# hannes-holey/GaPFlow

Measured on AMD Instinct MI355X. Metric: Mcell-updates/s (fp64), 4096^2 grid, higher is better.
Workload: dtype f64; 1 GPU; 2D journal bearing 4096x4096, fixed DH EOS, all-periodic, adaptive CFL 0.5 (BASELINE.json configs[2]); slabs=1

## Files before the change

### gapflow_amd/_lib.py

```python
import ctypes as C
import os

import numpy as np

HERE = os.path.dirname(os.path.abspath(__file__))
LIB_PATH = os.environ.get('GPF_LIB_PATH', os.path.join(HERE, 'lib', 'libgapflow_hip.so'))

EOS_IDS = {'DH': 0, 'PL': 1, 'vdW': 2, 'MT': 3, 'cubic': 4, 'BWR': 5, 'Bayada': 6}
EOS_KEYS = {'DH': ['rho0', 'P0', 'C1', 'C2'], 'PL': ['rho0', 'P0', 'alpha'], 'vdW': ['M', 'T', 'a', 'b'],
            'MT': ['rho0', 'P0', 'K', 'n'], 'cubic': ['a', 'b', 'c', 'd'], 'BWR': ['T', 'gamma'],
            'Bayada': ['rho_l', 'rho_v', 'c_l', 'c_v']}
EOS_DEFAULTS = {'DH': {'rho0': 877.7007, 'P0': 101325., 'C1': 3.5e8, 'C2': 1.23}, 'PL': {'rho0': 1.1853, 'P0': 101325., 'alpha': 0.},
                'vdW': {'M': 39.948, 'T': 100., 'a': 1.355, 'b': 0.03201}, 'MT': {'rho0': 700., 'P0': 0.101e6, 'K': 0.557e9, 'n': 7.33},
                'cubic': {'a': 15.2, 'b': -9.6, 'c': 3.35, 'd': -0.07}, 'BWR': {'gamma': 3.}, 'Bayada': {}}
PIEZO_IDS = {'Barus': 1, 'Roelands': 2, 'Dukler': 3, 'McAdams': 4}
PIEZO_KEYS = {'Barus': ['aB'], 'Roelands': ['mu_inf', 'p_ref', 'z'], 'Dukler': ['eta_v', 'rho_l', 'rho_v'],
              'McAdams': ['eta_v', 'rho_l', 'rho_v']}
PIEZO_DEFAULTS = {'Barus': {'aB': 2.e-8}, 'Roelands': {'mu_inf': 1.e-3, 'p_ref': 1.96e8, 'z': 0.68},
                  'Dukler': {'eta_v': 3.9e-5, 'rho_l': 850., 'rho_v': 0.019}, 'McAdams': {'eta_v': 3.9e-5, 'rho_l': 850., 'rho_v': 0.019}}
THINNING_DEFAULTS = {'Eyring': {'tauE': 5.e5}, 'Carreau': {'mu_inf': 1.e-3, 'lam': 0.02, 'a': 2., 'N': 0.8}}
THINNING_IDS = {'Eyring': 1, 'Carreau': 2}
THINNING_KEYS = {'Eyring': ['tauE'], 'Carreau': ['mu_inf', 'lam', 'a', 'N']}
BC_P, BC_D, BC_N = 0, 1, 2
FIELD_Q, FIELD_TOPO, FIELD_EXTRA, FIELD_PRESSURE, FIELD_TAU_AVG, FIELD_WALL_LOWER, FIELD_WALL_UPPER = range(7)
FIELD_PRESSURE_VAR, FIELD_WALL_XZ_VAR, FIELD_WALL_YZ_VAR = 7, 8, 9
FIELD_DEFORMATION = 10
PROFILE_Z, PROFILE_U, PROFILE_V, PROFILE_TAU = 1, 2, 4, 8
PROFILE_GRADIENTS = 1
PROFILE_MODES = {'both': 0, 'top': 1, 'bottom': 2, 'none': 3}
FIELD_NCOMP = {FIELD_Q: 3, FIELD_TOPO: 3, FIELD_EXTRA: 1, FIELD_PRESSURE: 1, FIELD_TAU_AVG: 3,
               FIELD_WALL_LOWER: 6, FIELD_WALL_UPPER: 6, 7: 1, 8: 1, 9: 1, 10: 1}


class GpfConfig(C.Structure):
    _fields_ = [('Nx', C.c_int32), ('Ny', C.c_int32), ('dx', C.c_double), ('dy', C.c_double),
                ('U', C.c_double), ('V', C.c_double), ('eta', C.c_double), ('zeta', C.c_double),
                ('eos', C.c_int32), ('eos_par', C.c_double * 8),
                ('piezo', C.c_int32), ('piezo_par', C.c_double * 4),
                ('bc_rule', (C.c_int32 * 3) * 4), ('bc_value', C.c_double * 4),
                ('halo_lo', C.c_int32), ('halo_hi', C.c_int32),
                ('adaptive', C.c_int32), ('CFL', C.c_double), ('dt_fixed', C.c_double), ('tol', C.c_double),
                ('max_it', C.c_int64), ('mc_order', C.c_int32), ('device', C.c_int32),
                ('thinning', C.c_int32), ('thinning_par', C.c_double * 4)]


class GpfScalars(C.Structure):
    _fields_ = [('step', C.c_int64), ('simtime', C.c_double), ('dt', C.c_double), ('ekin', C.c_double),
                ('ekin_old', C.c_double), ('residual', C.c_double), ('v_max', C.c_double), ('v_sound', C.c_double),
                ('mass', C.c_double), ('invalid', C.c_int32), ('converged', C.c_int32)]


_DP = C.POINTER(C.c_double)
_VPP = C.POINTER(C.c_void_p)
SIGNATURES = {
    'gpf_create': (C.c_int, [C.POINTER(GpfConfig), _VPP]),
    'gpf_destroy': (C.c_int, [C.c_void_p]),
    'gpf_set_stream': (C.c_int, [C.c_void_p, C.c_void_p]),
    'gpf_last_error': (C.c_char_p, []),
    'gpf_device_count': (C.c_int, []),
    'gpf_upload': (C.c_int, [C.c_void_p, C.c_int, _DP, C.c_size_t]),
    'gpf_download': (C.c_int, [C.c_void_p, C.c_int, _DP, C.c_size_t]),
    'gpf_update_closures': (C.c_int, [C.c_void_p]),
    'gpf_pre_run': (C.c_int, [C.c_void_p]),
    'gpf_step': (C.c_int, [C.c_void_p, C.c_int64, C.c_int, C.POINTER(GpfScalars), C.c_int64, C.POINTER(C.c_int64)]),
    'gpf_step_unfused': (C.c_int, [C.c_void_p]),
    'gpf_step_timed': (C.c_int, [C.c_void_p, C.c_int64, _DP, _DP]),
    'gpf_scalars': (C.c_int, [C.c_void_p, C.POINTER(GpfScalars)]),
    'gpf_set_ekin_old': (C.c_int, [C.c_void_p, C.c_double]),
    'gpf_set_dt': (C.c_int, [C.c_void_p, C.c_double]),
    'gpf_slab_message': (C.c_int, [C.c_void_p, _VPP, C.POINTER(C.c_size_t)]),
    'gpf_step_local': (C.c_int, [C.c_void_p, C.c_int]),
    'gpf_step_commit': (C.c_int, [C.c_void_p, C.c_int, C.c_void_p, C.c_int, C.c_int, C.c_int]),
    'gpf_state': (C.c_int, [C.c_void_p, C.POINTER(GpfScalars)]),
    'gpf_viscous_stress': (C.c_int, [C.c_int64] + [C.c_void_p] * 6 + [C.c_double] * 3 + [C.c_int] + [C.c_void_p] * 3),
    'gpf_eos': (C.c_int, [C.c_int, C.c_void_p, C.c_int64, C.c_void_p, C.c_void_p, C.c_void_p]),
    'gpf_viscosity': (C.c_int, [C.c_int, C.c_int, C.c_void_p, C.c_double, C.c_int64, C.c_void_p, C.c_void_p, C.c_void_p,
                              C.c_double, C.c_double, C.c_void_p]),
    'gpf_elastic_setup': (C.c_int, [C.c_void_p, C.c_int, C.c_int, C.c_void_p, C.c_size_t, C.c_double, C.c_double, C.c_int]),
    'gpf_elastic_update': (C.c_int, [C.c_void_p]),
    'gpf_elastic_slab_setup': (C.c_int, [C.c_void_p, C.c_int, C.c_int, C.c_int, C.c_void_p, C.c_size_t, C.c_void_p, C.c_size_t,
                                         C.c_void_p, C.c_size_t, C.c_double, C.c_double, C.c_int]),
    'gpf_elastic_slab_buffer': (C.c_int, [C.c_void_p, C.c_int, C.POINTER(C.c_void_p), C.POINTER(C.c_size_t)]),
    'gpf_elastic_slab_forward': (C.c_int, [C.c_void_p, C.c_void_p, C.c_int]),
    'gpf_elastic_slab_convolve': (C.c_int, [C.c_void_p]),
    'gpf_elastic_slab_finish': (C.c_int, [C.c_void_p]),
    'gpf_elastic_slab_apply': (C.c_int, [C.c_void_p]),
    'gpf_p2p_export': (C.c_int, [C.c_void_p, C.c_void_p, C.c_size_t]),
    'gpf_p2p_connect': (C.c_int, [C.c_void_p, C.c_int, C.c_int, C.c_void_p, C.c_int, C.c_int]),
    'gpf_p2p_set_timeout': (C.c_int, [C.c_void_p, C.c_double]),
    'gpf_upload_beyond': (C.c_int, [C.c_void_p, C.c_int, _DP, C.c_size_t]),
    'gpf_stream_probe': (C.c_int, [C.c_int, C.c_int, C.c_int, C.c_int64, C.c_int, _DP]),
    'gpf_step_p2p': (C.c_int, [C.c_void_p, C.c_int64, C.c_int]),
    'gpf_stage_message': (C.c_int, [C.c_void_p]),
    'gpf_stage_absorb': (C.c_int, [C.c_void_p, C.c_void_p, C.c_int, C.c_int, C.c_int]),
    'gpf_close_step_local': (C.c_int, [C.c_void_p]),
    'gpf_close_step_commit': (C.c_int, [C.c_void_p, C.c_void_p, C.c_int, C.POINTER(GpfScalars)]),
    'gpf_set_seam_topo': (C.c_int, [C.c_void_p, C.c_int, _DP, C.c_size_t]),
    'gpf_predictor_corrector': (C.c_int, [C.c_int, C.c_int, _DP, _DP, _DP, C.c_int, _DP, _DP]),
    'gpf_source': (C.c_int, [C.c_int, C.c_int, _DP, _DP, _DP, _DP, _DP, _DP]),
    'gpf_open_step': (C.c_int, [C.c_void_p]),
    'gpf_stage_closures': (C.c_int, [C.c_void_p]),
    'gpf_stage_advance': (C.c_int, [C.c_void_p, C.c_int]),
    'gpf_close_step': (C.c_int, [C.c_void_p, C.POINTER(GpfScalars)]),
    'gpf_gp_fit': (C.c_int, [C.c_int, C.c_int, C.c_int, C.c_int, _DP, _DP, C.c_double, _DP, C.c_double, _DP, _DP, _DP]),
    'gpf_gp_set_model': (C.c_int, [C.c_void_p, C.c_int, C.c_int, C.c_int, C.c_int, C.POINTER(C.c_int32), _DP, _DP, _DP,
                                   C.c_double, _DP, C.c_double, C.c_double]),
    'gpf_gp_clear_model': (C.c_int, [C.c_void_p, C.c_int]),
    'gpf_gp_factorisation': (C.c_char_p, []),
    'gpf_plan_note': (C.c_char_p, [C.c_void_p]),
    'gpf_gp_set_scales': (C.c_int, [C.c_void_p, C.c_int, _DP, C.c_double]),
    'gpf_gp_variance': (C.c_int, [C.c_void_p, C.c_int, C.c_int, _DP]),
    'gpf_gp_pass_counts': (C.c_int, [C.c_void_p, C.POINTER(C.c_int64), C.POINTER(C.c_int64)]),
    'gpf_gp_nll_open': (C.c_int, [C.c_int, C.c_int, C.c_int, C.c_int, _DP, _DP, C.c_double, C.POINTER(C.c_void_p)]),
    'gpf_gp_nll_eval': (C.c_int, [C.c_void_p, _DP, _DP, _DP, C.POINTER(C.c_int)]),
    'gpf_gp_nll_close': (C.c_int, [C.c_void_p]),
    'gpf_gap_profiles_op': (C.c_int, [C.c_int64, C.c_int] + [C.c_void_p] * 8 + [C.c_int, C.c_double, C.c_double, C.c_int, C.c_int,
                                                                              C.c_void_p]),
    'gpf_gap_profiles': (C.c_int, [C.c_void_p, C.c_int, C.c_int, C.c_int, C.c_int, C.c_int, C.c_void_p]),
    'gpf_profile_store_probe': (C.c_int, [C.c_int, C.c_int64, C.c_int, C.c_int, C.c_int, _DP]),
}

_lib = None


class GapflowHipError(RuntimeError):
    pass


def _pin_hip_runtime():
    import sys
    if os.environ.get('GPF_SYSTEM_HIP') == '1':
        return
    if 'torch' in sys.modules:
        libdir = os.path.join(os.path.dirname(sys.modules['torch'].__file__), 'lib')
        for var, name in (('GPF_ROCBLAS_PATH', 'librocblas.so'), ('GPF_HIPFFT_PATH', 'libhipfft.so')):
            if os.path.exists(os.path.join(libdir, name)):
                os.environ.setdefault(var, os.path.join(libdir, name))
        return
    try:
        import importlib.util
        spec = importlib.util.find_spec('torch')
    except (ImportError, ValueError):
        spec = None
    if spec is None or not spec.submodule_search_locations:
        return
    libdir = os.path.join(list(spec.submodule_search_locations)[0], 'lib')
    cand = os.path.join(libdir, 'libamdhip64.so')
    if os.path.exists(cand):
        C.CDLL(cand, mode=C.RTLD_GLOBAL)
        for var, name in (('GPF_ROCBLAS_PATH', 'librocblas.so'), ('GPF_HIPFFT_PATH', 'libhipfft.so')):
            if os.path.exists(os.path.join(libdir, name)):
                os.environ.setdefault(var, os.path.join(libdir, name))


def _preload_rocsolver():
    if os.environ.get('GPF_USE_ROCSOLVER') == '0':
        return
    path = os.environ.get('GPF_ROCBLAS_PATH')
    try:
        blas = C.CDLL(path if path and os.path.exists(path) else 'librocblas.so.5', mode=C.RTLD_GLOBAL)
    except OSError:
        return
    info = _DlInfo()
    libdl = C.CDLL(None)
    libdl.dladdr.argtypes, libdl.dladdr.restype = [C.c_void_p, C.POINTER(_DlInfo)], C.c_int
    if not libdl.dladdr(C.cast(blas.rocblas_create_handle, C.c_void_p), C.byref(info)) or not info.dli_fname:
        return
    here = os.path.dirname(info.dli_fname.decode())
    for name in ('librocsolver.so.0', 'librocsolver.so'):
        if os.path.exists(os.path.join(here, name)):
            try:
                C.CDLL(os.path.join(here, name), mode=C.RTLD_GLOBAL)
            except OSError:
                pass
            return


class _DlInfo(C.Structure):
    _fields_ = [('dli_fname', C.c_char_p), ('dli_fbase', C.c_void_p), ('dli_sname', C.c_char_p), ('dli_saddr', C.c_void_p)]


def load():
    global _lib
    if _lib is None:
        _pin_hip_runtime()
        _preload_rocsolver()
        if not os.path.exists(LIB_PATH):
            raise GapflowHipError(
                f"{LIB_PATH} not found: build it with `python -m gapflow_amd.build` (needs hipcc). "
                "gapflow_amd has no CPU fallback.")
        lib = C.CDLL(LIB_PATH)
        for name, (res, args) in SIGNATURES.items():
            fn = getattr(lib, name)
            fn.restype, fn.argtypes = res, args
        _lib = lib
    return _lib


def check(code):
    if code != 0:
        raise GapflowHipError(f"libgapflow_hip error {code}: {load().gpf_last_error().decode()}")


def require_device():
    lib = load()
    if lib.gpf_device_count() < 1:
        raise GapflowHipError("no HIP device visible: gapflow_amd runs its hot path on an MI355X only "
                              "(there is no CPU fallback)")
    return lib


def as_dp(a):
    return a.ctypes.data_as(_DP)


def f64c(a):
    return np.ascontiguousarray(a, dtype=np.float64)
```

### gapflow_amd/csrc/api.hip

```cpp
#include <hip/hip_runtime.h>
#include <algorithm>
#include <cmath>
#include <cstdio>
#include <cstdlib>
#include <cstring>
#include <map>
#include <mutex>
#include <string>
#include <tuple>
#include <vector>

#include "../../include/gapflow_hip.h"
#include "phys_setup.hpp"
#include "step_kernel.hip"
#include "aux_kernels.hip"
#include "step2_kernel.hip"
#include "gp_kernels.hip"
#include "elastic_kernels.hip"
#include "small_kernel.hip"
#include "profile_kernels.hip"

using namespace gpf;

static thread_local std::string g_err;
static const bool g_debug = std::getenv("GPF_DEBUG") != nullptr;
#define DBG(...) do { if (g_debug) { std::fprintf(stderr, "[gpf] " __VA_ARGS__); std::fprintf(stderr, "\n"); std::fflush(stderr); } } while (0)

static int fail(int code, const std::string& msg) {
    g_err = msg;
    return code;
}

struct gpf_handle;
static int enter(gpf_handle* h, bool reads_only = false);

#define HIP_TRY(expr)                                                                                   \
    do {                                                                                                \
        hipError_t e_ = (expr);                                                                         \
        if (e_ != hipSuccess)                                                                           \
            return fail(GPF_ERR_HIP, std::string(#expr) + ": " + hipGetErrorString(e_));               \
    } while (0)

#define GPF_TRY(expr)                                                                                   \
    do {                                                                                                \
        int r_ = (expr);                                                                                \
        if (r_ != GPF_OK) return r_;                                                                    \
    } while (0)

static_assert(sizeof(LogEntry) == sizeof(gpf_scalars_t), "LogEntry must mirror gpf_scalars_t");
static constexpr size_t PLANE_PAD_BYTES = 256;

struct gpf_handle {
    gpf_config cfg;
    Layout L;
    Edges E;
    Phys P;
    hipStream_t stream = nullptr;
    size_t field_bytes = 0;
    double* q[2] = {nullptr, nullptr};
    double* topo = nullptr;
    double* topo_line = nullptr;
    int topo_mode = 0;
    bool topo_hy0 = false;
    double* Ls = nullptr;
    double* g1 = nullptr;
    double* seam = nullptr;
    bool has_seam[2] = {false, false};
    struct { bool on = false; int nranks = 0, rank = 0, rank_lo = -1, rank_hi = -1; char* mine = nullptr;
             char* box[P2P_MAX_RANKS] = {}; unsigned long long* seq = nullptr; } p2p;
    double* halo = nullptr;
    double* beyond = nullptr;
    StepState* st = nullptr;
    Partial* partials = nullptr;
    unsigned int* arrive = nullptr;
    long long p2p_timeout_ticks = P2P_TIMEOUT_TICKS;
    bool split_edges = false;
    bool g1_ready = false;
    Partial* block_partials = nullptr;
    int nghost_blocks = 0;
    ScalarPartial* spart = nullptr;
    int nspart = 0;
    LogEntry* log = nullptr;
    long long log_cap = 0;
    double* stage = nullptr;
    size_t stage_doubles = 0;
    double* fields = nullptr;
    double* work = nullptr;
    struct GpHost {
        bool set = false;
        GpModelDev dev;
        double *Z = nullptr, *alpha = nullptr, *L = nullptr, *Linv = nullptr, *W = nullptr;
        int cap = 0;
        bool has_linv = false;
        double xscale0 = 1.0;
        double inv_scale[GP_MAX_D] = {};
        double yscale_fit = 1.0;
    } gp[3];
    double* gp_state_mean = nullptr;
    bool gp_state_mean_valid = false;
    long long gp_state_mean_step = -1;
    bool gp_state_mean_fresh = false;
    bool open_first_closures = false;
    bool gp_reuse_state_mean = true;
    long long gp_passes[3] = {0, 0, 0}, gp_reused = 0;
    double* gpvar = nullptr;
    double* gpscratch = nullptr;
    int gpscratch_n = 0;
    struct { bool on = false; int px = 0, py = 0, relative = 0; double alpha = 1.0, scale = 1.0; void* plan_f = nullptr; void* plan_b = nullptr;
             double2* greens = nullptr; double2* spec = nullptr; double* dense = nullptr;
             double* u_prev = nullptr; double* h0 = nullptr; double* deformation = nullptr; } el;
    struct { bool on = false; int px = 0, py = 0, nky = 0, nranks = 1, relative = 0;
             int row0 = 0, nrows = 0, k0 = 0, nk = 0, nret = 0, nrows_all = 0, nmain = 0, main_g0 = 0, seam_side = -1, seam_g0 = 0, ref_row = -1;
             double alpha = 1.0, scale = 1.0;
             void* plan_y = nullptr; void* plan_x = nullptr; void* plan_yb = nullptr; int nxg = 0, g_lo = 0;
             double* dense = nullptr; double2* spec = nullptr; double2* send1 = nullptr; double2* recv1 = nullptr; double2* xspec = nullptr;
             double2* greens = nullptr; double2* send2 = nullptr; double2* recv2 = nullptr; double2* line = nullptr; double* ureal = nullptr;
             double* u_prev = nullptr; double* h0 = nullptr; double* deformation = nullptr; double* ref = nullptr; int* rows_all = nullptr; } els;
    double* gptile = nullptr;
    size_t gptile_doubles = 0;
    void* blas = nullptr;
    bool step_open = false;
    int open_parity = 0;
    bool has_q = false, has_topo = false, pre_run_done = false;
    bool prev_state_valid = false;
    long long host_step = 0;
    long long next_step = 0;
    Strip2Geom geom2[2];
    int nchunks2 = 0, nblocks2 = 0, npartials2_cap = 0, nblock_partials_cap = 0;
    bool plan2_valid = false;
    int nt_policy2 = 0;
    int keep_rows2 = 0;
    StepState* st_trial = nullptr;
    double* plan_master = nullptr;
    char plan2_note[400] = "";
};

static int enter(gpf_handle* h, bool reads_only) {
    HIP_TRY(hipSetDevice(h->cfg.device));
    if (!reads_only) h->gp_state_mean_valid = false;
    return GPF_OK;
}

static void make_phys(const gpf_config& c, Phys& P) {
    setup_phys(P, c.U, c.V, c.eta, c.zeta, c.dx, c.dy, c.eos, c.eos_par, c.piezo, c.piezo_par, c.thinning, c.thinning_par);
}

static int blocks_for(long long n, int bs = 256, int cap = 4096) {
    long long b = (n + bs - 1) / bs;
    return (int)std::max<long long>(1, std::min<long long>(b, cap));
}

#ifdef GPF_ONLY_EOS_DH
#define EOS_DISPATCH(eos, ...)                                                                          \
    do {                                                                                                \
        if ((eos) == GPF_EOS_DH) { constexpr int EOS_ = EOS_DH; __VA_ARGS__; }       \
    } while (0)
#else
#define EOS_DISPATCH(eos, ...)                                                                          \
    switch (eos) {                                                                                      \
    case GPF_EOS_DH: { constexpr int EOS_ = EOS_DH; __VA_ARGS__; } break;                              \
    case GPF_EOS_PL: { constexpr int EOS_ = EOS_PL; __VA_ARGS__; } break;                              \
    case GPF_EOS_VDW: { constexpr int EOS_ = EOS_VDW; __VA_ARGS__; } break;                            \
    case GPF_EOS_MT: { constexpr int EOS_ = EOS_MT; __VA_ARGS__; } break;                              \
    case GPF_EOS_CUBIC: { constexpr int EOS_ = EOS_CUBIC; __VA_ARGS__; } break;                        \
    case GPF_EOS_BWR: { constexpr int EOS_ = EOS_BWR; __VA_ARGS__; } break;                            \
    default: { constexpr int EOS_ = EOS_BAYADA; __VA_ARGS__; } break;                                  \
    }
#endif

#define LS_PIEZO_DISPATCH(ls, pz, ...)                                                                  \
    do {                                                                                                \
        if (ls) {                                                                                       \
            constexpr bool LS_ = true;                                                                  \
            if (pz) { constexpr bool PZ_ = true; __VA_ARGS__; } else { constexpr bool PZ_ = false; __VA_ARGS__; }     \
        } else {                                                                                        \
            constexpr bool LS_ = false;                                                                 \
            if (pz) { constexpr bool PZ_ = true; __VA_ARGS__; } else { constexpr bool PZ_ = false; __VA_ARGS__; }     \
        }                                                                                               \
    } while (0)

extern "C" const char* gpf_last_error(void) { return g_err.c_str(); }

extern "C" int gpf_device_count(void) {
    int n = 0;
    if (hipGetDeviceCount(&n) != hipSuccess) return 0;
    return n;
}

static int ensure_stage(gpf_handle* h, size_t doubles) {
    if (h->stage_doubles >= doubles) return GPF_OK;
    if (h->stage) HIP_TRY(hipFree(h->stage));
    h->stage = nullptr; h->stage_doubles = 0;
    HIP_TRY(hipMalloc(&h->stage, doubles * sizeof(double)));
    h->stage_doubles = doubles;
    return GPF_OK;
}

#include "api_fields.inc"

extern "C" int gpf_create(const gpf_config* cfg, gpf_handle** out) {
    if (!cfg || !out) return fail(GPF_ERR_INVALID, "gpf_create: null argument");
    if (cfg->Nx < 1 || cfg->Ny < 1) return fail(GPF_ERR_INVALID, "gpf_create: Nx, Ny must be >= 1");
    if (!(cfg->dx > 0) || !(cfg->dy > 0)) return fail(GPF_ERR_INVALID, "gpf_create: dx, dy must be > 0");
    if (((long long)cfg->Nx + 2) * ((long long)cfg->Ny + 2 + 64) > 2000000000ll)
        return fail(GPF_ERR_INVALID, "gpf_create: more than 2e9 cells per plane; cut the domain into x-slabs (gapflow_amd/slab.py)");
    if (cfg->eos < GPF_EOS_DH || cfg->eos > GPF_EOS_BAYADA) return fail(GPF_ERR_INVALID, "gpf_create: unknown EOS id");
    if (cfg->thinning < 0 || cfg->thinning > GPF_THINNING_CARREAU) return fail(GPF_ERR_INVALID, "gpf_create: unknown shear-thinning id");
    for (int e = 0; e < 4; ++e) {
        int np = 0;
        for (int c = 0; c < 3; ++c) {
            int r = cfg->bc_rule[e][c];
            if (r < 0 || r > 2) return fail(GPF_ERR_INVALID, "gpf_create: bad ghost rule");
            np += (r == GPF_BC_PERIODIC);
        }
        if (np != 0 && np != 3)
            return fail(GPF_ERR_INVALID, "gpf_create: an edge must be periodic for all components or for none "
                                         "(problem.py:682-707 applies the periodic copy only when all three are 'P')");
    }
#ifdef GPF_ONLY_EOS_DH
    if (cfg->eos != GPF_EOS_DH) return fail(GPF_ERR_INVALID, "gpf_create: this build (-DGPF_ONLY_EOS_DH) holds the Dowson-Higginson kernels only");
#endif
    int ndev = 0;
    if (hipGetDeviceCount(&ndev) != hipSuccess || ndev == 0)
        return fail(GPF_ERR_NO_DEVICE, "gpf_create: no HIP device visible (this library has no CPU path)");
    if (cfg->device < 0 || cfg->device >= ndev) return fail(GPF_ERR_INVALID, "gpf_create: device ordinal out of range");
    HIP_TRY(hipSetDevice(cfg->device));

    gpf_handle* h = new gpf_handle();
    h->cfg = *cfg;
    Layout& L = h->L;
    L.Nx = cfg->Nx; L.Ny = cfg->Ny; L.off = 15;
    L.pitch = ((cfg->Ny + 2 + L.off + 15) / 16) * 16;
    if (const char* s = std::getenv("GPF_PITCH_PAD")) L.pitch += (std::atoi(s) / 16) * 16;
    L.plane = (long long)(cfg->Nx + 2) * L.pitch;
    if (const char* s = std::getenv("GPF_PLANE_PAD")) L.plane += (std::atoll(s) & ~1ll);
    for (int e = 0; e < 4; ++e) {
        for (int c = 0; c < 3; ++c) h->E.rule[e][c] = cfg->bc_rule[e][c];
        h->E.value[e] = cfg->bc_value[e];
    }
    h->E.halo[0] = cfg->halo_lo; h->E.halo[1] = cfg->halo_hi;
    h->split_edges = std::getenv("GPF_STEP_UNFUSED_EDGES") != nullptr;
    h->gp_reuse_state_mean = std::getenv("GPF_GP_NO_STATE_MEAN") == nullptr;
    make_phys(*cfg, h->P);

    const size_t plane_b = (size_t)L.plane * sizeof(double);
    auto cleanup = [&](int code) { gpf_destroy(h); return code; };
#define HIP_TRY_C(expr)                                                                                 \
    do {                                                                                                \
        hipError_t e_ = (expr);                                                                         \
        if (e_ != hipSuccess)                                                                           \
            return cleanup(fail(GPF_ERR_HIP, std::string(#expr) + ": " + hipGetErrorString(e_)));      \
    } while (0)
    h->field_bytes = (3 * plane_b + PLANE_PAD_BYTES + 255) & ~(size_t)255;
    for (int b = 0; b < 2; ++b) {
        HIP_TRY_C(field_malloc((void**)&h->q[b], h->field_bytes));
        if (field_zero(0, h->q[b], h->field_bytes) != GPF_OK) { gpf_destroy(h); return GPF_ERR_HIP; }
    }
    HIP_TRY_C(field_malloc((void**)&h->topo, h->field_bytes));
    if (field_zero(0, h->topo, h->field_bytes) != GPF_OK) { gpf_destroy(h); return GPF_ERR_HIP; }
    HIP_TRY_C(hipDeviceSynchronize());
    const size_t g1n = (size_t)3 * L.pitch + (size_t)3 * (L.Nx + 2);
    HIP_TRY_C(hipMalloc(&h->g1, g1n * sizeof(double)));
    HIP_TRY_C(hipMemset(h->g1, 0, g1n * sizeof(double)));
    HIP_TRY_C(hipMalloc(&h->st, sizeof(StepState)));
    HIP_TRY_C(hipMemset(h->st, 0, sizeof(StepState)));
    h->nghost_blocks = std::max(1, std::min(64, (2 * (L.Ny + 2) + 2 * L.Nx + 255) / 256));
    HIP_TRY_C(hipMalloc(&h->arrive, 4 * sizeof(unsigned int)));
    HIP_TRY_C(hipMemset(h->arrive, 0, 4 * sizeof(unsigned int)));
    HIP_TRY_C(hipMalloc(&h->block_partials, 1024 * sizeof(Partial)));
    h->nspart = 1024;
    HIP_TRY_C(hipMalloc(&h->spart, (size_t)(h->nspart + 8) * sizeof(ScalarPartial)));
    HIP_TRY_C(hipMemset(h->spart, 0, (size_t)(h->nspart + 8) * sizeof(ScalarPartial)));
    h->log_cap = 4096;
    HIP_TRY_C(hipMalloc(&h->log, (size_t)h->log_cap * sizeof(LogEntry)));
#undef HIP_TRY_C
    *out = h;
    return GPF_OK;
}

extern "C" int gpf_destroy(gpf_handle* h) {
    if (!h) return GPF_OK;
    hipSetDevice(h->cfg.device);
    hipStreamSynchronize(h->stream);
    for (void* p : {(void*)h->q[0], (void*)h->q[1], (void*)h->topo, (void*)h->plan_master}) field_free(p);
    void* ptrs[] = {h->topo_line, h->Ls, h->g1, h->seam, h->halo, h->beyond, h->st, h->partials, h->arrive, h->block_partials, h->spart,
                    h->log, h->stage, h->fields, h->work, h->st_trial, h->gpvar, h->gp_state_mean, h->gpscratch, h->gptile,
                    h->gp[0].Z, h->gp[0].alpha, h->gp[0].L, h->gp[1].Z, h->gp[1].alpha, h->gp[1].L,
                    h->gp[2].Z, h->gp[2].alpha, h->gp[2].L, h->gp[0].Linv, h->gp[1].Linv, h->gp[2].Linv, h->gp[0].W, h->gp[1].W, h->gp[2].W};
    if (h->blas && roclibs().ok) roclibs().destroy(h->blas);
    if (h->el.plan_f) fftlib().destroy(h->el.plan_f);
    if (h->el.plan_b) fftlib().destroy(h->el.plan_b);
    for (void* p : {(void*)h->el.greens, (void*)h->el.spec, (void*)h->el.dense, (void*)h->el.u_prev})
        if (p) hipFree(p);
    for (void* pl : {h->els.plan_y, h->els.plan_x, h->els.plan_yb})
        if (pl) fftlib().destroy(pl);
    for (void* p : {(void*)h->els.dense, (void*)h->els.spec, (void*)h->els.send1, (void*)h->els.recv1, (void*)h->els.xspec, (void*)h->els.greens,
                    (void*)h->els.send2, (void*)h->els.recv2, (void*)h->els.line, (void*)h->els.ureal, (void*)h->els.u_prev, (void*)h->els.ref,
                    (void*)h->els.rows_all})
        if (p) hipFree(p);
    for (int r = 0; r < h->p2p.nranks; ++r)
        if (h->p2p.box[r] && r != h->p2p.rank) hipIpcCloseMemHandle(h->p2p.box[r]);
    if (h->p2p.mine) hipFree(h->p2p.mine);
    if (h->p2p.seq) hipFree(h->p2p.seq);
    for (void* p : ptrs)
        if (p) hipFree(p);
    delete h;
    return GPF_OK;
}

extern "C" int gpf_set_stream(gpf_handle* h, void* s) {
    if (!h) return fail(GPF_ERR_INVALID, "null handle");
    h->stream = (hipStream_t)s;
    return GPF_OK;
}

static int field_ncomp(int field) {
    switch (field) {
    case GPF_FIELD_Q: return 3;
    case GPF_FIELD_TOPO: return 3;
    case GPF_FIELD_EXTRA: return 1;
    case GPF_FIELD_PRESSURE: return 1;
    case GPF_FIELD_TAU_AVG: return 3;
    case GPF_FIELD_WALL_LOWER: return 6;
    case GPF_FIELD_WALL_UPPER: return 6;
    case GPF_FIELD_PRESSURE_VAR: case GPF_FIELD_WALL_XZ_VAR: case GPF_FIELD_WALL_YZ_VAR: return 1;
    case GPF_FIELD_DEFORMATION: return 1;
    }
    return 0;
}

static int current_parity(gpf_handle* h, int* par) {
    StepState s;
    HIP_TRY(hipMemcpyAsync(&s, h->st, sizeof(s), hipMemcpyDeviceToHost, h->stream));
    HIP_TRY(hipStreamSynchronize(h->stream));
    *par = s.parity;
    return GPF_OK;
}

static int ensure_fields(gpf_handle* h) {
    if (h->fields) return GPF_OK;
    HIP_TRY(hipMalloc(&h->fields, (size_t)16 * h->L.plane * sizeof(double)));
    HIP_TRY(hipMemsetAsync(h->fields, 0, (size_t)16 * h->L.plane * sizeof(double), h->stream));
    return GPF_OK;
}

extern "C" int gpf_upload(gpf_handle* h, int field, const double* host, size_t count) {
    if (!h || !host) return fail(GPF_ERR_INVALID, "gpf_upload: null argument");
    GPF_TRY(enter(h));
    const Layout& L = h->L;
    const int nc = field_ncomp(field);
    if (field != GPF_FIELD_Q && field != GPF_FIELD_TOPO && field != GPF_FIELD_EXTRA)
        return fail(GPF_ERR_INVALID, "gpf_upload: only q, topography and the extra field are inputs");
    const size_t ncell = (size_t)(L.Nx + 2) * (L.Ny + 2);
    if (count != ncell * nc) return fail(GPF_ERR_INVALID, "gpf_upload: count does not match ncomp*(Nx+2)*(Ny+2)");
    double* dst = nullptr;
    if (field == GPF_FIELD_Q) {
        int par = 0;
        GPF_TRY(current_parity(h, &par));
        dst = h->q[par];
    } else if (field == GPF_FIELD_TOPO) {
        dst = h->topo;
    } else {
        bool nz = false;
        for (size_t i = 0; i < count && !nz; ++i) nz = host[i] != 0.0;
        if (!nz && !h->Ls) return GPF_OK;
        if (!h->Ls) { HIP_TRY(hipMalloc(&h->Ls, (size_t)L.plane * sizeof(double) + PLANE_PAD_BYTES)); h->plan2_valid = false; }
        HIP_TRY(hipMemsetAsync(h->Ls, 0, (size_t)L.plane * sizeof(double), h->stream));
        dst = h->Ls;
    }
    if (field == GPF_FIELD_TOPO) {
        const int nx = L.Nx + 2, ny = L.Ny + 2;
        bool xonly = true, yonly = true;
        for (int c = 0; c < 3 && (xonly || yonly); ++c)
            for (int ix = 0; ix < nx && (xonly || yonly); ++ix) {
                const double* row = host + ((size_t)c * nx + ix) * ny;
                const double* row0 = host + (size_t)c * nx * ny;
                for (int iy = 0; iy < ny; ++iy) {
                    if (std::memcmp(&row[iy], &row[0], 8) != 0) xonly = false;
                    if (std::memcmp(&row[iy], &row0[iy], 8) != 0) yonly = false;
                }
            }
        const int mode = xonly ? 1 : (yonly ? 2 : 0);
        if (mode != h->topo_mode) { h->plan2_valid = false; }
        h->topo_mode = (h->el.on || h->els.on) ? 0 : mode;
        if (mode) {
            const int n = mode == 1 ? nx : ny;
            std::vector<double> line((size_t)3 * n);
            for (int c = 0; c < 3; ++c)
                for (int i = 0; i < n; ++i)
                    line[(size_t)c * n + i] = mode == 1 ? host[((size_t)c * nx + i) * ny] : host[(size_t)c * nx * ny + i];
            bool hy0 = mode == 1;
            for (int i = 0; i < n && hy0; ++i) hy0 = line[(size_t)2 * n + i] == 0.0;
            if (hy0 != h->topo_hy0) h->plan2_valid = false;
            h->topo_hy0 = hy0;
            if (!h->topo_line) HIP_TRY(hipMalloc(&h->topo_line, (size_t)3 * (std::max(nx, ny)) * sizeof(double)));
            HIP_TRY(hipMemcpy(h->topo_line, line.data(), line.size() * sizeof(double), hipMemcpyHostToDevice));
        }
    }
    GPF_TRY(ensure_stage(h, count));
    HIP_TRY(hipMemcpyAsync(h->stage, host, count * sizeof(double), hipMemcpyHostToDevice, h->stream));
    hipLaunchKernelGGL(k_pack, dim3(blocks_for((long long)count)), dim3(256), 0, h->stream, h->stage, dst, L, nc);
    HIP_TRY(hipGetLastError());
    HIP_TRY(hipStreamSynchronize(h->stream));
    if (field == GPF_FIELD_Q) h->has_q = true;
    h->g1_ready = false;
    h->prev_state_valid = false;
    if (field == GPF_FIELD_TOPO) h->has_topo = true;
    return GPF_OK;
}

extern "C" int gpf_download(gpf_handle* h, int field, double* host, size_t count) {
    if (!h || !host) return fail(GPF_ERR_INVALID, "gpf_download: null argument");
    GPF_TRY(enter(h, true));
    const Layout& L = h->L;
    const int nc = field_ncomp(field);
    if (nc == 0) return fail(GPF_ERR_INVALID, "gpf_download: unknown field id");
    const size_t ncell = (size_t)(L.Nx + 2) * (L.Ny + 2);
    if (count != ncell * nc) return fail(GPF_ERR_INVALID, "gpf_download: count does not match ncomp*(Nx+2)*(Ny+2)");
    const double* src = nullptr;
    switch (field) {
    case GPF_FIELD_Q: {
        int par = 0;
        GPF_TRY(current_parity(h, &par));
        src = h->q[par];
        break;
    }
    case GPF_FIELD_TOPO: src = h->topo; break;
    case GPF_FIELD_EXTRA:
        if (!h->Ls) { std::memset(host, 0, count * sizeof(double)); return GPF_OK; }
        src = h->Ls; break;
    case GPF_FIELD_DEFORMATION:
        if (!h->el.on && !h->els.on) { std::memset(host, 0, count * sizeof(double)); return GPF_OK; }
        src = h->el.on ? h->el.deformation : h->els.deformation; break;
    case GPF_FIELD_PRESSURE_VAR: case GPF_FIELD_WALL_XZ_VAR: case GPF_FIELD_WALL_YZ_VAR:
        if (!h->gpvar) return fail(GPF_ERR_STATE, "gpf_download: no GP variance has been computed");
        src = h->gpvar + (size_t)(field - GPF_FIELD_PRESSURE_VAR) * L.plane;
        break;
    default:
        if (!h->fields) return fail(GPF_ERR_STATE, "gpf_download: derived fields requested before gpf_update_closures");
        src = h->fields + (field == GPF_FIELD_PRESSURE ? 0 : field == GPF_FIELD_TAU_AVG ? 1 : field == GPF_FIELD_WALL_LOWER ? 4 : 10) * L.plane;
    }
    GPF_TRY(ensure_stage(h, count));
    hipLaunchKernelGGL(k_unpack, dim3(blocks_for((long long)count)), dim3(256), 0, h->stream, src, h->stage, L, nc);
    HIP_TRY(hipGetLastError());
    HIP_TRY(hipMemcpyAsync(host, h->stage, count * sizeof(double), hipMemcpyDeviceToHost, h->stream));
    HIP_TRY(hipStreamSynchronize(h->stream));
    return GPF_OK;
}

static FieldPtrs field_ptrs(gpf_handle* h) {
    FieldPtrs F;
    F.p = h->fields; F.tau = h->fields + h->L.plane; F.lower = h->fields + 4 * h->L.plane; F.upper = h->fields + 10 * h->L.plane;
    return F;
}

static int gp_launch_mean(gpf_handle* h, int which, const double* q, bool with_grad, double* c2_out);
static int read_state(gpf_handle* h, StepState& s);

static const double* beyond_rows(gpf_handle* h, const double* q) {
    if (!h->beyond || (h->E.halo[0] != 1 && h->E.halo[1] != 1)) return nullptr;
    const bool working = h->step_open && q == h->q[h->open_parity ^ 1];
    return h->beyond + (working ? 2 * h->L.pitch : 0);
}

static int launch_fields(gpf_handle* h, const double* q, bool pressure_mean_cached = false) {
    GPF_TRY(ensure_fields(h));
    const Layout& L = h->L;
    const long long n = (long long)(L.Nx + 2) * (L.Ny + 2);
    FieldPtrs F = field_ptrs(h);
    EOS_DISPATCH(h->cfg.eos, {
        if (h->cfg.thinning != GPF_THINNING_NONE) {
            hipLaunchKernelGGL((k_pressure<EOS_>), dim3(blocks_for(n)), dim3(256), 0, h->stream, q, F.p, L, h->P);
            if ((h->E.halo[0] == 1 || h->E.halo[1] == 1) && !h->beyond)
                return fail(GPF_ERR_STATE, "shear thinning on a slab: upload the rows beyond the halo first (gpf_upload_beyond)");
            const double* by = beyond_rows(h, q);
            if (h->Ls) hipLaunchKernelGGL((k_fields_thinning<EOS_, true>), dim3(blocks_for(n)), dim3(256), 0, h->stream, q, h->topo, h->Ls, F, L, h->P, h->cfg.dx, h->cfg.dy, h->E.halo[0], h->E.halo[1], by);
            else hipLaunchKernelGGL((k_fields_thinning<EOS_, false>), dim3(blocks_for(n)), dim3(256), 0, h->stream, q, h->topo, (const double*)nullptr, F, L, h->P, h->cfg.dx, h->cfg.dy, h->E.halo[0], h->E.halo[1], by);
        } else if (h->Ls) hipLaunchKernelGGL((k_fields<EOS_, true>), dim3(blocks_for(n)), dim3(256), 0, h->stream, q, h->topo, h->Ls, F, L, h->P);
        else hipLaunchKernelGGL((k_fields<EOS_, false>), dim3(blocks_for(n)), dim3(256), 0, h->stream, q, h->topo, (const double*)nullptr, F, L, h->P);
    });
    HIP_TRY(hipGetLastError());
    for (int w = 0; w < 3; ++w) {
        if (!h->gp[w].set) continue;
        if (w == 0 && pressure_mean_cached) {
            HIP_TRY(hipMemcpyAsync(F.p, h->gp_state_mean, (size_t)L.plane * sizeof(double), hipMemcpyDeviceToDevice, h->stream));
            h->gp_reused += 1;
        } else GPF_TRY(gp_launch_mean(h, w, q, false, nullptr));
    }
    return GPF_OK;
}

extern "C" int gpf_update_closures(gpf_handle* h) {
    if (!h) return fail(GPF_ERR_INVALID, "null handle");
    if (!h->has_q || !h->has_topo) return fail(GPF_ERR_STATE, "gpf_update_closures: upload q and topography first");
    GPF_TRY(enter(h));
    int par = 0;
    GPF_TRY(current_parity(h, &par));
    if (h->prev_state_valid && !h->E.halo[0] && !h->E.halo[1]) {
        const Layout& L = h->L;
        StepState s;
        GPF_TRY(read_state(h, s));
        double* w = h->q[par ^ 1];
        const long long n = (long long)(L.Nx + 2) * (L.Ny + 2);
        const int nb = blocks_for(n);
        if (!h->work) HIP_TRY(hipMalloc(&h->work, (size_t)9 * L.plane * sizeof(double)));
        GPF_TRY(launch_fields(h, w));
        double *fx = h->work, *fy = h->work + 3 * L.plane, *src = h->work + 6 * L.plane;
        FieldPtrs F = field_ptrs(h);
        const int mc = h->cfg.mc_order;
        const int sw = mc == 0 ? (((s.step - 1) % 2 == 0) ? 1 : -1) : mc;
        const int dir = ((sw + 1) / 2) ? 1 : -1;
        hipLaunchKernelGGL(k_fluxdiff, dim3(nb), dim3(256), 0, h->stream, w, F.p, F.tau, dir, fx, fy, L);
        hipLaunchKernelGGL(k_source, dim3(nb), dim3(256), 0, h->stream, w, h->topo, F.tau, F.lower, F.upper, src, L);
        hipLaunchKernelGGL(k_axpy, dim3(nb), dim3(256), 0, h->stream, w, fx, fy, src, (const double*)&h->st->dt_last, h->cfg.dx, h->cfg.dy, L);
        hipLaunchKernelGGL(k_bc_x, dim3((L.Ny + 2 + 255) / 256), dim3(256), 0, h->stream, w, L, h->E);
        hipLaunchKernelGGL(k_bc_y, dim3((L.Nx + 2 + 255) / 256), dim3(256), 0, h->stream, w, L, h->E);
        HIP_TRY(hipGetLastError());
        GPF_TRY(launch_fields(h, w));
        h->prev_state_valid = false;
    } else {
        GPF_TRY(launch_fields(h, h->q[par]));
    }
    HIP_TRY(hipStreamSynchronize(h->stream));
    return GPF_OK;
}

static int launch_scalars(gpf_handle* h, const double* q, ScalarPartial* total, bool need_sound_speed = true) {
    const Layout& L = h->L;
    const int row0 = h->E.halo[0] == 1 ? 1 : 0, row1 = h->E.halo[1] == 1 ? L.Nx : L.Nx + 1;
    const long long n = (long long)(row1 - row0 + 1) * (L.Ny + 2);
    const int nb = blocks_for(n, 256, h->nspart);
    EOS_DISPATCH(h->cfg.eos, {
        hipLaunchKernelGGL((k_scalars<EOS_>), dim3(nb), dim3(256), 0, h->stream, q, h->topo, L, h->P, row0, row1, h->spart);
    });
    HIP_TRY(hipGetLastError());
    hipLaunchKernelGGL(k_scalars_final, dim3(1), dim3(256), 0, h->stream, h->spart, nb, total);
    HIP_TRY(hipGetLastError());
    if (h->gp[0].set && need_sound_speed) GPF_TRY(gp_launch_mean(h, 0, q, true, &total->c2));
    return GPF_OK;
}

static void fill_scalars(const StepState& s, const ScalarPartial* sp, double dxdy, gpf_scalars_t* out) {
    out->step = s.step; out->simtime = s.simtime; out->dt = s.dt;
    out->ekin = sp ? sp->ekin : s.ekin; out->ekin_old = s.ekin_old; out->residual = s.residual;
    out->v_max = std::sqrt(sp ? sp->v2 : s.vmax2);
    out->v_sound = (sp && ((int)sp->flags & 4)) ? std::nan("") : std::sqrt(sp ? sp->c2 : s.c2max);
    out->mass = sp ? sp->mass * dxdy : 0.0;
    out->invalid = s.invalid; out->converged = s.converged;
}

extern "C" int gpf_scalars(gpf_handle* h, gpf_scalars_t* out) {
    if (!h || !out) return fail(GPF_ERR_INVALID, "gpf_scalars: null argument");
    if (!h->has_q || !h->has_topo) return fail(GPF_ERR_STATE, "gpf_scalars: upload q and topography first");
    GPF_TRY(enter(h, true));
    int par = 0;
    GPF_TRY(current_parity(h, &par));
    ScalarPartial* tot = h->spart + h->nspart;
    h->gp_state_mean_fresh = false;
    GPF_TRY(launch_scalars(h, h->q[par], tot));
    ScalarPartial sp; StepState s;
    HIP_TRY(hipMemcpyAsync(&sp, tot, sizeof(sp), hipMemcpyDeviceToHost, h->stream));
    HIP_TRY(hipMemcpyAsync(&s, h->st, sizeof(s), hipMemcpyDeviceToHost, h->stream));
    HIP_TRY(hipStreamSynchronize(h->stream));
    if (h->gp_state_mean_fresh && s.parity == par) {
        h->gp_state_mean_valid = true;
        h->gp_state_mean_step = s.step;
    }
    h->gp_state_mean_fresh = false;
    fill_scalars(s, &sp, h->cfg.dx * h->cfg.dy, out);
    return GPF_OK;
}

static int write_state(gpf_handle* h, const StepState& s) {
    HIP_TRY(hipMemcpyAsync(h->st, &s, sizeof(s), hipMemcpyHostToDevice, h->stream));
    HIP_TRY(hipStreamSynchronize(h->stream));
    return GPF_OK;
}
static int read_state(gpf_handle* h, StepState& s) {
    HIP_TRY(hipMemcpyAsync(&s, h->st, sizeof(s), hipMemcpyDeviceToHost, h->stream));
    HIP_TRY(hipStreamSynchronize(h->stream));
    return GPF_OK;
}

extern "C" int gpf_set_ekin_old(gpf_handle* h, double v) {
    if (!h) return fail(GPF_ERR_INVALID, "null handle");
    StepState s;
    GPF_TRY(read_state(h, s));
    s.ekin_old = v;
    return write_state(h, s);
}

extern "C" int gpf_set_dt(gpf_handle* h, double dt) {
    if (!h) return fail(GPF_ERR_INVALID, "null handle");
    StepState s;
    GPF_TRY(read_state(h, s));
    s.dt = dt;
    h->g1_ready = false;
    return write_state(h, s);
}

extern "C" int gpf_pre_run(gpf_handle* h) {
    if (!h) return fail(GPF_ERR_INVALID, "null handle");
    if (!h->has_q || !h->has_topo) return fail(GPF_ERR_STATE, "gpf_pre_run: upload q and topography first");
    GPF_TRY(enter(h));
    gpf_scalars_t sc;
    GPF_TRY(gpf_scalars(h, &sc));
    StepState s;
    GPF_TRY(read_state(h, s));
    const gpf_config& c = h->cfg;
    s.hmin = std::min(c.dx, c.dy);
    s.tol = c.tol; s.CFL = c.CFL; s.adaptive = c.adaptive; s.mc_order = c.mc_order; s.max_it = c.max_it;
    s.step = 0; s.simtime = 0.0; s.residual = 1.0;
    s.rbuf[0] = 1.0; s.rcount = 1; s.rhead = 0;
    s.converged = (1.0 < c.tol) ? 1 : 0;
    s.invalid = 0;
    s.dt_last = 0.0;
    if (!h->pre_run_done) s.ekin_old = sc.ekin;
    s.ekin = sc.ekin;
    s.vmax2 = sc.v_max * sc.v_max; s.c2max = sc.v_sound * sc.v_sound;
    const double dt_crit = s.hmin / (sc.v_max + sc.v_sound);
    s.dt = c.adaptive ? c.CFL * dt_crit : c.dt_fixed;
    GPF_TRY(write_state(h, s));
    h->pre_run_done = true;
    h->g1_ready = false;
    h->prev_state_valid = false;
    h->host_step = 0; h->next_step = 0;
    return GPF_OK;
}

static int topo_mode_of(const gpf_handle* h) {
    if (h->Ls != nullptr || h->cfg.piezo != 0 || std::getenv("GPF_TOPO_PLANES")) return 0;
    if (h->topo_mode == 1 && h->topo_hy0 && !std::getenv("GPF_TOPO_GENERIC")) return 3;
    return h->topo_mode;
}

typedef void (*step2_kernel_t)(const Step2Args, const Phys);

static step2_kernel_t step2_kernel(int eos, bool has_ls, bool piezo, int D, int topo_mode) {
    step2_kernel_t k = nullptr;
    EOS_DISPATCH(eos, {
        if (piezo) {
            if (has_ls) k = D > 0 ? k_step2<EOS_, true, true, 1, 0> : k_step2<EOS_, true, true, -1, 0>;
            else k = D > 0 ? k_step2<EOS_, false, true, 1, 0> : k_step2<EOS_, false, true, -1, 0>;
        } else if (has_ls) {
            k = D > 0 ? k_step2<EOS_, true, false, 1, 0> : k_step2<EOS_, true, false, -1, 0>;
        } else if (topo_mode == 1) {
            k = D > 0 ? k_step2<EOS_, false, false, 1, 1> : k_step2<EOS_, false, false, -1, 1>;
        } else if (topo_mode == 2) {
            k = D > 0 ? k_step2<EOS_, false, false, 1, 2> : k_step2<EOS_, false, false, -1, 2>;
        } else if (topo_mode == 3) {
            k = D > 0 ? k_step2<EOS_, false, false, 1, 3> : k_step2<EOS_, false, false, -1, 3>;
        } else {
            k = D > 0 ? k_step2<EOS_, false, false, 1, 0> : k_step2<EOS_, false, false, -1, 0>;
        }
    });
    return k;
}

static Strip2Geom strip2_geom(const Layout& L, int D) {
    Strip2Geom G;
    const int e = (D < 0 && (L.Ny & 1)) ? 1 : 0;
    for (int k = 0; k < 2; ++k) {
        G.w0 = -1 - e - 4 * k;
        G.s_ghost = (L.Ny - G.w0 - 1) / STRIP2;
        const int p_ny = L.Ny - G.w0 - STRIP2 * G.s_ghost;
        G.lane_ghost = (p_ny + 1) >> 1; G.slot_ghost = (p_ny + 1) & 1;
        if (G.lane_ghost + 2 <= 63) break;
    }
    G.nstrips = G.s_ghost + 1;
    G.lane_wrap = G.lane_ghost + 1;
    const int p0 = -G.w0;
    G.wrap_ma = (p0 % 2 == 0) ? 0 : -1;
    const int d = 1 - G.wrap_ma;
    G.wrap_src_lane = G.lane_wrap + d / 2; G.wrap_src_slot = d & 1;
    return G;
}

static bool step2_fused(const gpf_handle* h) { return !h->split_edges; }

#include "api_plan.inc"

#ifndef GPF_SLAB_COMMIT_BLOCKS
#define GPF_SLAB_COMMIT_BLOCKS 24
#endif
constexpr int SLAB_COMMIT_BLOCKS = GPF_SLAB_COMMIT_BLOCKS;

static P2PArgs p2p_args(gpf_handle* h, bool on) {
    P2PArgs c;
    c.on = on ? 1 : 0; c.nranks = h->p2p.nranks; c.rank = h->p2p.rank; c.rank_lo = h->p2p.rank_lo; c.rank_hi = h->p2p.rank_hi;
    for (int r = 0; r < P2P_MAX_RANKS; ++r) c.box[r] = h->p2p.box[r];
    c.seq = h->p2p.seq; c.qa = h->q[0]; c.qb = h->q[1];
    return c;
}

static int ghost_args(gpf_handle* h, int honor_stop, GhostArgs& g) {
    const Layout& L = h->L;
    g.qa = h->q[0]; g.qb = h->q[1]; g.topo = h->topo; g.Ls = h->Ls;
    for (int e = 0; e < 2; ++e) {
        g.seam[e] = nullptr;
        if (h->E.halo[e] == 2) {
            if (!h->has_seam[e]) return fail(GPF_ERR_STATE, "periodic slab seam: call gpf_set_seam_topo for this edge first");
            g.seam[e] = h->seam + (size_t)e * 8 * L.pitch;
        }
    }
    g.g1x = h->g1; g.g1y = h->g1 + 3 * L.pitch;
    g.st = h->st; g.L = L; g.E = h->E; g.honor_stop = honor_stop;
    return GPF_OK;
}

static void fill_step2_args(gpf_handle* h, Step2Args& a2, int D, int honor_stop, long long log_base, double* slab_out, bool p2p) {
    const Layout& L = h->L;
    const bool fused = step2_fused(h);
    const Strip2Geom& G2 = h->geom2[D > 0 ? 0 : 1];
    a2.qa = h->q[0]; a2.qb = h->q[1]; a2.topo = h->topo; a2.topo_line = h->topo_line; a2.Ls = h->Ls;
    a2.g1x = h->g1; a2.g1y = h->g1 + 3 * L.pitch;
    a2.st = h->st; a2.partials = h->partials; a2.block_partials = h->block_partials; a2.arrive = h->arrive;
    a2.log = h->log; a2.log_base = log_base; a2.log_cap = h->log_cap;
    a2.L = L; a2.E = h->E; a2.G = G2; a2.nchunks = h->nchunks2; a2.fused = (fused ? 1 : 0) | (h->nt_policy2 >= 1 ? 2 : 0) | (h->nt_policy2 >= 2 ? 4 : 0) |
               (h->nt_policy2 >= 1 ? h->keep_rows2 << 3 : 0); a2.honor_stop = honor_stop;
    const bool slab = slab_out != nullptr;
    for (int e = 0; e < 2; ++e) a2.seam[e] = (h->E.halo[e] == 2 && h->has_seam[e]) ? h->seam + (size_t)e * 8 * L.pitch : nullptr;
    a2.out = slab_out; a2.msg = (slab && !p2p) ? h->halo : nullptr; a2.p2p = p2p_args(h, p2p);
}

static int enqueue_step(gpf_handle* h, int honor_stop, long long log_base, double* slab_out,
                        hipEvent_t ev0 = nullptr, hipEvent_t ev1 = nullptr, bool p2p = false) {
    const Layout& L = h->L;
    const int mc = h->cfg.mc_order;
    const int D = mc == 0 ? ((h->next_step % 2 == 0) ? 1 : -1) : (((mc + 1) / 2) ? 1 : -1);
    GPF_TRY(plan_step2(h, D));
    h->next_step += 1;
    const bool fused = step2_fused(h);
    const Strip2Geom& G2 = h->geom2[D > 0 ? 0 : 1];
    const int np_step = G2.nstrips * h->nchunks2;
    GhostArgs g;
    GPF_TRY(ghost_args(h, honor_stop, g));
    Step2Args a2;
    fill_step2_args(h, a2, D, honor_stop, log_base, slab_out, p2p);
    const bool slab = slab_out != nullptr;
    FinishArgs f;
    f.partials = h->partials; f.st = h->st;
    f.log = h->log; f.log_base = log_base; f.log_cap = h->log_cap; f.out = slab_out; f.honor_stop = honor_stop;
    f.L = L; f.E = h->E;
    f.p2p = p2p_args(h, p2p);
    f.arrive = h->arrive; f.msg = slab ? h->halo : nullptr;
    f.nstep_partials = np_step; f.block_partials = h->block_partials;
    GhostFillArgs gf;
    gf.qa = h->q[0]; gf.qb = h->q[1]; gf.st = h->st;
    gf.L = L; gf.E = h->E; gf.honor_stop = honor_stop;

    const int ntiles = (L.Nx + L.Ny + 63) / 64;
    const dim3 ggrid(std::min(ntiles, 512));
    const int nsend = slab ? std::min((6 * L.pitch + 1023) / 1024, 256) : 0;
    WaitArgs w;
    w.qa = h->q[0]; w.qb = h->q[1]; w.st = h->st; w.log = h->log; w.log_base = log_base; w.log_cap = h->log_cap;
    w.L = L; w.E = h->E; w.honor_stop = honor_stop; w.arrive = h->arrive + 1; w.timeout_ticks = h->p2p_timeout_ticks; w.p2p = f.p2p;
    w.gathered = nullptr; w.msg_len = 0; w.nranks = 0; w.rank_lo = w.rank_hi = -1; w.stage1 = fused ? 0 : 1;
    const bool has_ls = h->Ls != nullptr;
    if (fused) {
        const step2_kernel_t k2 = step2_kernel(h->cfg.eos, h->Ls != nullptr, h->cfg.piezo != 0, D, topo_mode_of(h));
        if (ev0) hipEventRecord(ev0, h->stream);
        hipLaunchKernelGGL(k2, dim3(h->nblocks2), dim3(256), 0, h->stream, a2, h->P);
        if (ev1) hipEventRecord(ev1, h->stream);
        if (p2p) {
            const dim3 cgrid(SLAB_COMMIT_BLOCKS);
            EOS_DISPATCH(h->cfg.eos, {
                hipLaunchKernelGGL((k_begin_slab<EOS_, false, false, false, true>), cgrid, dim3(256), 0, h->stream, g, w, h->P);
            });
        }
        h->g1_ready = false;
        HIP_TRY(hipGetLastError());
        return GPF_OK;
    }
    EOS_DISPATCH(h->cfg.eos, {
        if (!h->g1_ready) {
            if (topo_mode_of(h) == 3) hipLaunchKernelGGL((k_ghost_stage1<EOS_, false, false, true>), ggrid, dim3(256), 0, h->stream, g, h->P);
            else LS_PIEZO_DISPATCH(has_ls, h->cfg.piezo != 0, hipLaunchKernelGGL((k_ghost_stage1<EOS_, LS_, PZ_, false>), ggrid, dim3(256), 0, h->stream, g, h->P));
        }
        if (ev0) hipEventRecord(ev0, h->stream);
        hipLaunchKernelGGL(step2_kernel(h->cfg.eos, h->Ls != nullptr, h->cfg.piezo != 0, D, topo_mode_of(h)), dim3(h->nblocks2), dim3(256), 0, h->stream, a2, h->P);
        if (ev1) hipEventRecord(ev1, h->stream);
        hipLaunchKernelGGL((k_ghost_fill<EOS_>), dim3(h->nghost_blocks + nsend), dim3(256), 0, h->stream, gf, f, h->nghost_blocks, h->P);
        if (p2p) {
            if (topo_mode_of(h) == 3) hipLaunchKernelGGL((k_begin_slab<EOS_, false, false, true, true>), ggrid, dim3(256), 0, h->stream, g, w, h->P);
            else LS_PIEZO_DISPATCH(has_ls, h->cfg.piezo != 0, hipLaunchKernelGGL((k_begin_slab<EOS_, LS_, PZ_, false, true>), ggrid, dim3(256), 0, h->stream, g, w, h->P));
        }
    });
    h->g1_ready = p2p;
    HIP_TRY(hipGetLastError());
    return GPF_OK;
}

static bool small_grid_eligible(gpf_handle* h) {
    static const bool off = getenv("GPF_SMALL_GRID") && atoi(getenv("GPF_SMALL_GRID")) == 0;
    const long long nc = (long long)(h->L.Nx + 2) * (h->L.Ny + 2);
    return !off && nc * SMALL_DOUBLES_PER_CELL * 8 <= 150 * 1024 && h->cfg.thinning == GPF_THINNING_NONE && !h->E.halo[0] && !h->E.halo[1] &&
           !h->gp[0].set && !h->gp[1].set && !h->gp[2].set && !h->el.on;
}

static int enqueue_small_steps(gpf_handle* h, int nsteps, int honor_stop, long long log_base) {
    const Layout& L = h->L;
    SmallArgs a;
    a.qa = h->q[0]; a.qb = h->q[1]; a.topo = h->topo; a.Ls = h->Ls; a.st = h->st;
    a.log = h->log; a.log_base = log_base; a.log_cap = h->log_cap; a.L = L; a.E = h->E; a.nsteps = nsteps; a.honor_stop = honor_stop;
    const size_t lds = (size_t)(L.Nx + 2) * (L.Ny + 2) * SMALL_DOUBLES_PER_CELL * 8;
    EOS_DISPATCH(h->cfg.eos, {
        if (h->Ls) {
            HIP_TRY(hipFuncSetAttribute((const void*)k_small_steps<EOS_, true>, hipFuncAttributeMaxDynamicSharedMemorySize, (int)lds));
            hipLaunchKernelGGL((k_small_steps<EOS_, true>), dim3(1), dim3(512), lds, h->stream, a, h->P);
        } else {
            HIP_TRY(hipFuncSetAttribute((const void*)k_small_steps<EOS_, false>, hipFuncAttributeMaxDynamicSharedMemorySize, (int)lds));
            hipLaunchKernelGGL((k_small_steps<EOS_, false>), dim3(1), dim3(512), lds, h->stream, a, h->P);
        }
    });
    HIP_TRY(hipGetLastError());
    h->next_step += nsteps;
    h->g1_ready = false;
    return GPF_OK;
}

extern "C" int gpf_step(gpf_handle* h, int64_t n, int honor_stop, gpf_scalars_t* log, int64_t log_capacity,
                        int64_t* n_executed) {
    if (!h) return fail(GPF_ERR_INVALID, "null handle");
    if (!h->pre_run_done) return fail(GPF_ERR_STATE, "gpf_step: call gpf_pre_run first (Problem._pre_run, problem.py:412)");
    if (h->E.halo[0] || h->E.halo[1]) return fail(GPF_ERR_STATE, "gpf_step: this handle is a slab; use gpf_step_local / gpf_step_commit");
    if (h->cfg.thinning != GPF_THINNING_NONE)
        return fail(GPF_ERR_STATE, "gpf_step: shear thinning needs grad p (a wider stencil than the fused step has); use the stage-wise calls");
    if (n < 0) return fail(GPF_ERR_INVALID, "gpf_step: n < 0");
    GPF_TRY(enter(h));
    int64_t done = 0, logged = 0;
    const bool small = small_grid_eligible(h);
    while (done < n) {
        const int64_t batch = std::min<int64_t>(n - done, h->log_cap);
        const long long base = h->host_step;
        if (small) GPF_TRY(enqueue_small_steps(h, (int)batch, honor_stop, base));
        else for (int64_t i = 0; i < batch; ++i) GPF_TRY(enqueue_step(h, honor_stop, base, nullptr));
        StepState s;
        GPF_TRY(read_state(h, s));
        const long long ran = s.step - base;
        const long long entries = ran + ((s.invalid && ran < batch) ? 1 : 0);
        if (log && entries > 0) {
            const long long take = std::min<long long>(entries, log_capacity - logged);
            if (take > 0) {
                HIP_TRY(hipMemcpy(log + logged, h->log, (size_t)take * sizeof(LogEntry), hipMemcpyDeviceToHost));
                logged += take;
            }
        }
        h->host_step = s.step; h->next_step = s.step;
        h->prev_state_valid = ran >= 1 && !s.invalid;
        done += batch;
        if (ran < batch) break;
    }
    if (n_executed) *n_executed = h->host_step;
    return GPF_OK;
}

extern "C" int gpf_step_timed(gpf_handle* h, int64_t n, double* kernel_ms, double* total_ms) {
    if (!h || !kernel_ms || !total_ms) return fail(GPF_ERR_INVALID, "gpf_step_timed: null argument");
    if (!h->pre_run_done) return fail(GPF_ERR_STATE, "gpf_step_timed: call gpf_pre_run first");
    if (n < 1 || n > h->log_cap) return fail(GPF_ERR_INVALID, "gpf_step_timed: 1 <= n <= 4096");
    GPF_TRY(enter(h));
    std::vector<hipEvent_t> ev(2 * n + 2);
    for (auto& e : ev) HIP_TRY(hipEventCreate(&e));
    HIP_TRY(hipEventRecord(ev[2 * n], h->stream));
    int rc = GPF_OK;
    for (int64_t i = 0; i < n && rc == GPF_OK; ++i) rc = enqueue_step(h, 0, h->host_step, nullptr, ev[2 * i], ev[2 * i + 1]);
    HIP_TRY(hipEventRecord(ev[2 * n + 1], h->stream));
    HIP_TRY(hipStreamSynchronize(h->stream));
    double sum = 0.0;
    float ms = 0.f;
    for (int64_t i = 0; i < n; ++i) {
        HIP_TRY(hipEventElapsedTime(&ms, ev[2 * i], ev[2 * i + 1]));
        sum += ms;
    }
    HIP_TRY(hipEventElapsedTime(&ms, ev[2 * n], ev[2 * n + 1]));
    *kernel_ms = sum; *total_ms = ms;
    for (auto& e : ev) hipEventDestroy(e);
    StepState s;
    GPF_TRY(read_state(h, s));
    h->prev_state_valid = s.step > h->host_step && !s.invalid;
    h->host_step = s.step; h->next_step = s.step;
    return rc;
}

#include "api_unfused_step.inc"
#include "api_operators.inc"
#include "api_slab_allgather.inc"
#include "api_elastic.inc"
#include "api_slab_p2p.inc"
#include "api_gp.inc"
#include "api_stagewise.inc"
#include "api_slab_stagewise.inc"
#include "api_slab_elastic.inc"
#include "api_profiles.inc"
```

### gapflow_amd/csrc/api_plan.inc

```

constexpr int K2_LONG_MARCH_ROWS = 100;

static int plan_apply(gpf_handle* h, int nchunks, int nt, int keep = 0) {
    const Layout& L = h->L;
    const int nstrips = std::max(h->geom2[0].nstrips, h->geom2[1].nstrips);
    nchunks = std::max(1, std::min(nchunks, std::max(1, L.Nx / 4)));
    h->nchunks2 = nchunks;
    h->nt_policy2 = nt;
    h->keep_rows2 = nt >= 1 ? std::max(0, std::min(7, keep)) : 0;
    const int nwaves = nstrips * nchunks;
    h->nblocks2 = (((nwaves + 3) / 4) + 7) / 8 * 8;
    if (nwaves > h->npartials2_cap) {
        if (h->partials) HIP_TRY(hipFree(h->partials));
        h->partials = nullptr;
        HIP_TRY(hipMalloc(&h->partials, (size_t)nwaves * sizeof(Partial)));
        HIP_TRY(hipMemset(h->partials, 0, (size_t)nwaves * sizeof(Partial)));
        h->npartials2_cap = nwaves;
    }
    if (h->nblocks2 > h->nblock_partials_cap) {
        const int cap = std::max(1024, h->nblocks2);
        if (h->block_partials) HIP_TRY(hipFree(h->block_partials));
        h->block_partials = nullptr;
        HIP_TRY(hipMalloc(&h->block_partials, (size_t)cap * sizeof(Partial)));
        h->nblock_partials_cap = cap;
    }
    return GPF_OK;
}

static void fill_step2_args(gpf_handle* h, Step2Args& a2, int D, int honor_stop, long long log_base, double* slab_out, bool p2p);

static int plan_trial(gpf_handle* h, int D, float* us, int reps = 6, bool both = false) {
    static const int parity_value[2] = {0, 1};
    if (!h->st_trial) HIP_TRY(hipMalloc(&h->st_trial, sizeof(StepState)));
    h->prev_state_valid = false;
    both = both && h->plan_master != nullptr;
    int par = 0;
    if (both) GPF_TRY(current_parity(h, &par));
    Step2Args a2;
    fill_step2_args(h, a2, D, 0, 0, nullptr, false);
    a2.st = h->st_trial; a2.log = nullptr;
    const step2_kernel_t k2 = step2_kernel(h->cfg.eos, h->Ls != nullptr, h->cfg.piezo != 0, D, topo_mode_of(h));
    hipEvent_t e0, e1;
    HIP_TRY(hipEventCreate(&e0)); HIP_TRY(hipEventCreate(&e1));
    float total = 0.f;
    for (int r = -1; r < reps; ++r) {
        HIP_TRY(hipMemcpyAsync(h->st_trial, h->st, sizeof(StepState), hipMemcpyDeviceToDevice, h->stream));
        if (both && ((r + 1) & 1))
            HIP_TRY(hipMemcpyAsync(&h->st_trial->parity, &parity_value[par ^ 1], sizeof(int), hipMemcpyHostToDevice, h->stream));
        HIP_TRY(hipEventRecord(e0, h->stream));
        hipLaunchKernelGGL(k2, dim3(h->nblocks2), dim3(256), 0, h->stream, a2, h->P);
        HIP_TRY(hipEventRecord(e1, h->stream));
        HIP_TRY(hipEventSynchronize(e1));
        float ms = 0.f;
        HIP_TRY(hipEventElapsedTime(&ms, e0, e1));
        if (r >= 0) total += ms;
    }
    hipEventDestroy(e0); hipEventDestroy(e1);
    if (both) GPF_TRY(field_copy(h->stream, h->q[par], h->plan_master, h->field_bytes));
    HIP_TRY(hipGetLastError());
    *us = total / reps * 1e3f;
    return GPF_OK;
}

static float placement_best_seen(const gpf_handle* h, int D, float mine) {
    static std::mutex lock;
    static std::map<std::tuple<int, int, int, int, int, int, int>, float> seen;
    const auto key = std::make_tuple(h->L.Nx, h->L.Ny, h->cfg.eos, topo_mode_of(h), D, h->Ls ? 1 : 0, h->cfg.piezo != 0 ? 1 : 0);
    std::lock_guard<std::mutex> g(lock);
    float& v = seen[key];
    if (mine > 0.f && (v == 0.f || mine < v)) v = mine;
    return v;
}

static int plan_placement(gpf_handle* h, int D, std::string& note) {
    const char* env_tries = std::getenv("GPF_PLACEMENT_TRIES");
    const int fixed = env_tries ? std::atoi(env_tries) : -1;
    if (fixed == 0 || !h->plan_master) return GPF_OK;
    const bool print = std::getenv("GPF_PLACEMENT_PRINT") && std::atoi(std::getenv("GPF_PLACEMENT_PRINT")) != 0;
    int par = 0;
    GPF_TRY(current_parity(h, &par));
    const bool planes = topo_mode_of(h) == 0;
    double* const master = h->plan_master;
    std::vector<double*> pool = {h->q[par], h->q[par ^ 1]};
    std::vector<char> holds_state = {1, 0};
    std::vector<float> w = {0.f, 0.f};
    auto trial = [&](int i, int j, float* us, bool both) -> int {
        if (!holds_state[i]) {
            GPF_TRY(field_copy(h->stream, pool[i], master, h->field_bytes));
            holds_state[i] = 1;
        }
        holds_state[j] = 0;
        h->q[par] = pool[i]; h->q[par ^ 1] = pool[j];
        return plan_trial(h, D, us, 6, both);
    };
    float best_w = 0.f;
    for (int round = 0; round < (fixed > 0 ? 1 : 5); ++round) {
        int want = fixed > 0 ? fixed : 12;
        size_t free_b = 0, total_b = 0;
        HIP_TRY(hipMemGetInfo(&free_b, &total_b));
        while (want > 0 && (size_t)want * h->field_bytes + (2ull << 30) > free_b) --want;
        const size_t first = pool.size();
        for (int k = 0; k < want; ++k) {
            double* b = nullptr;
            if (field_malloc((void**)&b, h->field_bytes) != hipSuccess) { (void)hipGetLastError(); break; }
            GPF_TRY(field_zero(h->stream, b, h->field_bytes));
            pool.push_back(b); holds_state.push_back(0); w.push_back(0.f);
        }
        if (pool.size() == first) break;
        float batch_best = 0.f;
        for (size_t k = first; k < pool.size(); ++k) {
            GPF_TRY(trial(0, (int)k, &w[k], false));
            if (batch_best == 0.f || w[k] < batch_best) batch_best = w[k];
        }
        const bool paid = best_w == 0.f || batch_best < 0.99f * best_w;
        if (best_w == 0.f || batch_best < best_w) best_w = batch_best;
        const float known = placement_best_seen(h, D, 0.f);
        if (round >= 1 && !paid && !(known > 0.f && best_w > 1.03f * known)) break;
    }
    (void)placement_best_seen(h, D, best_w);
    const int n = (int)pool.size();
    if (n == 2) return GPF_OK;
    GPF_TRY(trial(0, 1, &w[1], false));
    GPF_TRY(trial(1, 0, &w[0], false));
    std::vector<int> order(n);
    for (int k = 0; k < n; ++k) order[k] = k;
    std::stable_sort(order.begin(), order.end(), [&](int x, int y) { return w[x] < w[y]; });
    const int m = std::min(n, 4);
    float own_pair = 0.f;
    GPF_TRY(trial(0, 1, &own_pair, true));
    int bi = 0, bj = 1;
    float best = own_pair, worst = own_pair;
    std::string pairs;
    for (int i = 0; i < m; ++i)
        for (int j = i + 1; j < m; ++j) {
            const int x = std::min(order[i], order[j]), y = std::max(order[i], order[j]);
            if (x == 0 && y == 1) continue;
            float t = 0.f;
            GPF_TRY(trial(x, y, &t, true));
            if (print) { char b2[40]; std::snprintf(b2, sizeof b2, " (%d,%d) %.1f", x, y, t); pairs += b2; }
            if (t < best) { best = t; bi = x; bj = y; }
            worst = std::max(worst, t);
        }
    if (print) {
        std::fprintf(stderr, "[gpf] placement: us per step writing each buffer (0, 1: the handle's own):");
        for (int k = 0; k < n; ++k) std::fprintf(stderr, " %.1f", w[k]);
        std::fprintf(stderr, "\n[gpf] placement: pairs, both directions: (0,1) %.1f%s\n", own_pair, pairs.c_str());
    }
    char buf[200];
    std::snprintf(buf, sizeof buf, " placement: %d buffers, written %.0f .. %.0f us, pair kept %.0f, the handle's own %.0f", n,
                  *std::min_element(w.begin(), w.end()), *std::max_element(w.begin(), w.end()), best, own_pair);
    note = buf;
    std::vector<double*> rest;
    for (int k = 0; k < n; ++k) if (k != bi && k != bj) rest.push_back(pool[k]);
    float us = 0.f;
    if (planes) {
        double* const own = h->topo;
        double* best_home = own;
        float best_t = 0.f;
        std::string seen;
        for (size_t k = 0; k <= std::min<size_t>(rest.size(), 3); ++k) {
            double* cand = k == 0 ? own : rest[k - 1];
            if (cand != own) GPF_TRY(field_copy(h->stream, cand, own, h->field_bytes));
            h->topo = cand;
            float t = 0.f;
            GPF_TRY(trial(bi, bj, &t, true));
            std::snprintf(buf, sizeof buf, " %.0f", t);
            seen += buf;
            if (k == 0 || t < best_t) { best_t = t; best_home = cand; }
        }
        note += "; gap planes:" + seen;
        if (best_home != own) {
            rest.erase(std::find(rest.begin(), rest.end(), best_home));
            rest.push_back(own);
        }
        h->topo = best_home;
    }
    GPF_TRY(trial(bi, bj, &us, true));
    HIP_TRY(hipStreamSynchronize(h->stream));
    for (double* b : rest) field_free(b);
    h->q[par] = pool[bi]; h->q[par ^ 1] = pool[bj];
    return GPF_OK;
}

static const char* const NT_NAME[3] = {"plain loads and stores", "non-temporal stores", "non-temporal loads and stores"};
constexpr int K2_KEEP_ROWS_DEFAULT = 4;
static const int K2_KEEP_CANDIDATES[2] = {3, 4};
static std::string keep_note(const gpf_handle* h) {
    if (h->nt_policy2 < 1) return "";
    char buf[64];
    std::snprintf(buf, sizeof buf, ", keep %d/8 rows on-die", h->keep_rows2);
    return buf;
}
static int plan_step2(gpf_handle* h, int D) {
    if (h->plan2_valid) return GPF_OK;
    const Layout& L = h->L;
    h->geom2[0] = strip2_geom(L, 1);
    h->geom2[1] = strip2_geom(L, -1);
    const int nstrips = std::max(h->geom2[0].nstrips, h->geom2[1].nstrips);
    int per_cu = 0, ncu = 0;
    HIP_TRY(hipOccupancyMaxActiveBlocksPerMultiprocessor(&per_cu, (const void*)step2_kernel(h->cfg.eos, h->Ls != nullptr, h->cfg.piezo != 0, 1, topo_mode_of(h)), 256, 0));
    HIP_TRY(hipDeviceGetAttribute(&ncu, hipDeviceAttributeMultiprocessorCount, h->cfg.device));
    const int all_resident = std::max(1, std::max(1, per_cu * ncu) * 4 / nstrips);
    const int one_per_simd = (ncu * 4) / nstrips;
    const double streamed = (double)L.plane * 8.0 * (6 + (topo_mode_of(h) == 0 ? 3 : 0) + (h->Ls ? 1 : 0));
    const bool nt_possible = streamed > 192.0 * 1024 * 1024;
    const char* env_chunks = std::getenv("GPF_CHUNKS");
    const char* env_nt = std::getenv("GPF_NT") ? std::getenv("GPF_NT") : std::getenv("GPF_NT_STORES");
    const char* env_tune = std::getenv("GPF_PLAN_TUNE");
    int nchunks = all_resident;
    if (one_per_simd >= 1 && L.Nx / one_per_simd >= K2_LONG_MARCH_ROWS) nchunks = one_per_simd;
    int nt = nt_possible ? 2 : 0;
    if (env_chunks && std::atoi(env_chunks) > 0) nchunks = std::atoi(env_chunks);
    if (env_nt) nt = std::max(0, std::min(2, std::atoi(env_nt)));
    const char* env_keep = std::getenv("GPF_KEEP_ROWS");
    int keep = nt_possible ? K2_KEEP_ROWS_DEFAULT : 0;
    if (env_keep) keep = std::max(0, std::min(7, std::atoi(env_keep)));
    const bool tune = !(env_tune && std::atoi(env_tune) == 0) && !h->split_edges && h->pre_run_done && (long long)L.Nx * L.Ny >= (1ll << 20) &&
                      one_per_simd >= 1 && L.Nx / one_per_simd >= 16 && !(env_chunks && env_nt);
    if (!tune) {
        GPF_TRY(plan_apply(h, nchunks, nt, keep));
        std::snprintf(h->plan2_note, sizeof h->plan2_note, "%d chunks per strip, %s%s (rule of thumb%s)", h->nchunks2,
                      NT_NAME[h->nt_policy2], keep_note(h).c_str(), (env_chunks || env_nt || env_keep) ? ", pinned by the environment" : "");
        h->plan2_valid = true;
        return GPF_OK;
    }
    std::string placement_note;
    GPF_TRY(plan_apply(h, nchunks, nt));
    {
        int par = 0;
        GPF_TRY(current_parity(h, &par));
        if (field_malloc((void**)&h->plan_master, h->field_bytes) == hipSuccess)
            GPF_TRY(field_copy(h->stream, h->plan_master, h->q[par], h->field_bytes));
        else { (void)hipGetLastError(); h->plan_master = nullptr; }
    }
    {
        float unused = 0.f;
        const double step_s = 1.1e-11 * (double)L.Nx * L.Ny + 1e-5;
        GPF_TRY(plan_trial(h, D, &unused, (int)std::min(200.0, std::max(8.0, 0.012 / step_s))));
    }
    float best = 0.f;
    int best_chunks = nchunks;
    int best_nt = nt;
    int best_keep = 0;
    std::string seen, keep_seen;
    auto pick_plan = [&]() -> int {
        best = 0.f;
        seen.clear();
        for (int c : {one_per_simd, all_resident}) {
            if (env_chunks && std::atoi(env_chunks) > 0) c = std::atoi(env_chunks);
            for (int pol = 0; pol < (nt_possible && !env_nt ? 3 : 1); ++pol) {
                const int cand_nt = env_nt ? nt : pol;
                GPF_TRY(plan_apply(h, c, cand_nt));
                float us = 0.f;
                GPF_TRY(plan_trial(h, D, &us, 6, true));
                char buf[48];
                std::snprintf(buf, sizeof buf, " %d/%s %.0f", h->nchunks2, cand_nt == 2 ? "nt" : cand_nt == 1 ? "nts" : "plain", us);
                seen += buf;
                if (best == 0.f || us < best) { best = us; best_chunks = c; best_nt = cand_nt; }
            }
            if ((env_chunks && std::atoi(env_chunks) > 0) || one_per_simd == all_resident) break;
        }
        best_keep = 0;
        keep_seen.clear();
        if (best_nt >= 1) {
            if (env_keep) best_keep = keep;
            else if (nt_possible) {
                char buf[48];
                std::snprintf(buf, sizeof buf, " 0 %.0f", best);
                keep_seen = buf;
                float best_k = best;
                for (int k : K2_KEEP_CANDIDATES) {
                    GPF_TRY(plan_apply(h, best_chunks, best_nt, k));
                    float us = 0.f;
                    GPF_TRY(plan_trial(h, D, &us, 6, true));
                    std::snprintf(buf, sizeof buf, ", %d %.0f", k, us);
                    keep_seen += buf;
                    if (us < best_k) { best_k = us; best_keep = k; }
                }
            }
        }
        return plan_apply(h, best_chunks, best_nt, best_keep);
    };
    const bool verify = std::getenv("GPF_PLACEMENT_PRINT") && std::atoi(std::getenv("GPF_PLACEMENT_PRINT")) >= 2;
    auto stamp = [&](const char* when) {
        if (!verify) return;
        int par = 0;
        if (current_parity(h, &par) != GPF_OK) return;
        std::fprintf(stderr, "[gpf] %-28s q[par] %p %016llx   master %p %016llx\n", when, (void*)h->q[par], field_checksum(h->stream, h->q[par], h->field_bytes),
                     (void*)h->plan_master, h->plan_master ? field_checksum(h->stream, h->plan_master, h->field_bytes) : 0ull);
    };
    stamp("before the first plan");
    GPF_TRY(pick_plan());
    stamp("after the first plan");
    const std::string first_seen = seen;
    GPF_TRY(plan_placement(h, D, placement_note));
    stamp("after the placement");
    if (!placement_note.empty()) GPF_TRY(pick_plan());
    stamp("after the second plan");
    HIP_TRY(hipStreamSynchronize(h->stream));
    field_free(h->plan_master);
    h->plan_master = nullptr;
    GPF_TRY(plan_apply(h, best_chunks, best_nt, best_keep));
    const std::string kept = keep_note(h) + (keep_seen.empty() ? (env_keep && h->nt_policy2 >= 1 ? " (pinned by the environment)" : "")
                                                               : " (timed, us: k" + keep_seen + ")");
    std::snprintf(h->plan2_note, sizeof h->plan2_note, "%d chunks per strip, %s%s (timed, us:%s;%s%s%s)", h->nchunks2,
                  NT_NAME[h->nt_policy2], kept.c_str(), seen.c_str(), placement_note.c_str(),
                  placement_note.empty() ? "" : "; before the placement:", placement_note.empty() ? "" : first_seen.c_str());
    DBG("plan_step2: %s", h->plan2_note);
    h->plan2_valid = true;
    return GPF_OK;
}

extern "C" const char* gpf_plan_note(gpf_handle* h) { return h ? h->plan2_note : ""; }
```

### gapflow_amd/csrc/api_slab_allgather.inc

```
static size_t halo_rows(const gpf_handle* h) { return h->cfg.thinning != GPF_THINNING_NONE ? 8 : 6; }
static size_t halo_len(gpf_handle* h) { return halo_rows(h) * h->L.pitch + 8; }

static int ensure_halo(gpf_handle* h) {
    if (h->halo) return GPF_OK;
    HIP_TRY(hipMalloc(&h->halo, halo_len(h) * sizeof(double)));
    HIP_TRY(hipMemsetAsync(h->halo, 0, halo_len(h) * sizeof(double), h->stream));
    return GPF_OK;
}

extern "C" int gpf_slab_message(gpf_handle* h, void** message, size_t* count) {
    if (!h || !message || !count) return fail(GPF_ERR_INVALID, "gpf_slab_message: null argument");
    GPF_TRY(enter(h, true));
    GPF_TRY(ensure_halo(h));
    *message = h->halo;
    *count = halo_len(h);
    return GPF_OK;
}

static HaloArgs halo_args(gpf_handle* h, int honor_stop, const double* gathered, int rank_lo, int rank_hi) {
    HaloArgs a;
    a.qa = h->q[0]; a.qb = h->q[1];
    a.msg = h->halo; a.gathered = gathered; a.rank_lo = rank_lo; a.rank_hi = rank_hi;
    a.st = h->st; a.L = h->L; a.E = h->E; a.honor_stop = honor_stop;
    a.work_parity = -1;
    a.beyond = nullptr;
    a.msg_rows = (int)halo_rows(h);
    return a;
}

extern "C" int gpf_step_local(gpf_handle* h, int honor_stop) {
    if (!h) return fail(GPF_ERR_INVALID, "gpf_step_local: null handle");
    if (!h->pre_run_done) return fail(GPF_ERR_STATE, "gpf_step_local: call gpf_pre_run first");
    GPF_TRY(enter(h));
    if (h->cfg.thinning != GPF_THINNING_NONE)
        return fail(GPF_ERR_STATE, "gpf_step_local: shear thinning needs grad p; use the stage-wise slab calls (gpf_stage_message / gpf_stage_absorb)");
    GPF_TRY(ensure_halo(h));
    double* rec = h->halo + (size_t)6 * h->L.pitch;
    GPF_TRY(enqueue_step(h, honor_stop, h->host_step, rec));
    return GPF_OK;
}

extern "C" int gpf_step_commit(gpf_handle* h, int honor_stop, const void* gathered, int nranks, int rank_lo, int rank_hi) {
    if (!h || !gathered || nranks < 1) return fail(GPF_ERR_INVALID, "gpf_step_commit: bad argument");
    if (rank_lo >= nranks || rank_hi >= nranks) return fail(GPF_ERR_INVALID, "gpf_step_commit: neighbour rank out of range");
    if (!h->halo) return fail(GPF_ERR_STATE, "gpf_step_commit without gpf_step_local");
    GPF_TRY(enter(h));
    const Layout& L = h->L;
    GhostArgs g;
    GPF_TRY(ghost_args(h, honor_stop, g));
    const bool fused = step2_fused(h);
    WaitArgs w;
    w.qa = h->q[0]; w.qb = h->q[1]; w.st = h->st; w.log = h->log; w.log_base = h->host_step; w.log_cap = h->log_cap;
    w.L = L; w.E = h->E; w.honor_stop = honor_stop; w.arrive = h->arrive + 1; w.timeout_ticks = h->p2p_timeout_ticks; w.p2p = p2p_args(h, false);
    w.gathered = (const double*)gathered; w.msg_len = (long long)halo_len(h); w.nranks = nranks; w.rank_lo = rank_lo; w.rank_hi = rank_hi;
    w.stage1 = fused ? 0 : 1;
    const dim3 ggrid(fused ? SLAB_COMMIT_BLOCKS : std::min((L.Nx + L.Ny + 63) / 64, 512));
    EOS_DISPATCH(h->cfg.eos, {
        if (fused) hipLaunchKernelGGL((k_begin_slab<EOS_, false, false, false, false>), ggrid, dim3(256), 0, h->stream, g, w, h->P);
        else if (topo_mode_of(h) == 3) hipLaunchKernelGGL((k_begin_slab<EOS_, false, false, true, false>), ggrid, dim3(256), 0, h->stream, g, w, h->P);
        else LS_PIEZO_DISPATCH(h->Ls != nullptr, h->cfg.piezo != 0, hipLaunchKernelGGL((k_begin_slab<EOS_, LS_, PZ_, false, false>), ggrid, dim3(256), 0, h->stream, g, w, h->P));
    });
    HIP_TRY(hipGetLastError());
    h->g1_ready = !fused;
    return GPF_OK;
}
```

### gapflow_amd/csrc/api_slab_p2p.inc

```
extern "C" int gpf_p2p_export(gpf_handle* h, void* ipc_handle, size_t handle_bytes) {
    if (!h || !ipc_handle) return fail(GPF_ERR_INVALID, "gpf_p2p_export: null argument");
    if (handle_bytes != sizeof(hipIpcMemHandle_t)) return fail(GPF_ERR_INVALID, "gpf_p2p_export: the handle buffer must hold 64 bytes");
    if (h->p2p.on) return fail(GPF_ERR_STATE, "gpf_p2p_export: already connected");
    GPF_TRY(enter(h));
    const size_t bytes = p2p_mailbox_bytes(h->L.pitch);
    if (!h->p2p.mine) {
        HIP_TRY(hipExtMallocWithFlags((void**)&h->p2p.mine, bytes, hipDeviceMallocFinegrained));
    }
    HIP_TRY(hipMemset(h->p2p.mine, 0, bytes));
    HIP_TRY(hipDeviceSynchronize());
    hipIpcMemHandle_t hm;
    HIP_TRY(hipIpcGetMemHandle(&hm, h->p2p.mine));
    std::memcpy(ipc_handle, &hm, sizeof(hm));
    return GPF_OK;
}

extern "C" int gpf_p2p_connect(gpf_handle* h, int rank, int nranks, const void* ipc_handles, int rank_lo, int rank_hi) {
    if (!h || !ipc_handles) return fail(GPF_ERR_INVALID, "gpf_p2p_connect: null argument");
    if (nranks < 1 || nranks > P2P_MAX_RANKS) return fail(GPF_ERR_INVALID, "gpf_p2p_connect: 1 <= nranks <= 16");
    if (rank < 0 || rank >= nranks || rank_lo >= nranks || rank_hi >= nranks) return fail(GPF_ERR_INVALID, "gpf_p2p_connect: rank out of range");
    if (!h->p2p.mine) return fail(GPF_ERR_STATE, "gpf_p2p_connect: call gpf_p2p_export first");
    if (h->p2p.on) return fail(GPF_ERR_STATE, "gpf_p2p_connect: already connected");
    GPF_TRY(enter(h));
    const hipIpcMemHandle_t* hs = (const hipIpcMemHandle_t*)ipc_handles;
    for (int r = 0; r < nranks; ++r) {
        if (r == rank) { h->p2p.box[r] = h->p2p.mine; continue; }
        void* p = nullptr;
        hipError_t e = hipIpcOpenMemHandle(&p, hs[r], hipIpcMemLazyEnablePeerAccess);
        if (e != hipSuccess) {
            for (int k = 0; k < r; ++k)
                if (k != rank && h->p2p.box[k]) { hipIpcCloseMemHandle(h->p2p.box[k]); h->p2p.box[k] = nullptr; }
            return fail(GPF_ERR_HIP, std::string("gpf_p2p_connect: hipIpcOpenMemHandle(rank ") + std::to_string(r) + "): " + hipGetErrorString(e));
        }
        h->p2p.box[r] = (char*)p;
    }
    if (!h->p2p.seq) HIP_TRY(hipMalloc((void**)&h->p2p.seq, sizeof(unsigned long long)));
    HIP_TRY(hipMemset(h->p2p.seq, 0, sizeof(unsigned long long)));
    HIP_TRY(hipDeviceSynchronize());
    h->p2p.nranks = nranks; h->p2p.rank = rank; h->p2p.rank_lo = rank_lo; h->p2p.rank_hi = rank_hi;
    h->p2p.on = true;
    return GPF_OK;
}

extern "C" int gpf_p2p_set_timeout(gpf_handle* h, double seconds) {
    if (!h || !(seconds > 0.0)) return fail(GPF_ERR_INVALID, "gpf_p2p_set_timeout: need a handle and a positive time");
    h->p2p_timeout_ticks = (long long)(seconds * 1e8);
    return GPF_OK;
}

extern "C" int gpf_step_p2p(gpf_handle* h, int64_t n, int honor_stop) {
    if (!h) return fail(GPF_ERR_INVALID, "gpf_step_p2p: null handle");
    if (!h->pre_run_done) return fail(GPF_ERR_STATE, "gpf_step_p2p: call gpf_pre_run first");
    if (!h->p2p.on) return fail(GPF_ERR_STATE, "gpf_step_p2p: call gpf_p2p_export / gpf_p2p_connect first");
    if (n < 0) return fail(GPF_ERR_INVALID, "gpf_step_p2p: n < 0");
    if (h->cfg.thinning != GPF_THINNING_NONE) return fail(GPF_ERR_STATE, "gpf_step_p2p: shear thinning needs grad p; use the stage-wise slab calls");
    GPF_TRY(enter(h));
    GPF_TRY(ensure_halo(h));
    double* rec = h->halo + (size_t)6 * h->L.pitch;
    for (int64_t i = 0; i < n; ++i) GPF_TRY(enqueue_step(h, honor_stop, h->host_step, rec, nullptr, nullptr, true));
    return GPF_OK;
}

extern "C" int gpf_state(gpf_handle* h, gpf_scalars_t* out) {
    if (!h || !out) return fail(GPF_ERR_INVALID, "gpf_state: null argument");
    GPF_TRY(enter(h, true));
    StepState s;
    GPF_TRY(read_state(h, s));
    fill_scalars(s, nullptr, 0.0, out);
    h->host_step = s.step; h->next_step = s.step;
    return GPF_OK;
}

extern "C" int gpf_set_seam_topo(gpf_handle* h, int side, const double* host, size_t count) {
    if (!h || !host || side < 0 || side > 1) return fail(GPF_ERR_INVALID, "gpf_set_seam_topo: bad argument");
    const Layout& L = h->L;
    if (count != (size_t)8 * (L.Ny + 2)) return fail(GPF_ERR_INVALID, "gpf_set_seam_topo: count must be 2*4*(Ny+2)");
    GPF_TRY(enter(h));
    if (!h->seam) {
        HIP_TRY(hipMalloc(&h->seam, (size_t)16 * L.pitch * sizeof(double)));
        HIP_TRY(hipMemset(h->seam, 0, (size_t)16 * L.pitch * sizeof(double)));
    }
    std::vector<double> tmp((size_t)8 * L.pitch, 0.0);
    for (int r = 0; r < 8; ++r)
        for (int iy = 0; iy < L.Ny + 2; ++iy) tmp[(size_t)r * L.pitch + L.off + iy] = host[(size_t)r * (L.Ny + 2) + iy];
    HIP_TRY(hipMemcpy(h->seam + (size_t)side * 8 * L.pitch, tmp.data(), tmp.size() * sizeof(double), hipMemcpyHostToDevice));
    h->has_seam[side] = true;
    return GPF_OK;
}
```

### gapflow_amd/csrc/aux_kernels.hip

```cpp
#include <hip/hip_runtime.h>
#include "device_types.hpp"

namespace gpf {

__global__ void k_pack(const double* __restrict__ src, double* __restrict__ dst, Layout L, int ncomp) {
    const long long ncell = (long long)(L.Nx + 2) * (L.Ny + 2);
    for (long long i = blockIdx.x * (long long)blockDim.x + threadIdx.x; i < ncell * ncomp;
         i += (long long)gridDim.x * blockDim.x) {
        const int c = (int)(i / ncell);
        const long long r = i - c * ncell;
        const int ix = (int)(r / (L.Ny + 2)), iy = (int)(r - (long long)ix * (L.Ny + 2));
        dst[c * L.plane + L.at(ix, iy)] = src[i];
    }
}

__global__ void k_unpack(const double* __restrict__ src, double* __restrict__ dst, Layout L, int ncomp) {
    const long long ncell = (long long)(L.Nx + 2) * (L.Ny + 2);
    for (long long i = blockIdx.x * (long long)blockDim.x + threadIdx.x; i < ncell * ncomp;
         i += (long long)gridDim.x * blockDim.x) {
        const int c = (int)(i / ncell);
        const long long r = i - c * ncell;
        const int ix = (int)(r / (L.Ny + 2)), iy = (int)(r - (long long)ix * (L.Ny + 2));
        dst[i] = src[c * L.plane + L.at(ix, iy)];
    }
}

__device__ __forceinline__ double ghost_x(const double* q, const Layout& L, const Edges& E, int e, int c, int iy) {
    const int r = E.rule[e][c];
    const int adj = e == 0 ? 1 : L.Nx;
    const int src = (r == BC_P) ? (e == 0 ? L.Nx : 1) : adj;
    const double v = q[c * L.plane + L.at(src, iy)];
    return r == BC_D ? 2.0 * E.value[e] - v : v;
}
__device__ __forceinline__ double ghost_y(const double* q, const Layout& L, const Edges& E, int e, int c, int ix) {
    const int r = E.rule[e][c];
    const int adj = e == 2 ? 1 : L.Ny;
    const int src = (r == BC_P) ? (e == 2 ? L.Ny : 1) : adj;
    const double v = q[c * L.plane + L.at(ix, src)];
    return r == BC_D ? 2.0 * E.value[e] - v : v;
}

__global__ void k_bc_x(double* q, Layout L, Edges E) {
    const int iy = blockIdx.x * blockDim.x + threadIdx.x;
    if (iy > L.Ny + 1) return;
    for (int e = 0; e < 2; ++e) {
        if (E.halo[e]) continue;
        const int ix = e == 0 ? 0 : L.Nx + 1;
        double v[3];
        for (int c = 0; c < 3; ++c) v[c] = ghost_x(q, L, E, e, c, iy);
        for (int c = 0; c < 3; ++c) q[c * L.plane + L.at(ix, iy)] = v[c];
    }
}
__global__ void k_bc_y(double* q, Layout L, Edges E) {
    const int ix = blockIdx.x * blockDim.x + threadIdx.x;
    if (ix > L.Nx + 1) return;
    for (int e = 2; e < 4; ++e) {
        const int iy = e == 2 ? 0 : L.Ny + 1;
        double v[3];
        for (int c = 0; c < 3; ++c) v[c] = ghost_y(q, L, E, e, c, ix);
        for (int c = 0; c < 3; ++c) q[c * L.plane + L.at(ix, iy)] = v[c];
    }
}

struct Acc {
    double ekin, v2, c2, mass;
    int flags;
    __device__ __forceinline__ void zero() { ekin = 0; v2 = 0; c2 = 0; mass = 0; flags = 0; }
    template <int EOS>
    __device__ __forceinline__ void cell(double r, double jx, double jy, double h, const Phys& P, double w = 1.0) {
        const double v = (jx * jx + jy * jy) / r;
        ekin += w * (v * 0.5);
        v2 = nanmax(v2, v);
        const double c = eos_c2<EOS>(r, P);
        if (!(c >= 0.0)) flags |= 4;
        c2 = fmax(c2, c);
        mass += w * (r * h);
        if (r != r || jx != jx || jy != jy) flags |= 1;
        if (r < 0.0) flags |= 2;
    }
    __device__ __forceinline__ void merge(const Acc& o) {
        ekin += o.ekin; v2 = nanmax(v2, o.v2); c2 = nanmax(c2, o.c2); mass += o.mass; flags |= o.flags;
    }
};

__device__ __forceinline__ Acc wave_reduce(Acc a) {
    for (int s = 32; s >= 1; s >>= 1) {
        Acc o;
        o.ekin = __shfl_down(a.ekin, s); o.v2 = __shfl_down(a.v2, s); o.c2 = __shfl_down(a.c2, s);
        o.mass = __shfl_down(a.mass, s); o.flags = __shfl_down(a.flags, s);
        a.merge(o);
    }
    return a;
}

__device__ __forceinline__ Acc block_reduce(Acc a, Acc* smem) {
    a = wave_reduce(a);
    const int lane = threadIdx.x & 63, w = threadIdx.x >> 6;
    if (lane == 0) smem[w] = a;
    __syncthreads();
    Acc r; r.zero();
    if (threadIdx.x == 0) {
        for (int i = 0; i < (int)(blockDim.x >> 6); ++i) r.merge(smem[i]);
    }
    __syncthreads();
    return r;
}

struct ScalarPartial { double ekin, v2, c2, mass, flags; };

template <int EOS>
__global__ __launch_bounds__(256) void k_scalars(const double* q, const double* topo, Layout L, Phys P, int row0,
                                                 int row1, ScalarPartial* out) {
    __shared__ Acc sm[4];
    Acc a; a.zero();
    const long long w = L.Ny + 2;
    const long long n = (long long)(row1 - row0 + 1) * w;
    for (long long i = blockIdx.x * (long long)blockDim.x + threadIdx.x; i < n; i += (long long)gridDim.x * blockDim.x) {
        const int ix = row0 + (int)(i / w), iy = (int)(i % w);
        const long long o = L.at(ix, iy);
        a.cell<EOS>(q[o], q[o + L.plane], q[o + 2 * L.plane], topo[o], P);
    }
    a = block_reduce(a, sm);
    if (threadIdx.x == 0) {
        ScalarPartial p = {a.ekin, a.v2, a.c2, a.mass, (double)a.flags};
        out[blockIdx.x] = p;
    }
}

__device__ __forceinline__ double critical_dt(const StepState* st, double v2, double c2) {
    return st->hmin / (sqrt(v2) + sqrt(c2));
}

__device__ inline void commit_step(StepState* st, double ekin, double v2, double c2, int flags, LogEntry* log,
                                   long long log_base, long long log_cap) {
    if (flags & 4) c2 = __builtin_nan("");
    flags &= 3;
    if (flags) {
        st->invalid = (flags & 1) ? 1 : 2;
    } else {
        const double dt_crit = critical_dt(st, v2, c2);
        const double cfl = st->dt / dt_crit;
        const double res = fabs(ekin - st->ekin_old) / st->ekin_old / cfl;
        st->residual = res;
        if (st->rcount < 5) { st->rbuf[st->rcount++] = res; }
        else { st->rbuf[st->rhead] = res; st->rhead = (st->rhead + 1) % 5; }
        bool conv = true;
        for (int i = 0; i < st->rcount; ++i) conv = conv && (st->rbuf[i] < st->tol);
        st->converged = conv ? 1 : 0;
        st->ekin_old = ekin;
        st->ekin = ekin; st->vmax2 = v2; st->c2max = c2;
        st->step += 1;
        st->simtime += st->dt;
        st->dt_last = st->dt;
        if (st->adaptive) st->dt = st->CFL * dt_crit;
        st->parity ^= 1;
    }
    if (log) {
        const long long k = (flags ? st->step : st->step - 1) - log_base;
        if (k >= 0 && k < log_cap) {
            LogEntry e;
            e.step = st->step; e.simtime = st->simtime; e.dt = st->dt; e.ekin = st->ekin; e.ekin_old = st->ekin_old;
            e.residual = st->residual; e.v_max = sqrt(st->vmax2); e.v_sound = sqrt(st->c2max); e.mass = 0.0;
            e.invalid = st->invalid; e.converged = st->converged;
            log[k] = e;
        }
    }
}

constexpr long long P2P_TIMEOUT_TICKS = 3000000000ll;
constexpr int P2P_MAX_RANKS = 16;
constexpr size_t P2P_ROWS_OFFSET = 4096;
struct MailHeader {
    unsigned long long flag[2][P2P_MAX_RANKS];
    double rec[2][P2P_MAX_RANKS][8];
};
__host__ __device__ inline size_t p2p_mailbox_bytes(int pitch) { return P2P_ROWS_OFFSET + (size_t)2 * 2 * 3 * pitch * sizeof(double); }
__device__ inline double* p2p_rows(char* box, int slot, int side, int pitch) {
    return (double*)(box + P2P_ROWS_OFFSET) + (size_t)(slot * 2 + side) * 3 * pitch;
}
struct P2PArgs {
    int on, nranks, rank, rank_lo, rank_hi;
    char* box[P2P_MAX_RANKS];
    unsigned long long* seq;
    const double* qa; const double* qb;
};

struct FinishArgs {
    const Partial* partials;
    StepState* st;
    LogEntry* log; long long log_base, log_cap;
    double* out;
    int honor_stop;
    Layout L; Edges E;
    int nstep_partials;
    Partial* block_partials;
    unsigned int* arrive;
    double* msg;
    P2PArgs p2p;
};

#ifdef GPF_STRICT_ATOMICS
#define GPF_ORDER_ARRIVE __ATOMIC_ACQ_REL
#define GPF_ORDER_LOAD __ATOMIC_ACQUIRE
#else
#define GPF_ORDER_ARRIVE __ATOMIC_RELAXED
#define GPF_ORDER_LOAD __ATOMIC_RELAXED
#endif

__device__ __forceinline__ void publish_partial(Partial* slot, const Acc& acc) {
    unsigned long long* w = reinterpret_cast<unsigned long long*>(slot);
    __hip_atomic_store(w + 0, (unsigned long long)__double_as_longlong(acc.ekin), __ATOMIC_RELAXED, __HIP_MEMORY_SCOPE_AGENT);
    __hip_atomic_store(w + 1, (unsigned long long)__double_as_longlong(acc.v2), __ATOMIC_RELAXED, __HIP_MEMORY_SCOPE_AGENT);
    __hip_atomic_store(w + 2, (unsigned long long)__double_as_longlong(acc.c2), __ATOMIC_RELAXED, __HIP_MEMORY_SCOPE_AGENT);
    __hip_atomic_store(w + 3, (unsigned long long)__double_as_longlong((double)acc.flags), __ATOMIC_RELAXED, __HIP_MEMORY_SCOPE_AGENT);
    asm volatile("s_waitcnt vmcnt(0)" ::: "memory");
}
__device__ __forceinline__ void merge_published(Acc& acc, const Partial* slot) {
    const unsigned long long* w = reinterpret_cast<const unsigned long long*>(slot);
    const double ekin = __longlong_as_double((long long)__hip_atomic_load(w + 0, GPF_ORDER_LOAD, __HIP_MEMORY_SCOPE_AGENT));
    const double v2 = __longlong_as_double((long long)__hip_atomic_load(w + 1, GPF_ORDER_LOAD, __HIP_MEMORY_SCOPE_AGENT));
    const double c2 = __longlong_as_double((long long)__hip_atomic_load(w + 2, GPF_ORDER_LOAD, __HIP_MEMORY_SCOPE_AGENT));
    const double fl = __longlong_as_double((long long)__hip_atomic_load(w + 3, GPF_ORDER_LOAD, __HIP_MEMORY_SCOPE_AGENT));
    acc.ekin += ekin; acc.v2 = nanmax(acc.v2, v2); acc.c2 = nanmax(acc.c2, c2); acc.flags |= (int)fl;
}

__device__ inline void finish_tail(StepState* st, LogEntry* log, long long log_base, long long log_cap, double* out,
                                   const Partial* block_partials, const P2PArgs& p2p, Acc* sm) {
    __shared__ double rec_sm[8];
    Acc acc; acc.zero();
    for (int i = threadIdx.x; i < (int)gridDim.x; i += blockDim.x) merge_published(acc, block_partials + i);
    acc = block_reduce(acc, sm);
    if (threadIdx.x == 0) {
        if (out) {
            const double inf = __builtin_inf();
            out[0] = acc.ekin;
            out[1] = acc.v2 != acc.v2 ? inf : acc.v2;
            out[2] = acc.c2 != acc.c2 ? inf : acc.c2;
            out[3] = (double)acc.flags;
            out[4] = out[5] = out[6] = out[7] = 0.0;
            for (int k = 0; k < 8; ++k) rec_sm[k] = out[k];
        } else {
            commit_step(st, acc.ekin, acc.v2, acc.c2, acc.flags, log, log_base, log_cap);
        }
    }
    if (p2p.on) {
        __syncthreads();
        const P2PArgs& c = p2p;
        const unsigned long long n = *c.seq + 1;
        const int slot = (int)(n & 1);
        if (threadIdx.x < c.nranks) {
            MailHeader* hd = (MailHeader*)c.box[threadIdx.x];
            for (int k = 0; k < 8; ++k) hd->rec[slot][c.rank][k] = rec_sm[k];
            __hip_atomic_store(&hd->flag[slot][c.rank], n, __ATOMIC_RELEASE, __HIP_MEMORY_SCOPE_SYSTEM);
        }
    }
}

__device__ inline void finish_tail(const FinishArgs& a, Acc* sm) {
    finish_tail(a.st, a.log, a.log_base, a.log_cap, a.out, a.block_partials, a.p2p, sm);
}

__device__ inline void finish_step(const FinishArgs& f, Acc own, Acc* sm) {
    __shared__ int last;
    const int per = (f.nstep_partials + (int)gridDim.x - 1) / (int)gridDim.x;
    const int i0 = blockIdx.x * per, i1 = min(i0 + per, f.nstep_partials);
    for (int i = i0 + threadIdx.x; i < i1; i += blockDim.x) {
        const Partial p = f.partials[i];
        own.ekin += p.ekin; own.v2 = nanmax(own.v2, p.vmax2); own.c2 = nanmax(own.c2, p.c2max); own.flags |= (int)p.flags;
    }
    own = block_reduce(own, sm);
    if (threadIdx.x == 0) {
        publish_partial(f.block_partials + blockIdx.x, own);
        last = __hip_atomic_fetch_add(f.arrive, 1u, GPF_ORDER_ARRIVE, __HIP_MEMORY_SCOPE_AGENT) == gridDim.x - 1 ? 1 : 0;
        if (last) __hip_atomic_store(f.arrive, 0u, __ATOMIC_RELAXED, __HIP_MEMORY_SCOPE_AGENT);
    }
    __syncthreads();
    if (!last) return;
    finish_tail(f, sm);
}

__device__ inline void send_rows_block(const double* q, const FinishArgs& f, int sblock, int nsblocks) {
    const Layout& L = f.L;
    double *dst_first, *dst_last;
    if (f.p2p.on) {
        const P2PArgs& c = f.p2p;
        const int slot = (int)((*c.seq + 1) & 1);
        dst_first = (c.rank_lo >= 0 && f.E.halo[0]) ? p2p_rows(c.box[c.rank_lo], slot, 1, L.pitch) : nullptr;
        dst_last = (c.rank_hi >= 0 && f.E.halo[1]) ? p2p_rows(c.box[c.rank_hi], slot, 0, L.pitch) : nullptr;
    } else {
        dst_first = f.msg; dst_last = f.msg + 3 * L.pitch;
    }
    const int total = 6 * L.pitch;
    for (int t = sblock * blockDim.x + threadIdx.x; t < total; t += nsblocks * blockDim.x) {
        const int side = t / (3 * L.pitch), k = (t / L.pitch) % 3, i = t % L.pitch;
        double* dst = side ? dst_last : dst_first;
        if (!dst) continue;
        const int ix = side ? L.Nx : 1, iy = i - L.off;
        double v = 0.0;
        if (iy >= 1 && iy <= L.Ny) v = q[k * L.plane + (long long)ix * L.pitch + i];
        else if (iy == 0 || iy == L.Ny + 1) v = ghost_y(q, L, f.E, iy == 0 ? 2 : 3, k, ix);
        if (f.p2p.on)
            __hip_atomic_store(reinterpret_cast<unsigned long long*>(dst + k * L.pitch + i), (unsigned long long)__double_as_longlong(v),
                               __ATOMIC_RELAXED, __HIP_MEMORY_SCOPE_SYSTEM);
        else dst[k * L.pitch + i] = v;
    }
    if (f.p2p.on) asm volatile("s_waitcnt vmcnt(0)" ::: "memory");
}

struct GhostFillArgs {
    double* qa; double* qb;
    const StepState* st;
    Layout L; Edges E;
    int honor_stop;
};

template <int EOS>
__device__ __forceinline__ Acc ghost_fill_block(const GhostFillArgs& a, const Phys& P, int block, int nblocks) {
    const Layout& L = a.L;
    double* q = a.st->parity ? a.qa : a.qb;
    Acc acc; acc.zero();
    auto put = [&](int ix, int iy, const double v[3], double w) {
        const long long o = L.at(ix, iy);
        q[o] = v[0]; q[o + L.plane] = v[1]; q[o + 2 * L.plane] = v[2];
        acc.cell<EOS>(v[0], v[1], v[2], 0.0, P, w);
    };
    const int nrow = 2 * (L.Ny + 2), ncol = 2 * L.Nx;
    for (int t = block * blockDim.x + threadIdx.x; t < nrow + ncol; t += nblocks * blockDim.x) {
        double v[3];
        if (t < nrow) {
            const int e = t / (L.Ny + 2), iy = t % (L.Ny + 2);
            if (a.E.halo[e]) continue;
            const int ix = e == 0 ? 0 : L.Nx + 1;
            if (iy >= 1 && iy <= L.Ny) {
                for (int c = 0; c < 3; ++c) v[c] = ghost_x(q, L, a.E, e, c, iy);
            } else {
                const int ey = iy == 0 ? 2 : 3;
                const int r0 = a.E.rule[ey][0];
                const int src = (r0 == BC_P) ? (ey == 2 ? L.Ny : 1) : (ey == 2 ? 1 : L.Ny);
                for (int c = 0; c < 3; ++c) {
                    const double gx = ghost_x(q, L, a.E, e, c, src);
                    v[c] = a.E.rule[ey][c] == BC_D ? 2.0 * a.E.value[ey] - gx : gx;
                }
            }
            put(ix, iy, v, 1.0);
        } else {
            const int u = t - nrow;
            const int e = 2 + u / L.Nx, ix = 1 + u % L.Nx;
            for (int c = 0; c < 3; ++c) v[c] = ghost_y(q, L, a.E, e, c, ix);
            const double w = 1.0 + ((ix == 1 && a.E.halo[0] == 2) ? 1.0 : 0.0) + ((ix == L.Nx && a.E.halo[1] == 2) ? 1.0 : 0.0);
            put(ix, e == 2 ? 0 : L.Ny + 1, v, w);
        }
    }
    return acc;
}

template <int EOS>
__global__ __launch_bounds__(256) void k_ghost_fill(const GhostFillArgs a, const FinishArgs f, int nfill, const Phys P) {
    __shared__ Acc sm[4];
    const StepState* st = a.st;
    if (st->invalid != 0 || (a.honor_stop && (st->converged || st->step >= st->max_it))) return;
    Acc own; own.zero();
    if ((int)blockIdx.x < nfill) own = ghost_fill_block<EOS>(a, P, blockIdx.x, nfill);
    else send_rows_block(st->parity ? a.qa : a.qb, f, blockIdx.x - nfill, gridDim.x - nfill);
    finish_step(f, own, sm);
}


struct HaloArgs {
    double* qa; double* qb;
    double* msg;
    const double* gathered;
    int rank_lo, rank_hi;
    const StepState* st;
    Layout L; Edges E;
    int honor_stop;
    int work_parity;
    double* beyond;
    int msg_rows;
};
__global__ void k_halo_pack(const HaloArgs a) {
    if (a.st->invalid != 0 || (a.honor_stop && (a.st->converged || a.st->step >= a.st->max_it))) return;
    const double* q = a.work_parity >= 0 ? (a.work_parity ? a.qb : a.qa) : (a.st->parity ? a.qa : a.qb);
    const int i = blockIdx.x * blockDim.x + threadIdx.x;
    if (i >= a.L.pitch) return;
    for (int c = 0; c < 3; ++c) {
        a.msg[c * a.L.pitch + i] = q[c * a.L.plane + (long long)1 * a.L.pitch + i];
        a.msg[(3 + c) * a.L.pitch + i] = q[c * a.L.plane + (long long)a.L.Nx * a.L.pitch + i];
    }
    if (a.msg_rows == 8) {
        a.msg[6 * a.L.pitch + i] = q[(long long)min(2, a.L.Nx) * a.L.pitch + i];
        a.msg[7 * a.L.pitch + i] = q[(long long)max(a.L.Nx - 1, 1) * a.L.pitch + i];
    }
}
__global__ void k_halo_unpack(const HaloArgs a) {
    if (a.st->invalid != 0 || (a.honor_stop && (a.st->converged || a.st->step >= a.st->max_it))) return;
    double* q = a.work_parity >= 0 ? (a.work_parity ? a.qb : a.qa) : (a.st->parity ? a.qa : a.qb);
    const int i = blockIdx.x * blockDim.x + threadIdx.x;
    if (i >= a.L.pitch) return;
    const long long len = (long long)a.msg_rows * a.L.pitch + 8;
    for (int c = 0; c < 3; ++c) {
        if (a.E.halo[0] && a.rank_lo >= 0) q[c * a.L.plane + i] = a.gathered[a.rank_lo * len + (3 + c) * a.L.pitch + i];
        if (a.E.halo[1] && a.rank_hi >= 0)
            q[c * a.L.plane + (long long)(a.L.Nx + 1) * a.L.pitch + i] = a.gathered[a.rank_hi * len + c * a.L.pitch + i];
    }
    if (a.beyond) {
        if (a.E.halo[0] && a.rank_lo >= 0) a.beyond[i] = a.gathered[a.rank_lo * len + 7 * a.L.pitch + i];
        if (a.E.halo[1] && a.rank_hi >= 0) a.beyond[a.L.pitch + i] = a.gathered[a.rank_hi * len + 6 * a.L.pitch + i];
    }
}

__global__ void k_beyond_average(double* state, const double* work, int n) {
    const int i = blockIdx.x * blockDim.x + threadIdx.x;
    if (i < n) state[i] = (work[i] + state[i]) / 2.0;
}

constexpr int INVALID_PEER_TIMEOUT = 3;
struct WaitArgs {
    double* qa; double* qb;
    StepState* st;
    LogEntry* log; long long log_base, log_cap;
    Layout L; Edges E;
    int honor_stop;
    unsigned int* arrive;
    long long timeout_ticks;
    P2PArgs p2p;
    const double* gathered;
    long long msg_len;
    int nranks, rank_lo, rank_hi;
    int stage1;
};
template <int EOS, bool HAS_LS, bool PIEZO, bool XONLY, bool MAILBOX>
__global__ __launch_bounds__(256) void k_begin_slab(const GhostArgs g, const WaitArgs a, const Phys P) {
    __shared__ int missing, last;
    __shared__ double tiles[2][3][64];
    StepState* st = a.st;
    if (st->invalid != 0 || (a.honor_stop && (st->converged || st->step >= st->max_it))) return;
    const P2PArgs& c = a.p2p;
    const unsigned long long n = MAILBOX ? *c.seq + 1 : 0ull;
    const int slot = (int)(n & 1);
    MailHeader* hd = MAILBOX ? (MailHeader*)c.box[c.rank] : nullptr;
    const int nranks = MAILBOX ? c.nranks : a.nranks, rank_lo = MAILBOX ? c.rank_lo : a.rank_lo, rank_hi = MAILBOX ? c.rank_hi : a.rank_hi;
    if (threadIdx.x == 0) missing = 0;
    __syncthreads();
    if (MAILBOX && threadIdx.x < c.nranks) {
        const long long t0 = wall_clock64();
        bool ok = false;
        int probes = 0;
        for (;;) {
            ok = __hip_atomic_load(&hd->flag[slot][threadIdx.x], __ATOMIC_RELAXED, __HIP_MEMORY_SCOPE_SYSTEM) >= n;
            if (ok) break;
            __builtin_amdgcn_s_sleep(2);
            if ((++probes & 255) == 0 && wall_clock64() - t0 > a.timeout_ticks) break;
        }
        if (!ok) atomicAdd(&missing, 1);
        __builtin_amdgcn_fence(__ATOMIC_ACQUIRE, "");
    }
    __syncthreads();
    const bool timed_out = missing != 0;
    double ekin = 0.0, v2 = 0.0, c2 = 0.0;
    int flags = 0;
    const Layout& L = a.L;
    for (int r = 0; r < nranks; ++r) {
        const double* p = MAILBOX ? hd->rec[slot][r] : a.gathered + r * a.msg_len + 6ll * L.pitch;
        ekin += p[0];
        v2 = fmax(v2, p[1]); c2 = fmax(c2, p[2]);
        flags |= (int)p[3];
    }
    const double inf = __builtin_inf();
    if (v2 == inf) v2 = __builtin_nan("");
    if (c2 == inf) c2 = __builtin_nan("");
    const int nblocks = gridDim.x * gridDim.y, block = blockIdx.y * gridDim.x + blockIdx.x;
    if (!timed_out && (flags & 3) == 0) {
        double* q = st->parity ? a.qa : a.qb;
        const double* row_lo = !(rank_lo >= 0 && a.E.halo[0]) ? nullptr
                             : MAILBOX ? p2p_rows(c.box[c.rank], slot, 0, L.pitch) : a.gathered + rank_lo * a.msg_len + 3ll * L.pitch;
        const double* row_hi = !(rank_hi >= 0 && a.E.halo[1]) ? nullptr
                             : MAILBOX ? p2p_rows(c.box[c.rank], slot, 1, L.pitch) : a.gathered + rank_hi * a.msg_len;
        for (int t = block * blockDim.x + threadIdx.x; t < 6 * L.pitch; t += nblocks * blockDim.x) {
            const int side = t / (3 * L.pitch), k = (t / L.pitch) % 3, i = t % L.pitch;
            const double* src = side ? row_hi : row_lo;
            if (src) q[k * L.plane + (long long)(side ? L.Nx + 1 : 0) * L.pitch + i] = src[k * L.pitch + i];
        }
        if (a.stage1) {
        const double c2_eff = (flags & 4) ? __builtin_nan("") : c2;
        const double dt = st->adaptive ? st->CFL * critical_dt(st, v2, c2_eff) : st->dt;
        const int D = direction_of_step(st, st->step + 1);
        MailField fld;
        fld.q = q; fld.L = L; fld.row_lo = row_lo; fld.row_hi = row_hi;
        const int ntiles = (L.Ny + L.Nx + 63) / 64;
        for (int tile = block; tile < ntiles; tile += nblocks) ghost_stage1_tile<EOS, HAS_LS, PIEZO, XONLY>(fld, g, P, D, tile * 64, dt, tiles);
        }
    }
    __syncthreads();
    if (threadIdx.x == 0) {
        if (timed_out) {
            __hip_atomic_fetch_add(a.arrive + 1, 1u, __ATOMIC_RELAXED, __HIP_MEMORY_SCOPE_AGENT);
            asm volatile("s_waitcnt vmcnt(0)" ::: "memory");
        }
        last = __hip_atomic_fetch_add(a.arrive, 1u, GPF_ORDER_ARRIVE, __HIP_MEMORY_SCOPE_AGENT) == (unsigned)nblocks - 1 ? 1 : 0;
    }
    __syncthreads();
    if (last && threadIdx.x == 0) {
        const unsigned int misses = __hip_atomic_load(a.arrive + 1, __ATOMIC_RELAXED, __HIP_MEMORY_SCOPE_AGENT);
        __hip_atomic_store(a.arrive, 0u, __ATOMIC_RELAXED, __HIP_MEMORY_SCOPE_AGENT);
        __hip_atomic_store(a.arrive + 1, 0u, __ATOMIC_RELAXED, __HIP_MEMORY_SCOPE_AGENT);
        if (misses) {
            st->invalid = INVALID_PEER_TIMEOUT;
        } else {
            if (MAILBOX) *c.seq = n;
            commit_step(st, ekin, v2, c2, flags, a.log, a.log_base, a.log_cap);
        }
    }
}

__global__ void k_record_unfused(const ScalarPartial* pre, const ScalarPartial* post, double* rec) {
    const double inf = __builtin_inf();
    rec[0] = post->ekin;
    rec[1] = post->v2 != post->v2 ? inf : post->v2;
    rec[2] = post->c2 != post->c2 ? inf : post->c2;
    rec[3] = (double)(((int)pre->flags & 3) | ((int)post->flags & 4));
    rec[4] = rec[5] = rec[6] = rec[7] = 0.0;
}

__global__ void k_commit_gathered(StepState* st, const double* gathered, long long len, long long rec_off, int nranks,
                                  LogEntry* log, long long log_base, long long log_cap, int honor_stop) {
    if (st->invalid != 0 || (honor_stop && (st->converged || st->step >= st->max_it))) return;
    double ekin = 0.0, v2 = 0.0, c2 = 0.0;
    int flags = 0;
    for (int r = 0; r < nranks; ++r) {
        const double* p = gathered + r * len + rec_off;
        ekin += p[0];
        v2 = fmax(v2, p[1]); c2 = fmax(c2, p[2]);
        flags |= (int)p[3];
    }
    const double inf = __builtin_inf();
    if (v2 == inf) v2 = __builtin_nan("");
    if (c2 == inf) c2 = __builtin_nan("");
    commit_step(st, ekin, v2, c2, flags, log, log_base, log_cap);
}

__global__ __launch_bounds__(256) void k_scalars_final(const ScalarPartial* in, int n, ScalarPartial* out) {
    __shared__ Acc sm[4];
    Acc a; a.zero();
    for (int i = threadIdx.x; i < n; i += blockDim.x) {
        Acc o; o.ekin = in[i].ekin; o.v2 = in[i].v2; o.c2 = in[i].c2; o.mass = in[i].mass; o.flags = (int)in[i].flags;
        a.merge(o);
    }
    a = block_reduce(a, sm);
    if (threadIdx.x == 0) {
        ScalarPartial p = {a.ekin, a.v2, a.c2, a.mass, (double)a.flags};
        out[0] = p;
    }
}

struct FieldPtrs {
    double* p;
    double* tau;
    double* lower;
    double* upper;
};

template <int EOS, bool HAS_LS>
__global__ __launch_bounds__(256) void k_fields(const double* q, const double* topo, const double* Ls, FieldPtrs F,
                                                Layout L, Phys P) {
    const long long w = L.Ny + 2, n = (long long)(L.Nx + 2) * w;
    for (long long i = blockIdx.x * (long long)blockDim.x + threadIdx.x; i < n; i += (long long)gridDim.x * blockDim.x) {
        const long long o = L.at((int)(i / w), (int)(i % w));
        CellIn c;
        c.rho = q[o]; c.jx = q[o + L.plane]; c.jy = q[o + 2 * L.plane];
        c.h = topo[o]; c.hx = topo[o + L.plane]; c.hy = topo[o + 2 * L.plane];
        c.Ls = HAS_LS ? Ls[o] : 0.0;
        CellFields f;
        cell_fields<EOS>(c, P, f);
        F.p[o] = f.p;
        for (int k = 0; k < 3; ++k) F.tau[o + k * L.plane] = f.tau[k];
        for (int k = 0; k < 6; ++k) { F.lower[o + k * L.plane] = f.lower[k]; F.upper[o + k * L.plane] = f.upper[k]; }
    }
}

template <int EOS>
__global__ __launch_bounds__(256) void k_pressure(const double* q, double* p, Layout L, Phys P) {
    const long long w = L.Ny + 2, n = (long long)(L.Nx + 2) * w;
    for (long long i = blockIdx.x * (long long)blockDim.x + threadIdx.x; i < n; i += (long long)gridDim.x * blockDim.x) {
        const long long o = L.at((int)(i / w), (int)(i % w));
        p[o] = eos_pressure<EOS>(q[o], P);
    }
}

template <int EOS, bool HAS_LS>
__global__ __launch_bounds__(256) void k_fields_thinning(const double* q, const double* topo, const double* Ls, FieldPtrs F,
                                                         Layout L, Phys P, double dx, double dy, int halo_lo, int halo_hi,
                                                         const double* beyond) {
    const long long w = L.Ny + 2, n = (long long)(L.Nx + 2) * w;
    for (long long i = blockIdx.x * (long long)blockDim.x + threadIdx.x; i < n; i += (long long)gridDim.x * blockDim.x) {
        const int ix = (int)(i / w), iy = (int)(i % w);
        const long long o = L.at(ix, iy);
        CellIn c;
        c.rho = q[o]; c.jx = q[o + L.plane]; c.jy = q[o + 2 * L.plane];
        c.h = topo[o]; c.hx = topo[o + L.plane]; c.hy = topo[o + 2 * L.plane];
        c.Ls = HAS_LS ? Ls[o] : 0.0;
        const double pc = F.p[o];
        const int ixm = ix > 0 ? ix - 1 : ix, ixp = ix < L.Nx + 1 ? ix + 1 : ix;
        const int iym = iy > 0 ? iy - 1 : iy, iyp = iy < L.Ny + 1 ? iy + 1 : iy;
        double dpx = (F.p[L.at(ixp, iy)] - F.p[L.at(ixm, iy)]) / ((ixp - ixm) * dx);
        if (beyond && ix == 0 && halo_lo == 1)
            dpx = (F.p[L.at(1, iy)] - eos_pressure<EOS>(beyond[L.off + iy], P)) / (2 * dx);
        if (beyond && ix == L.Nx + 1 && halo_hi == 1)
            dpx = (eos_pressure<EOS>(beyond[L.pitch + L.off + iy], P) - F.p[L.at(L.Nx, iy)]) / (2 * dx);
        const double dpy = (F.p[L.at(ix, iyp)] - F.p[L.at(ix, iym)]) / ((iyp - iym) * dy);
        const double mu0 = (P.piezo == PIEZO_NONE) ? P.eta : piezo_eta(P.eta, (EOS == EOS_BAYADA) ? c.rho : pc, P);
        const double eta = thinning_eta(mu0, dpx, dpy, c.h, P);
        CellFields f;
        cell_fields<EOS>(c, P, f, eta);
        for (int k = 0; k < 3; ++k) F.tau[o + k * L.plane] = f.tau[k];
        for (int k = 0; k < 6; ++k) { F.lower[o + k * L.plane] = f.lower[k]; F.upper[o + k * L.plane] = f.upper[k]; }
    }
}

__global__ __launch_bounds__(256) void k_fluxdiff(const double* q, const double* p, const double* tau, int d, double* fx,
                                                  double* fy, Layout L) {
    const long long w = L.Ny + 2, n = (long long)(L.Nx + 2) * w;
    for (long long i = blockIdx.x * (long long)blockDim.x + threadIdx.x; i < n; i += (long long)gridDim.x * blockDim.x) {
        const int ix = (int)(i / w), iy = (int)(i % w);
        const int ixn = (ix - d + (L.Nx + 2)) % (L.Nx + 2);
        const int iyn = (iy - d + (L.Ny + 2)) % (L.Ny + 2);
        const long long o = L.at(ix, iy), ox = L.at(ixn, iy), oy = L.at(ix, iyn);
        const double Fx0 = q[o + L.plane], Fx1 = p[o] + tau[o], Fx2 = tau[o + 2 * L.plane];
        const double Fy0 = q[o + 2 * L.plane], Fy1 = Fx2, Fy2 = p[o] + tau[o + L.plane];
        const double Gx0 = q[ox + L.plane], Gx1 = p[ox] + tau[ox], Gx2 = tau[ox + 2 * L.plane];
        const double Gy0 = q[oy + 2 * L.plane], Gy1 = tau[oy + 2 * L.plane], Gy2 = p[oy] + tau[oy + L.plane];
        const double s = -(double)d;
        fx[o] = s * (Gx0 - Fx0); fx[o + L.plane] = s * (Gx1 - Fx1); fx[o + 2 * L.plane] = s * (Gx2 - Fx2);
        fy[o] = s * (Gy0 - Fy0); fy[o + L.plane] = s * (Gy1 - Fy1); fy[o + 2 * L.plane] = s * (Gy2 - Fy2);
    }
}

__global__ __launch_bounds__(256) void k_source(const double* q, const double* h, const double* tau, const double* lower,
                                                const double* upper, double* out, Layout L) {
    const long long w = L.Ny + 2, n = (long long)(L.Nx + 2) * w, S = L.plane;
    for (long long i = blockIdx.x * (long long)blockDim.x + threadIdx.x; i < n; i += (long long)gridDim.x * blockDim.x) {
        const long long o = L.at((int)(i / w), (int)(i % w));
        const double h0 = h[o], hx = h[o + S], hy = h[o + 2 * S];
        out[o] = (-q[o + S] * hx - q[o + 2 * S] * hy) / h0;
        out[o + S] = ((tau[o] - upper[o]) * hx + (tau[o + 2 * S] - upper[o + 5 * S]) * hy + upper[o + 4 * S] - lower[o + 4 * S]) / h0;
        out[o + 2 * S] = ((tau[o + 2 * S] - upper[o + 5 * S]) * hx + (tau[o + S] - upper[o + S]) * hy + upper[o + 3 * S] - lower[o + 3 * S]) / h0;
    }
}

__global__ __launch_bounds__(256) void k_axpy(double* q, const double* fx, const double* fy, const double* src,
                                              const double* dtp, double dx, double dy, Layout L) {
    const double dt = *dtp;
    const long long w = L.Ny + 2, n = (long long)(L.Nx + 2) * w;
    for (long long i = blockIdx.x * (long long)blockDim.x + threadIdx.x; i < n; i += (long long)gridDim.x * blockDim.x) {
        const long long o = L.at((int)(i / w), (int)(i % w));
        for (int c = 0; c < 3; ++c) {
            const long long oc = o + c * L.plane;
            q[oc] = q[oc] - dt * (fx[oc] / dx + fy[oc] / dy - src[oc]);
        }
    }
}

__global__ __launch_bounds__(256) void k_average(double* q, const double* q0, Layout L) {
    const long long w = L.Ny + 2, n = (long long)(L.Nx + 2) * w;
    for (long long i = blockIdx.x * (long long)blockDim.x + threadIdx.x; i < n; i += (long long)gridDim.x * blockDim.x) {
        const long long o = L.at((int)(i / w), (int)(i % w));
        for (int c = 0; c < 3; ++c) q[o + c * L.plane] = (q[o + c * L.plane] + q0[o + c * L.plane]) / 2.0;
    }
}

__global__ void k_copy3(const double* src, double* dst, long long n) {
    for (long long i = blockIdx.x * (long long)blockDim.x + threadIdx.x; i < n; i += (long long)gridDim.x * blockDim.x)
        dst[i] = src[i];
}

__global__ void k_commit_unfused(StepState* st, const ScalarPartial* pre_bc, const ScalarPartial* post_bc) {
    const int flags = ((int)pre_bc->flags & 3) | ((int)post_bc->flags & 4);
    commit_step(st, post_bc->ekin, post_bc->v2, post_bc->c2, flags, nullptr, 0, 0);
}

struct ViscousArgs {
    const double* q; const double* h; const double* dqx; const double* dqy;
    const double* eta; const double* Ls;
    double U, V, zeta;
    int slip_both;
    double* out[3];
    long long n;
};
__global__ __launch_bounds__(256) void k_viscous(const ViscousArgs a) {
    for (long long i = blockIdx.x * (long long)blockDim.x + threadIdx.x; i < a.n; i += (long long)gridDim.x * blockDim.x) {
        double q[3], h[3], dx[3] = {0.0, 0.0, 0.0}, dy[3] = {0.0, 0.0, 0.0};
        for (int c = 0; c < 3; ++c) {
            q[c] = a.q[c * a.n + i]; h[c] = a.h[c * a.n + i];
            if (a.dqx) dx[c] = a.dqx[c * a.n + i];
            if (a.dqy) dy[c] = a.dqy[c * a.n + i];
        }
        const double Ls = a.Ls[i], lo = a.slip_both ? Ls : 0.0;
        for (int w = 0; w < 3; ++w) {
            if (!a.out[w]) continue;
            double t[6];
            viscous_general(w, q, h, dx, dy, a.U, a.V, a.eta[i], a.zeta, lo, Ls, t);
            if (w < 2) {
                for (int c = 0; c < 6; ++c) a.out[w][c * a.n + i] = t[c];
            } else {
                a.out[2][i] = t[0]; a.out[2][a.n + i] = t[1]; a.out[2][2 * a.n + i] = t[5];
            }
        }
    }
}

template <int EOS>
__global__ __launch_bounds__(256) void k_eos(const double* rho, long long n, Phys P, double* p, double* c) {
    for (long long i = blockIdx.x * (long long)blockDim.x + threadIdx.x; i < n; i += (long long)gridDim.x * blockDim.x) {
        if (p) p[i] = eos_pressure<EOS>(rho[i], P);
        if (c) c[i] = sqrt(eos_c2<EOS>(rho[i], P));
    }
}

__global__ __launch_bounds__(256) void k_viscosity(int kind, const double* a0, const double* a1, const double* a2, long long n,
                                                   double mu0, double u1, double u2, Phys P, double* out) {
    for (long long i = blockIdx.x * (long long)blockDim.x + threadIdx.x; i < n; i += (long long)gridDim.x * blockDim.x) {
        if (kind == 0) out[i] = piezo_eta(mu0, a0[i], P);
        else if (kind == 1) out[i] = thinning_factor(a0[i], mu0, P);
        else out[i] = shear_rate_avg(a0[i], a1[i], a2[i], u1, u2, mu0);
    }
}

}
```

### gapflow_amd/csrc/step2_kernel.hip

```cpp
#include <hip/hip_runtime.h>
#include "device_types.hpp"

namespace gpf {

constexpr int STRIP2 = 126;
#ifndef GPF_K2_AHEAD
#define GPF_K2_AHEAD 2
#endif
#ifndef GPF_K2_AHEAD_LINE
#define GPF_K2_AHEAD_LINE 4
#endif
#ifndef GPF_K2_MINWAVES
#define GPF_K2_MINWAVES 2
#endif
#ifndef GPF_K2_MINWAVES_LINE
#define GPF_K2_MINWAVES_LINE GPF_K2_MINWAVES
#endif
template <int EOS, bool HAS_LS, bool PIEZO>
struct Step2Weight {
    static constexpr bool heavy = EOS == EOS_PL || EOS == EOS_MT || EOS == EOS_BWR || EOS == EOS_BAYADA || (HAS_LS && PIEZO);
};

struct Strip2Geom {
    int w0;
    int nstrips;
    int s_ghost, lane_ghost, slot_ghost;
    int lane_wrap;
    int wrap_ma;
    int wrap_src_lane, wrap_src_slot;
};

struct Step2Args {
    const double* qa; const double* qb;
    const double* topo; const double* topo_line; const double* Ls;
    const double* g1x; const double* g1y;
    const double* seam[2];
    double* out;
    double* msg;
    P2PArgs p2p;
    StepState* st;
    Partial* partials;
    Partial* block_partials;
    unsigned int* arrive;
    LogEntry* log; long long log_base, log_cap;
    Layout L; Edges E; Strip2Geom G;
    int nchunks;
    int fused;
    int honor_stop;
};

__device__ __forceinline__ double lane_from_below(double v) {
#ifdef GPF_SHUFFLE_BPERMUTE
    return __shfl_up(v, 1);
#else
    const long long b = __double_as_longlong(v);
    int lo = (int)b, hi = (int)(b >> 32);
    lo = __builtin_amdgcn_update_dpp(lo, lo, 0x138, 0xf, 0xf, false);
    hi = __builtin_amdgcn_update_dpp(hi, hi, 0x138, 0xf, 0xf, false);
    return __longlong_as_double(((long long)hi << 32) | (unsigned int)lo);
#endif
}
__device__ __forceinline__ double lane_from_above(double v) {
#ifdef GPF_SHUFFLE_BPERMUTE
    return __shfl_down(v, 1);
#else
    const long long b = __double_as_longlong(v);
    int lo = (int)b, hi = (int)(b >> 32);
    lo = __builtin_amdgcn_update_dpp(lo, lo, 0x130, 0xf, 0xf, false);
    hi = __builtin_amdgcn_update_dpp(hi, hi, 0x130, 0xf, 0xf, false);
    return __longlong_as_double(((long long)hi << 32) | (unsigned int)lo);
#endif
}

typedef double dpair __attribute__((ext_vector_type(2)));
#ifndef GPF_K2_NT
#define GPF_K2_NT 2
#endif
__device__ __forceinline__ void asm_load16(dpair& dst, const double* lane_ptr) {
#if GPF_K2_NT & 1
    asm volatile("global_load_dwordx4 %0, %1, off nt" : "=v"(dst) : "v"(lane_ptr) : "memory");
#else
    asm volatile("global_load_dwordx4 %0, %1, off" : "=v"(dst) : "v"(lane_ptr) : "memory");
#endif
}
template <int N>
__device__ __forceinline__ void asm_wait3(dpair& a, dpair& b, dpair& c) {
    asm volatile("s_waitcnt vmcnt(%3)" : "+v"(a), "+v"(b), "+v"(c) : "n"(N) : "memory");
}
template <int N>
__device__ __forceinline__ void asm_wait1(dpair& a) {
    asm volatile("s_waitcnt vmcnt(%1)" : "+v"(a) : "n"(N) : "memory");
}

__device__ __forceinline__ double uniform_load(const double* p) {
    typedef const __attribute__((address_space(4))) double* cptr;
    return *(cptr)(unsigned long long)p;
}

template <int TOPO, bool HAS_LS>
struct RawRow {
    dpair q[3];
    dpair t[TOPO == 0 ? 3 : 1];
    dpair ls[HAS_LS ? 1 : 1];
    double th, thx, thy;
};

struct Row2 { double rho[2], jx[2], jy[2], h[2], hx[2], hy[2], Ls[2]; };

template <int EOS>
struct Red {
    double ekin, v2, c2;
    int flags;
    __device__ __forceinline__ void init() { ekin = 0.0; v2 = 0.0; c2 = (EOS == EOS_DH) ? __builtin_inf() : 0.0; flags = 0; }
    __device__ __forceinline__ void cell(double r, double jx, double jy, double w, const Phys& P) {
        const double v = (jx * jx + jy * jy) * rcp(r);
        ekin += w * (v * 0.5);
        v2 = fmax(v2, v);
        if (v != v) flags |= 1;
        if (r < 0.0) flags |= 2;
        if (EOS == EOS_DH) {
            c2 = fmin(c2, fabs(P.e[7] - r));
        } else {
            const double c = eos_c2<EOS>(r, P);
            if (!(c >= 0.0)) flags |= 4;
            c2 = fmax(c2, c);
        }
    }
};

template <int EOS, bool HAS_LS, bool PIEZO, int D, int TOPO>
__device__ __forceinline__ void step_strip2(const Step2Args& a, const Phys& P, const double* __restrict__ qin,
                                            double* __restrict__ qout, int strip, int chunk, int lane,
                                            double (*stash)[128], Acc& result) {
    const Layout L = a.L;
    const Strip2Geom G = a.G;
    const bool fused = (a.fused & 1) != 0;
    const int policy = __builtin_amdgcn_readfirstlane(a.fused);

    const bool y_periodic = a.E.rule[2][0] == BC_P;
    const bool ghost_strip = strip == G.s_ghost;
    const bool wrap_strip = fused && y_periodic && ghost_strip;
    const bool wrap_lane = wrap_strip && (lane == G.lane_wrap || lane == G.lane_wrap + 1);
    const int ma = wrap_lane ? G.wrap_ma + 2 * (lane - G.lane_wrap) : G.w0 + strip * STRIP2 + 2 * lane;
    const int iy_lo_raw = D > 0 ? ma : L.Ny - ma;
    const bool lane_ok = iy_lo_raw >= -1 && iy_lo_raw <= L.Ny + 1;
    const int iy_lo = lane_ok ? iy_lo_raw : -1;
    const int iy0 = D > 0 ? iy_lo : iy_lo + 1, iy1 = D > 0 ? iy_lo + 1 : iy_lo;
    const bool out0 = lane_ok && !wrap_lane && lane >= 1 && ma >= 1 && ma <= L.Ny;
    const bool out1 = lane_ok && !wrap_lane && lane <= 62 && ma + 1 >= 1 && ma + 1 <= L.Ny;
    const bool is_ghost_lane = ghost_strip && lane == G.lane_ghost;
    const int gsrc_lane = y_periodic ? G.wrap_src_lane : (G.slot_ghost ? G.lane_ghost : G.lane_ghost - 1);
    const int gsrc_slot = y_periodic ? G.wrap_src_slot : (G.slot_ghost ? 0 : 1);

    const int n_first = 1 + (int)(((long long)chunk * L.Nx) / a.nchunks);
    const int n_last = (int)(((long long)(chunk + 1) * L.Nx) / a.nchunks);
    const int e_dw_x = D > 0 ? 1 : 0, e_dw_y = D > 0 ? 3 : 2;
    const bool dw_row_is_ghost = (n_last == L.Nx) && a.E.halo[e_dw_x] != 1;
    const bool x_periodic = a.E.rule[0][0] == BC_P;

    const double dt = a.st->dt;
    const double cx = (double)D * P.inv_dx, cy = (double)D * P.inv_dy;

    const double* __restrict__ q0p = qin;
    const double* __restrict__ q1p = qin + L.plane;
    const double* __restrict__ q2p = qin + 2 * L.plane;
    const double* __restrict__ hp = a.topo;
    const double* __restrict__ hxp = a.topo + L.plane;
    const double* __restrict__ hyp = a.topo + 2 * L.plane;
    double* __restrict__ qo0 = qout;
    double* __restrict__ qo1 = qout + L.plane;
    double* __restrict__ qo2 = qout + 2 * L.plane;

    double lh[2] = {0.0, 0.0}, lhx[2] = {0.0, 0.0}, lhy[2] = {0.0, 0.0};
    if (TOPO == 2) {
        const int c0 = min(max(iy0, 0), L.Ny + 1), c1 = min(max(iy1, 0), L.Ny + 1);
        lh[0] = a.topo_line[c0]; lhx[0] = a.topo_line[(L.Ny + 2) + c0]; lhy[0] = a.topo_line[2 * (L.Ny + 2) + c0];
        lh[1] = a.topo_line[c1]; lhx[1] = a.topo_line[(L.Ny + 2) + c1]; lhy[1] = a.topo_line[2 * (L.Ny + 2) + c1];
    }
    const unsigned int lane_bytes = (unsigned int)(L.off + iy_lo) * 8u;
    auto pair = [&](const double* __restrict__ rowp, double& s0, double& s1) {
        const double2 v = *reinterpret_cast<const double2*>(reinterpret_cast<const char*>(rowp) + lane_bytes);
        s0 = D > 0 ? v.x : v.y; s1 = D > 0 ? v.y : v.x;
    };
    auto load = [&](int n, Row2& r) {
        const int ix = D > 0 ? n : L.Nx + 1 - n;
        const long long rb = (long long)ix * L.pitch;
        pair(q0p + rb, r.rho[0], r.rho[1]); pair(q1p + rb, r.jx[0], r.jx[1]); pair(q2p + rb, r.jy[0], r.jy[1]);
        if (TOPO == 0) {
            pair(hp + rb, r.h[0], r.h[1]); pair(hxp + rb, r.hx[0], r.hx[1]); pair(hyp + rb, r.hy[0], r.hy[1]);
        } else if (TOPO == 1 || TOPO == 3) {
            const double th = a.topo_line[ix], thx = a.topo_line[(L.Nx + 2) + ix], thy = TOPO == 1 ? a.topo_line[2 * (L.Nx + 2) + ix] : 0.0;
            r.h[0] = r.h[1] = th; r.hx[0] = r.hx[1] = thx; r.hy[0] = r.hy[1] = thy;
        } else {
            r.h[0] = lh[0]; r.h[1] = lh[1]; r.hx[0] = lhx[0]; r.hx[1] = lhx[1]; r.hy[0] = lhy[0]; r.hy[1] = lhy[1];
        }
        if (HAS_LS) pair(a.Ls + rb, r.Ls[0], r.Ls[1]);
        else r.Ls[0] = r.Ls[1] = 0.0;
    };
    constexpr int NL = 3 + (TOPO == 0 ? 3 : 0) + (HAS_LS ? 1 : 0);
    typedef RawRow<TOPO, HAS_LS> Raw;
    const double* const lane_q = reinterpret_cast<const double*>(reinterpret_cast<const char*>(qin) + lane_bytes);
    const double* const lane_t = reinterpret_cast<const double*>(reinterpret_cast<const char*>(a.topo) + lane_bytes);
    const double* const lane_ls = HAS_LS ? reinterpret_cast<const double*>(reinterpret_cast<const char*>(a.Ls) + lane_bytes) : nullptr;
    auto issue = [&](int n, Raw& r) {
        const bool dummy = n > n_last + 1;
        const int ix = D > 0 ? min(n, n_last + 1) : L.Nx + 1 - min(n, n_last + 1);
        const long long rb = (long long)ix * L.pitch;
        const long long p1 = dummy ? 0 : L.plane, p2 = dummy ? 0 : 2 * L.plane;
        const double* const a0 = lane_q + rb; const double* const a1 = lane_q + p1 + rb; const double* const a2 = lane_q + p2 + rb;
#define GPF_LD(d, a) "global_load_dwordx4 %" #d ", %" #a ", off\n\t"
#define GPF_LDNT(d, a) "global_load_dwordx4 %" #d ", %" #a ", off nt\n\t"
#define GPF_ROW_HEAD "s_cmp_lg_u32 %[nt], 0\n\ts_cbranch_scc1 .Lgpf_ldnt_%=\n\t"
#define GPF_ROW_MID "s_branch .Lgpf_lddone_%=\n.Lgpf_ldnt_%=:\n\t"
#define GPF_ROW_TAIL "\n.Lgpf_lddone_%=:"
        if constexpr (TOPO == 0 && HAS_LS) {
            const double* t0 = dummy ? lane_q : lane_t;
            const double* const a3 = t0 + rb; const double* const a4 = t0 + p1 + rb; const double* const a5 = t0 + p2 + rb;
            const double* const a6 = (dummy ? lane_q : lane_ls) + rb;
            asm volatile(GPF_ROW_HEAD GPF_LD(0, 7) GPF_LD(1, 8) GPF_LD(2, 9) GPF_LD(3, 10) GPF_LD(4, 11) GPF_LD(5, 12) GPF_LD(6, 13) GPF_ROW_MID
                         GPF_LDNT(0, 7) GPF_LDNT(1, 8) GPF_LDNT(2, 9) GPF_LDNT(3, 10) GPF_LDNT(4, 11) GPF_LDNT(5, 12) GPF_LDNT(6, 13) GPF_ROW_TAIL
                         : "=&v"(r.q[0]), "=&v"(r.q[1]), "=&v"(r.q[2]), "=&v"(r.t[0]), "=&v"(r.t[1]), "=&v"(r.t[2]), "=&v"(r.ls[0])
                         : "v"(a0), "v"(a1), "v"(a2), "v"(a3), "v"(a4), "v"(a5), "v"(a6), [nt] "s"(policy & 4) : "memory", "scc");
        } else if constexpr (TOPO == 0) {
            const double* t0 = dummy ? lane_q : lane_t;
            const double* const a3 = t0 + rb; const double* const a4 = t0 + p1 + rb; const double* const a5 = t0 + p2 + rb;
            asm volatile(GPF_ROW_HEAD GPF_LD(0, 6) GPF_LD(1, 7) GPF_LD(2, 8) GPF_LD(3, 9) GPF_LD(4, 10) GPF_LD(5, 11) GPF_ROW_MID
                         GPF_LDNT(0, 6) GPF_LDNT(1, 7) GPF_LDNT(2, 8) GPF_LDNT(3, 9) GPF_LDNT(4, 10) GPF_LDNT(5, 11) GPF_ROW_TAIL
                         : "=&v"(r.q[0]), "=&v"(r.q[1]), "=&v"(r.q[2]), "=&v"(r.t[0]), "=&v"(r.t[1]), "=&v"(r.t[2])
                         : "v"(a0), "v"(a1), "v"(a2), "v"(a3), "v"(a4), "v"(a5), [nt] "s"(policy & 4) : "memory", "scc");
        } else if constexpr (HAS_LS) {
            const double* const a3 = (dummy ? lane_q : lane_ls) + rb;
            asm volatile(GPF_ROW_HEAD GPF_LD(0, 4) GPF_LD(1, 5) GPF_LD(2, 6) GPF_LD(3, 7) GPF_ROW_MID
                         GPF_LDNT(0, 4) GPF_LDNT(1, 5) GPF_LDNT(2, 6) GPF_LDNT(3, 7) GPF_ROW_TAIL
                         : "=&v"(r.q[0]), "=&v"(r.q[1]), "=&v"(r.q[2]), "=&v"(r.ls[0])
                         : "v"(a0), "v"(a1), "v"(a2), "v"(a3), [nt] "s"(policy & 4) : "memory", "scc");
        } else {
            asm volatile(GPF_ROW_HEAD GPF_LD(0, 3) GPF_LD(1, 4) GPF_LD(2, 5) GPF_ROW_MID GPF_LDNT(0, 3) GPF_LDNT(1, 4) GPF_LDNT(2, 5) GPF_ROW_TAIL
                         : "=&v"(r.q[0]), "=&v"(r.q[1]), "=&v"(r.q[2])
                         : "v"(a0), "v"(a1), "v"(a2), [nt] "s"(policy & 4) : "memory", "scc");
        }
#undef GPF_LD
#undef GPF_LDNT
#undef GPF_ROW_HEAD
#undef GPF_ROW_MID
#undef GPF_ROW_TAIL
        if (TOPO == 1 || TOPO == 3) {
            r.th = uniform_load(a.topo_line + ix); r.thx = uniform_load(a.topo_line + (L.Nx + 2) + ix);
            r.thy = TOPO == 1 ? uniform_load(a.topo_line + 2 * (L.Nx + 2) + ix) : 0.0;
        }
    };
    constexpr bool HEAVY = Step2Weight<EOS, HAS_LS, PIEZO>::heavy;
    constexpr int AHEAD_ROWS = PIEZO ? 1 : (TOPO == 3 ? (HEAVY ? 2 : GPF_K2_AHEAD_LINE) : GPF_K2_AHEAD);
#ifndef GPF_K2_COUNT_STORES
#define GPF_K2_COUNT_STORES 1
#endif
    const bool stores_every_row = GPF_K2_COUNT_STORES && __builtin_amdgcn_ballot_w64(out0 || out1) != 0ull;
    auto arrive = [&](Raw& r, const int n) {
        constexpr int LOOSE = AHEAD_ROWS * NL, EXACT = AHEAD_ROWS * (NL + 3);
        static_assert(EXACT <= 63, "vmcnt is a 6-bit counter");
        const int exact = __builtin_amdgcn_readfirstlane((stores_every_row && n > n_first + AHEAD_ROWS) ? 1 : 0);
#define GPF_WAIT_ROW "s_cmp_lg_u32 %[ex], 0\n\ts_cbranch_scc1 .Lgpf_exact_%=\n\ts_waitcnt vmcnt(%[loose])\n.Lgpf_exact_%=:\n\ts_waitcnt vmcnt(%[exact])"
        if constexpr (TOPO == 0 && HAS_LS)
            asm volatile(GPF_WAIT_ROW : "+v"(r.q[0]), "+v"(r.q[1]), "+v"(r.q[2]), "+v"(r.t[0]), "+v"(r.t[1]), "+v"(r.t[2]), "+v"(r.ls[0])
                         : [ex] "s"(exact), [loose] "n"(LOOSE), [exact] "n"(EXACT) : "memory", "scc");
        else if constexpr (TOPO == 0)
            asm volatile(GPF_WAIT_ROW : "+v"(r.q[0]), "+v"(r.q[1]), "+v"(r.q[2]), "+v"(r.t[0]), "+v"(r.t[1]), "+v"(r.t[2])
                         : [ex] "s"(exact), [loose] "n"(LOOSE), [exact] "n"(EXACT) : "memory", "scc");
        else if constexpr (HAS_LS)
            asm volatile(GPF_WAIT_ROW : "+v"(r.q[0]), "+v"(r.q[1]), "+v"(r.q[2]), "+v"(r.ls[0])
                         : [ex] "s"(exact), [loose] "n"(LOOSE), [exact] "n"(EXACT) : "memory", "scc");
        else
            asm volatile(GPF_WAIT_ROW : "+v"(r.q[0]), "+v"(r.q[1]), "+v"(r.q[2])
                         : [ex] "s"(exact), [loose] "n"(LOOSE), [exact] "n"(EXACT) : "memory", "scc");
#undef GPF_WAIT_ROW
    };
    auto unpack = [&](const Raw& r, Row2& o) {
        o.rho[0] = D > 0 ? r.q[0].x : r.q[0].y; o.rho[1] = D > 0 ? r.q[0].y : r.q[0].x;
        o.jx[0] = D > 0 ? r.q[1].x : r.q[1].y; o.jx[1] = D > 0 ? r.q[1].y : r.q[1].x;
        o.jy[0] = D > 0 ? r.q[2].x : r.q[2].y; o.jy[1] = D > 0 ? r.q[2].y : r.q[2].x;
        if (TOPO == 0) {
            o.h[0] = D > 0 ? r.t[0].x : r.t[0].y; o.h[1] = D > 0 ? r.t[0].y : r.t[0].x;
            o.hx[0] = D > 0 ? r.t[1].x : r.t[1].y; o.hx[1] = D > 0 ? r.t[1].y : r.t[1].x;
            o.hy[0] = D > 0 ? r.t[2].x : r.t[2].y; o.hy[1] = D > 0 ? r.t[2].y : r.t[2].x;
        } else if (TOPO == 1 || TOPO == 3) {
            o.h[0] = o.h[1] = r.th; o.hx[0] = o.hx[1] = r.thx; o.hy[0] = o.hy[1] = r.thy;
        } else {
            o.h[0] = lh[0]; o.h[1] = lh[1]; o.hx[0] = lhx[0]; o.hx[1] = lhx[1]; o.hy[0] = lhy[0]; o.hy[1] = lhy[1];
        }
        if (HAS_LS) { o.Ls[0] = D > 0 ? r.ls[0].x : r.ls[0].y; o.Ls[1] = D > 0 ? r.ls[0].y : r.ls[0].x; }
        else o.Ls[0] = o.Ls[1] = 0.0;
    };
    constexpr bool LS0 = !HAS_LS && !PIEZO;
    auto closure = [&](const Row2& r, int k, const double* q, const TopoRcp& t, const GapCoef& gc, const RowCoef& rc, CellFlux& f) {
        if (TOPO == 3) {
            cell_closure_xonly<EOS>(q ? q[0] : r.rho[k], q ? q[1] : r.jx[k], q ? q[2] : r.jy[k], rc, P, f);
        } else if (LS0) {
            cell_closure_ls0<EOS>(q ? q[0] : r.rho[k], q ? q[1] : r.jx[k], q ? q[2] : r.jy[k], gc, P, f);
        } else {
            CellIn c;
            c.rho = q ? q[0] : r.rho[k]; c.jx = q ? q[1] : r.jx[k]; c.jy = q ? q[2] : r.jy[k];
            c.h = r.h[k]; c.hx = r.hx[k]; c.hy = r.hy[k]; c.Ls = r.Ls[k];
            cell_closure<EOS, true, HAS_LS, PIEZO>(c, t, P, f);
        }
    };
    auto cell_of = [&](const Row2& r, int k) {
        CellIn c;
        c.rho = r.rho[k]; c.jx = r.jx[k]; c.jy = r.jy[k]; c.h = r.h[k]; c.hx = r.hx[k]; c.hy = r.hy[k]; c.Ls = r.Ls[k];
        return c;
    };

    Red<EOS> red;
    red.init();
    const int seam_row_lo = a.E.halo[0] == 2 ? 1 : -1, seam_row_hi = a.E.halo[1] == 2 ? L.Nx : -1;

    if (fused && dw_row_is_ghost && x_periodic) {
        Row2 r0, r1;
        if (a.E.halo[e_dw_x] == 2) {
            load(L.Nx, r0);
            load(L.Nx + 1, r1);
            auto seam_topo = [&](const double* __restrict__ t, Row2& r) {
                if (TOPO == 1 || TOPO == 3) {
                    r.h[0] = r.h[1] = t[L.off + 1]; r.hx[0] = r.hx[1] = t[L.pitch + L.off + 1];
                    r.hy[0] = r.hy[1] = TOPO == 1 ? t[2 * L.pitch + L.off + 1] : 0.0;
                } else {
                    pair(t, r.h[0], r.h[1]); pair(t + L.pitch, r.hx[0], r.hx[1]); pair(t + 2 * L.pitch, r.hy[0], r.hy[1]);
                }
                if (HAS_LS) pair(t + 3 * L.pitch, r.Ls[0], r.Ls[1]);
            };
            seam_topo(a.seam[e_dw_x] + 4 * L.pitch, r0);
            seam_topo(a.seam[e_dw_x], r1);
        } else {
            load(0, r0);
            load(1, r1);
        }
        double fy[2][3], q1[2][3];
        CellFlux f0[2], f1[2];
        const RowCoef rc0 = TOPO == 3 ? row_coefficients(r0.h[0], r0.hx[0], P) : RowCoef();
        const RowCoef rc1 = TOPO == 3 ? row_coefficients(r1.h[0], r1.hx[0], P) : RowCoef();
        for (int k = 0; k < 2; ++k) {
            closure(r0, k, nullptr, topo_rcp<HAS_LS>(cell_of(r0, k)), gap_coefficients(r0.h[k], r0.hx[k], r0.hy[k]), rc0, f0[k]);
            closure(r1, k, nullptr, topo_rcp<HAS_LS>(cell_of(r1, k)), gap_coefficients(r1.h[k], r1.hx[k], r1.hy[k]), rc1, f1[k]);
            fy[k][0] = r1.jy[k]; fy[k][1] = f1[k].fx2; fy[k][2] = f1[k].fy2;
        }
        const double u0 = lane_from_below(fy[1][0]), u1 = lane_from_below(fy[1][1]), u2 = lane_from_below(fy[1][2]);
        const double up[2][3] = {{u0, u1, u2}, {fy[0][0], fy[0][1], fy[0][2]}};
        for (int k = 0; k < 2; ++k) {
            q1[k][0] = predictor_value(r1.rho[k], dt, cx, r1.jx[k] - r0.jx[k], cy, fy[k][0] - up[k][0], f1[k].s0);
            q1[k][1] = predictor_value(r1.jx[k], dt, cx, f1[k].fx1 - f0[k].fx1, cy, fy[k][1] - up[k][1], f1[k].s1);
            q1[k][2] = predictor_value(r1.jy[k], dt, cx, f1[k].fx2 - f0[k].fx2, cy, fy[k][2] - up[k][2], f1[k].s2);
            for (int c = 0; c < 3; ++c) stash[c][2 * lane + k] = q1[k][c];
        }
    }

    if (!fused && dw_row_is_ghost) {
        const int c0 = min(max(iy0, 0), L.Ny + 1), c1 = min(max(iy1, 0), L.Ny + 1);
        for (int c = 0; c < 3; ++c) {
            stash[c][2 * lane] = a.g1x[c * L.pitch + L.off + c0];
            stash[c][2 * lane + 1] = a.g1x[c * L.pitch + L.off + c1];
        }
    }

    constexpr int AHEAD = AHEAD_ROWS;
    static_assert(AHEAD >= 1 && AHEAD <= 6, "1 to 6 rows ahead");
    constexpr int NB = AHEAD + 1;
    Raw rowbuf[NB];
    issue(n_first - 1, rowbuf[0]);
    if (AHEAD >= 2) issue(n_first, rowbuf[1 % NB]);
    if (AHEAD >= 3) issue(n_first + 1, rowbuf[2 % NB]);
    if (AHEAD >= 4) issue(n_first + 2, rowbuf[3 % NB]);
    if (AHEAD >= 5) issue(n_first + 3, rowbuf[4 % NB]);
    if (AHEAD >= 6) issue(n_first + 4, rowbuf[5 % NB]);

    double fx1p[2][3] = {{0, 0, 0}, {0, 0, 0}};
    double part[2][3] = {{0, 0, 0}, {0, 0, 0}};

    auto march = [&](const int n, Raw& raw, Raw& spare) {
        issue(n + AHEAD, spare);
        arrive(raw, n);
        Row2 cur;
        unpack(raw, cur);
        const bool first = (n == n_first - 1);
        const bool last = (n == n_last + 1);
        const int ix = D > 0 ? n : L.Nx + 1 - n;

        TopoRcp tr[2] = {TopoRcp(), TopoRcp()};
        GapCoef gc[2] = {GapCoef(), GapCoef()};
        RowCoef rc = RowCoef();
        if (TOPO == 3) {
            rc = row_coefficients(cur.h[0], cur.hx[0], P);
        } else if (LS0) {
            gc[0] = gap_coefficients(cur.h[0], cur.hx[0], cur.hy[0]);
            gc[1] = gap_coefficients(cur.h[1], cur.hx[1], cur.hy[1]);
        } else {
            tr[0] = topo_rcp<HAS_LS>(cell_of(cur, 0));
            tr[1] = topo_rcp<HAS_LS>(cell_of(cur, 1));
        }

        double q1[2][3];
        if (last && dw_row_is_ghost) {
            for (int k = 0; k < 2; ++k)
                for (int c = 0; c < 3; ++c) q1[k][c] = stash[c][2 * lane + k];
        } else {
            CellFlux f[2];
            double fy[2][3];
            for (int k = 0; k < 2; ++k) {
                closure(cur, k, nullptr, tr[k], gc[k], rc, f[k]);
                fy[k][0] = cur.jy[k]; fy[k][1] = f[k].fx2; fy[k][2] = f[k].fy2;
            }
            const double u0 = lane_from_below(fy[1][0]), u1 = lane_from_below(fy[1][1]), u2 = lane_from_below(fy[1][2]);
            const double up[2][3] = {{u0, u1, u2}, {fy[0][0], fy[0][1], fy[0][2]}};
            for (int k = 0; k < 2; ++k) {
                q1[k][0] = predictor_value(cur.rho[k], dt, cx, cur.jx[k] - fx1p[k][0], cy, fy[k][0] - up[k][0], f[k].s0);
                q1[k][1] = predictor_value(cur.jx[k], dt, cx, f[k].fx1 - fx1p[k][1], cy, fy[k][1] - up[k][1], f[k].s1);
                q1[k][2] = predictor_value(cur.jy[k], dt, cx, f[k].fx2 - fx1p[k][2], cy, fy[k][2] - up[k][2], f[k].s2);
                fx1p[k][0] = cur.jx[k]; fx1p[k][1] = f[k].fx1; fx1p[k][2] = f[k].fx2;
            }
            if (ghost_strip) {
                double gv[3];
                if (!fused) {
                    for (int c = 0; c < 3; ++c) gv[c] = uniform_load(a.g1y + c * (L.Nx + 2) + ix);
                } else {
                    for (int c = 0; c < 3; ++c)
                        gv[c] = ghost_rule(a.E, e_dw_y, c, __shfl(gsrc_slot ? q1[1][c] : q1[0][c], gsrc_lane));
                }
                if (is_ghost_lane) {
                    for (int c = 0; c < 3; ++c) {
                        if (G.slot_ghost) q1[1][c] = gv[c];
                        else q1[0][c] = gv[c];
                    }
                }
            }
            if (fused && n == n_last && dw_row_is_ghost && !x_periodic) {
                for (int k = 0; k < 2; ++k)
                    for (int c = 0; c < 3; ++c) stash[c][2 * lane + k] = ghost_rule(a.E, e_dw_x, c, q1[k][c]);
            }
        }

        if (!first) {
            CellFlux g[2];
            double gy[2][3];
            for (int k = 0; k < 2; ++k) {
                closure(cur, k, q1[k], tr[k], gc[k], rc, g[k]);
                gy[k][0] = q1[k][2]; gy[k][1] = g[k].fx2; gy[k][2] = g[k].fy2;
            }
            const double d0 = lane_from_above(gy[0][0]), d1 = lane_from_above(gy[0][1]), d2 = lane_from_above(gy[0][2]);
            const double dn[2][3] = {{gy[1][0], gy[1][1], gy[1][2]}, {d0, d1, d2}};

            if (n > n_first) {
                double o[2][3];
                for (int k = 0; k < 2; ++k) {
                    o[k][0] = 0.5 * (part[k][0] - dt * cx * q1[k][1]);
                    o[k][1] = 0.5 * (part[k][1] - dt * cx * g[k].fx1);
                    o[k][2] = 0.5 * (part[k][2] - dt * cx * g[k].fx2);
                }
                const int ixo = D > 0 ? n - 1 : L.Nx + 2 - n;
                const long long rbo = (long long)ixo * L.pitch;
#if GPF_K2_NT & 2
                const bool store_nt = (policy & 2) && (ixo & 7) >= ((policy >> 3) & 7);
#endif
                auto st16 = [&](double* __restrict__ rowp, double va, double vb) {
                    dpair v;
                    v.x = D > 0 ? va : vb; v.y = D > 0 ? vb : va;
                    dpair* p = reinterpret_cast<dpair*>(reinterpret_cast<char*>(rowp) + lane_bytes);
#if GPF_K2_NT & 2
                    asm volatile("s_cmp_lg_u32 %[nt], 0\n\ts_cbranch_scc1 .Lgpf_stnt_%=\n\t"
                                 "global_store_dwordx4 %0, %1, off\n\ts_branch .Lgpf_stdone_%=\n"
                                 ".Lgpf_stnt_%=:\n\tglobal_store_dwordx4 %0, %1, off nt\n"
                                 ".Lgpf_stdone_%=:\n\ts_nop 0"
                                 :: "v"(p), "v"(v), [nt] "s"(__builtin_amdgcn_readfirstlane(store_nt ? 1 : 0)) : "memory", "scc");
#else
                    *p = v;
#endif
                };
                auto st8 = [&](double* __restrict__ rowp, unsigned int bytes, double v) {
                    *reinterpret_cast<double*>(reinterpret_cast<char*>(rowp) + bytes) = v;
                };
                if (out0 && out1) {
                    st16(qo0 + rbo, o[0][0], o[1][0]); st16(qo1 + rbo, o[0][1], o[1][1]); st16(qo2 + rbo, o[0][2], o[1][2]);
                } else if (out0) {
                    const unsigned int b = (unsigned int)(L.off + iy0) * 8u;
                    st8(qo0 + rbo, b, o[0][0]); st8(qo1 + rbo, b, o[0][1]); st8(qo2 + rbo, b, o[0][2]);
                } else if (out1) {
                    const unsigned int b = (unsigned int)(L.off + iy1) * 8u;
                    st8(qo0 + rbo, b, o[1][0]); st8(qo1 + rbo, b, o[1][1]); st8(qo2 + rbo, b, o[1][2]);
                }
                const double w = 1.0 + (ixo == seam_row_lo ? 1.0 : 0.0) + (ixo == seam_row_hi ? 1.0 : 0.0);
                if (out0) red.cell(o[0][0], o[0][1], o[0][2], w, P);
                if (out1) red.cell(o[1][0], o[1][1], o[1][2], w, P);
            }
            for (int k = 0; k < 2; ++k) {
                part[k][0] = (cur.rho[k] + q1[k][0]) - dt * (-cx * q1[k][1] + cy * (dn[k][0] - gy[k][0]) - g[k].s0);
                part[k][1] = (cur.jx[k] + q1[k][1]) - dt * (-cx * g[k].fx1 + cy * (dn[k][1] - gy[k][1]) - g[k].s1);
                part[k][2] = (cur.jy[k] + q1[k][2]) - dt * (-cx * g[k].fx2 + cy * (dn[k][2] - gy[k][2]) - g[k].s2);
            }
        }
    };
    for (int n = n_first - 1;;) {
        march(n, rowbuf[0], rowbuf[AHEAD]); if (++n > n_last + 1) break;
        march(n, rowbuf[1], rowbuf[0]); if (++n > n_last + 1) break;
        if (AHEAD >= 2) { march(n, rowbuf[2 % NB], rowbuf[1]); if (++n > n_last + 1) break; }
        if (AHEAD >= 3) { march(n, rowbuf[3 % NB], rowbuf[2 % NB]); if (++n > n_last + 1) break; }
        if (AHEAD >= 4) { march(n, rowbuf[4 % NB], rowbuf[3 % NB]); if (++n > n_last + 1) break; }
        if (AHEAD >= 5) { march(n, rowbuf[5 % NB], rowbuf[4 % NB]); if (++n > n_last + 1) break; }
        if (AHEAD >= 6) { march(n, rowbuf[6 % NB], rowbuf[5 % NB]); if (++n > n_last + 1) break; }
    }
    for (int b = 0; b <= AHEAD; ++b) {
        asm_wait3<0>(rowbuf[b].q[0], rowbuf[b].q[1], rowbuf[b].q[2]);
        if (TOPO == 0) asm_wait3<0>(rowbuf[b].t[0], rowbuf[b].t[1], rowbuf[b].t[2]);
        if (HAS_LS) asm_wait1<0>(rowbuf[b].ls[0]);
    }

#ifndef GPF_K2_NO_POSTPASS
    if (fused) {
        asm volatile("s_waitcnt vmcnt(0)" ::: "memory");
        const int src_row[2] = {x_periodic ? L.Nx : 1, x_periodic ? 1 : L.Nx};
        const int src_col[2] = {y_periodic ? L.Ny : 1, y_periodic ? 1 : L.Ny};
        const int ix_lo = D > 0 ? n_first : L.Nx + 1 - n_last, ix_hi = D > 0 ? n_last : L.Nx + 1 - n_first;
        auto get = [&](int ix, int iy, double v[3]) {
            const long long o = (long long)ix * L.pitch + L.off + iy;
            v[0] = qo0[o]; v[1] = qo1[o]; v[2] = qo2[o];
        };
        auto put = [&](int ix, int iy, const double v[3], double w) {
            const long long o = (long long)ix * L.pitch + L.off + iy;
            qo0[o] = v[0]; qo1[o] = v[1]; qo2[o] = v[2];
            red.cell(v[0], v[1], v[2], w, P);
        };
        double* send_to[2] = {nullptr, nullptr};
        if (a.p2p.on) {
            const int slot = (int)((*a.p2p.seq + 1) & 1);
            if (a.E.halo[0] && a.p2p.rank_lo >= 0) send_to[0] = p2p_rows(a.p2p.box[a.p2p.rank_lo], slot, 1, L.pitch);
            if (a.E.halo[1] && a.p2p.rank_hi >= 0) send_to[1] = p2p_rows(a.p2p.box[a.p2p.rank_hi], slot, 0, L.pitch);
        } else if (a.msg) {
            if (a.E.halo[0]) send_to[0] = a.msg;
            if (a.E.halo[1]) send_to[1] = a.msg + 3 * L.pitch;
        }
        auto send = [&](int e, int iy, const double v[3]) {
            double* d = send_to[e] + L.off + iy;
            for (int c = 0; c < 3; ++c) {
                if (a.p2p.on)
                    __hip_atomic_store(reinterpret_cast<unsigned long long*>(d + c * L.pitch), (unsigned long long)__double_as_longlong(v[c]),
                                       __ATOMIC_RELAXED, __HIP_MEMORY_SCOPE_SYSTEM);
                else d[c * L.pitch] = v[c];
            }
        };
        const int m_out_lo = max(G.w0 + strip * STRIP2 + 1, 1), m_out_hi = min(G.w0 + strip * STRIP2 + STRIP2, L.Ny);
        for (int ey = 0; ey < 2; ++ey) {
            const int msrc = D > 0 ? src_col[ey] : L.Ny + 1 - src_col[ey];
            if (msrc < m_out_lo || msrc > m_out_hi) continue;
            for (int ix = ix_lo + lane; ix <= ix_hi; ix += 64) {
                double v[3], g[3];
                get(ix, src_col[ey], v);
                for (int c = 0; c < 3; ++c) g[c] = ghost_rule(a.E, 2 + ey, c, v[c]);
                put(ix, ey ? L.Ny + 1 : 0, g, 1.0 + (ix == seam_row_lo ? 1.0 : 0.0) + (ix == seam_row_hi ? 1.0 : 0.0));
                if (ix == 1 && send_to[0]) send(0, ey ? L.Ny + 1 : 0, g);
                if (ix == L.Nx && send_to[1]) send(1, ey ? L.Ny + 1 : 0, g);
            }
        }
        for (int e = 0; e < 2; ++e) {
            if (a.E.halo[e]) continue;
            if (src_row[e] < ix_lo || src_row[e] > ix_hi) continue;
            const int ixg = e ? L.Nx + 1 : 0;
            for (int k = 0; k < 2; ++k) {
                if (!(k ? out1 : out0)) continue;
                const int iy = k ? iy1 : iy0;
                double v[3], g[3], gc[3];
                get(src_row[e], iy, v);
                for (int c = 0; c < 3; ++c) g[c] = ghost_rule(a.E, e, c, v[c]);
                put(ixg, iy, g, 1.0);
                for (int ey = 0; ey < 2; ++ey) {
                    if (iy != src_col[ey]) continue;
                    for (int c = 0; c < 3; ++c) gc[c] = ghost_rule(a.E, 2 + ey, c, g[c]);
                    put(ixg, ey ? L.Ny + 1 : 0, gc, 1.0);
                }
            }
        }
        for (int e = 0; e < 2; ++e) {
            const int ixb = e ? L.Nx : 1;
            if (!send_to[e] || ixb < ix_lo || ixb > ix_hi) continue;
            for (int k = 0; k < 2; ++k) {
                if (!(k ? out1 : out0)) continue;
                double v[3];
                get(ixb, k ? iy1 : iy0, v);
                send(e, k ? iy1 : iy0, v);
            }
        }
        if (a.p2p.on) asm volatile("s_waitcnt vmcnt(0)" ::: "memory");
    }
#endif

    for (int s = 32; s >= 1; s >>= 1) {
        red.ekin += __shfl_down(red.ekin, s);
        red.v2 = fmax(red.v2, __shfl_down(red.v2, s));
        const double oc = __shfl_down(red.c2, s);
        red.c2 = (EOS == EOS_DH) ? fmin(red.c2, oc) : fmax(red.c2, oc);
        red.flags |= __shfl_down(red.flags, s);
    }
    if (EOS == EOS_DH) {
        const double it = rcp(red.c2);
        red.c2 = (red.c2 == __builtin_inf()) ? 0.0 : P.e[6] * (it * it);
    }
#ifdef GPF_K2_NO_POSTPASS
    red.flags = 0;
#endif
    result.ekin = red.ekin; result.v2 = red.v2; result.c2 = red.c2; result.mass = 0.0; result.flags = red.flags;
}

template <int EOS, bool HAS_LS, bool PIEZO, int D, int TOPO>
__global__ __launch_bounds__(256, (Step2Weight<EOS, HAS_LS, PIEZO>::heavy ? 1 : ((TOPO == 1 || TOPO == 3) ? GPF_K2_MINWAVES_LINE : GPF_K2_MINWAVES)))
void k_step2(const Step2Args a, const Phys P) {
    __shared__ double stash[4][3][128];
    __shared__ Acc red_sm[4];
    __shared__ int s_last;
    if (halted(a.st, a.honor_stop)) return;
    if (predictor_direction(a.st) != D) __builtin_trap();
    const int par = a.st->parity;
    const double* qin = par ? a.qb : a.qa;
    double* qout = const_cast<double*>(par ? a.qa : a.qb);

    const int nb = gridDim.x;
    const int lb = (int)(blockIdx.x & 7) * (nb >> 3) + (int)(blockIdx.x >> 3);
    const int wv = __builtin_amdgcn_readfirstlane(threadIdx.x >> 6), lane = threadIdx.x & 63;
    const int w = lb * 4 + wv;
    const int strip = w % a.G.nstrips, chunk = w / a.G.nstrips;
    const bool active = chunk < a.nchunks;

    Acc own;
    own.zero();
    if (active) step_strip2<EOS, HAS_LS, PIEZO, D, TOPO>(a, P, qin, qout, strip, chunk, lane, stash[wv], own);

    if (!(a.fused & 1)) {
        if (active && lane == 0) {
            Partial p;
            p.ekin = own.ekin; p.vmax2 = own.v2; p.c2max = own.c2; p.flags = (double)own.flags;
            a.partials[w] = p;
        }
        return;
    }
#ifdef GPF_K2_NO_FINISH
    if (blockIdx.x == 0 && threadIdx.x == 0) commit_step(a.st, own.ekin + 1.0, own.v2, own.c2, own.flags, a.log, a.log_base, a.log_cap);
    return;
#endif
    if (lane == 0) red_sm[wv] = own;
    __syncthreads();
    if (threadIdx.x == 0) {
        Acc tot = red_sm[0];
        for (int i = 1; i < 4; ++i) { tot.ekin += red_sm[i].ekin; tot.v2 = fmax(tot.v2, red_sm[i].v2); tot.c2 = fmax(tot.c2, red_sm[i].c2); tot.flags |= red_sm[i].flags; }
        publish_partial(a.block_partials + blockIdx.x, tot);
        const unsigned int t = __hip_atomic_fetch_add(a.arrive, 1u, GPF_ORDER_ARRIVE, __HIP_MEMORY_SCOPE_AGENT);
        s_last = (t == (unsigned int)nb - 1) ? 1 : 0;
        if (s_last) __hip_atomic_store(a.arrive, 0u, __ATOMIC_RELAXED, __HIP_MEMORY_SCOPE_AGENT);
    }
    __syncthreads();
    if (!s_last) return;
    finish_tail(a.st, a.log, a.log_base, a.log_cap, a.out, a.block_partials, a.p2p, red_sm);
}

}
```

### include/gapflow_hip.h

```cpp
#ifndef GAPFLOW_HIP_H
#define GAPFLOW_HIP_H

#include <stddef.h>
#include <stdint.h>

#ifdef __cplusplus
extern "C" {
#endif

typedef struct gpf_handle gpf_handle;

typedef enum {
    GPF_OK = 0,
    GPF_ERR_INVALID = -1,
    GPF_ERR_HIP = -2,
    GPF_ERR_NO_DEVICE = -3,
    GPF_ERR_SOLVER = -4,
    GPF_ERR_STATE = -5
} gpf_status;

enum { GPF_EOS_DH = 0, GPF_EOS_PL = 1, GPF_EOS_VDW = 2, GPF_EOS_MT = 3,
       GPF_EOS_CUBIC = 4, GPF_EOS_BWR = 5, GPF_EOS_BAYADA = 6 };

enum { GPF_BC_PERIODIC = 0, GPF_BC_DIRICHLET = 1, GPF_BC_NEUMANN = 2 };

enum { GPF_PIEZO_NONE = 0, GPF_PIEZO_BARUS = 1, GPF_PIEZO_ROELANDS = 2,
       GPF_PIEZO_DUKLER = 3, GPF_PIEZO_MCADAMS = 4 };

enum { GPF_THINNING_NONE = 0, GPF_THINNING_EYRING = 1, GPF_THINNING_CARREAU = 2 };

enum {
    GPF_FIELD_Q = 0,
    GPF_FIELD_TOPO = 1,
    GPF_FIELD_EXTRA = 2,
    GPF_FIELD_PRESSURE = 3,
    GPF_FIELD_TAU_AVG = 4,
    GPF_FIELD_WALL_LOWER = 5,
    GPF_FIELD_WALL_UPPER = 6,
    GPF_FIELD_PRESSURE_VAR = 7,
    GPF_FIELD_WALL_XZ_VAR = 8,
    GPF_FIELD_WALL_YZ_VAR = 9,
    GPF_FIELD_DEFORMATION = 10
};

typedef struct {
    int32_t Nx, Ny;
    double  dx, dy;
    double  U, V;
    double  eta, zeta;
    int32_t eos;
    double  eos_par[8];
    int32_t piezo;
    double  piezo_par[4];
    int32_t bc_rule[4][3];
    double  bc_value[4];
    int32_t halo_lo, halo_hi;
    int32_t adaptive;
    double  CFL, dt_fixed, tol;
    int64_t max_it;
    int32_t mc_order;
    int32_t device;
    int32_t thinning;
    double  thinning_par[4];
} gpf_config;

typedef struct {
    int64_t step;
    double  simtime, dt;
    double  ekin, ekin_old;
    double  residual;
    double  v_max, v_sound;
    double  mass;
    int32_t invalid;
    int32_t converged;
} gpf_scalars_t;

int gpf_create(const gpf_config* cfg, gpf_handle** out);
int gpf_destroy(gpf_handle* h);
int gpf_set_stream(gpf_handle* h, void* hip_stream);
const char* gpf_last_error(void);
int gpf_device_count(void);

int gpf_upload(gpf_handle* h, int field, const double* host, size_t count);
int gpf_download(gpf_handle* h, int field, double* host, size_t count);
int gpf_update_closures(gpf_handle* h);

int gpf_pre_run(gpf_handle* h);
int gpf_step(gpf_handle* h, int64_t n, int honor_stop, gpf_scalars_t* log, int64_t log_capacity,
             int64_t* n_executed);
int gpf_step_timed(gpf_handle* h, int64_t n, double* kernel_ms, double* total_ms);
const char* gpf_plan_note(gpf_handle* h);
int gpf_step_unfused(gpf_handle* h);
int gpf_scalars(gpf_handle* h, gpf_scalars_t* out);
int gpf_set_ekin_old(gpf_handle* h, double value);
int gpf_set_dt(gpf_handle* h, double dt);

int gpf_slab_message(gpf_handle* h, void** message, size_t* count);
int gpf_step_local(gpf_handle* h, int honor_stop);
int gpf_step_commit(gpf_handle* h, int honor_stop, const void* gathered, int nranks, int rank_lo, int rank_hi);
int gpf_elastic_setup(gpf_handle* h, int px, int py, const double* greens_ri, size_t count, double alpha,
                      double force_scale, int relative);
int gpf_elastic_update(gpf_handle* h);
int gpf_elastic_slab_setup(gpf_handle* h, int px, int py, int nranks, const int32_t* plan, size_t plan_count,
                           const double* greens_ri, size_t greens_count, const double* h0_rows, size_t h0_count,
                           double alpha, double force_scale, int relative);
int gpf_elastic_slab_buffer(gpf_handle* h, int which, void** ptr, size_t* count);
int gpf_elastic_slab_forward(gpf_handle* h, const void* gathered, int nranks);
int gpf_elastic_slab_convolve(gpf_handle* h);
int gpf_elastic_slab_finish(gpf_handle* h);
int gpf_elastic_slab_apply(gpf_handle* h);

int gpf_p2p_export(gpf_handle* h, void* ipc_handle, size_t handle_bytes);
int gpf_p2p_connect(gpf_handle* h, int rank, int nranks, const void* ipc_handles, int rank_lo, int rank_hi);
int gpf_step_p2p(gpf_handle* h, int64_t n, int honor_stop);
int gpf_p2p_set_timeout(gpf_handle* h, double seconds);
int gpf_upload_beyond(gpf_handle* h, int side, const double* rho_row, size_t count);
int gpf_stage_message(gpf_handle* h);
int gpf_stage_absorb(gpf_handle* h, const void* gathered, int nranks, int rank_lo, int rank_hi);
int gpf_close_step_local(gpf_handle* h);
int gpf_close_step_commit(gpf_handle* h, const void* gathered, int nranks, gpf_scalars_t* out);
int gpf_state(gpf_handle* h, gpf_scalars_t* out);
int gpf_set_seam_topo(gpf_handle* h, int side, const double* host, size_t count);

int gpf_predictor_corrector(int nx, int ny, const double* q, const double* p, const double* tau,
                            int direction, double* flux_x, double* flux_y);
int gpf_source(int nx, int ny, const double* q, const double* h, const double* stress,
               const double* lower, const double* upper, double* out);

int gpf_viscous_stress(int64_t n, const double* q, const double* hh, const double* dqx, const double* dqy,
                       const double* eta, const double* Ls, double U, double V, double zeta, int slip_both,
                       double* bottom, double* top, double* avg);
int gpf_eos(int eos, const double* eos_par, int64_t n, const double* rho, double* pressure, double* sound);
int gpf_viscosity(int kind, int law, const double* par, double mu0, int64_t n, const double* a0, const double* a1,
                  const double* a2, double u1, double u2, double* out);

int gpf_open_step(gpf_handle* h);
int gpf_stage_closures(gpf_handle* h);
int gpf_stage_advance(gpf_handle* h, int stage);
int gpf_close_step(gpf_handle* h, gpf_scalars_t* out);

const char* gpf_gp_factorisation(void);
int gpf_gp_fit(int device, int n, int d, int m, const double* Xn, const double* Yn, double amp,
               const double* inv_scale, double sigma, double* L, double* alpha, double* logdet);
int gpf_gp_set_model(gpf_handle* h, int which, int n, int d, int m, const int32_t* dims, const double* x_scale,
                     const double* Xn, const double* Yn, double amp, const double* inv_scale, double sigma,
                     double yscale);
int gpf_gp_clear_model(gpf_handle* h, int which);
int gpf_gp_set_scales(gpf_handle* h, int which, const double* x_scale, double yscale);
int gpf_gp_variance(gpf_handle* h, int which, int on_open_step, double* max_var);
int gpf_gp_pass_counts(gpf_handle* h, int64_t launched[3], int64_t* reused);

typedef struct gpf_nll gpf_nll;
int gpf_gp_nll_open(int device, int n, int d, int m, const double* Xn, const double* Yn, double sigma, gpf_nll** out);
int gpf_gp_nll_eval(gpf_nll* s, const double* theta, double* value, double* grad, int* info);
int gpf_gp_nll_close(gpf_nll* s);

enum {
    GPF_PROFILE_Z = 1,
    GPF_PROFILE_U = 2,
    GPF_PROFILE_V = 4,
    GPF_PROFILE_TAU = 8
};
enum { GPF_PROFILE_GRADIENTS = 1 };
enum { GPF_PROFILE_BOTH = 0, GPF_PROFILE_TOP = 1, GPF_PROFILE_BOTTOM = 2, GPF_PROFILE_NONE = 3 };
int gpf_gap_profiles_op(int64_t n, int nz, const double* z, const double* q, const double* hh, const double* dqx,
                        const double* dqy, const double* eta, const double* zeta, const double* Ls, int per_cell,
                        double U, double V, int mode, int field_mask, double* out);
int gpf_gap_profiles(gpf_handle* h, int nz, int ix0, int ix1, int field_mask, int flags, double* host_out);
int gpf_profile_store_probe(int device, int64_t ncell, int nlev, int nplanes, int reps, double* ms_per_pass);

int gpf_stream_probe(int device, int nin, int nout, int64_t doubles_per_plane, int reps, double* ms_per_pass);

#ifdef __cplusplus
}
#endif
#endif
```

Baseline: 120,000 Mcell-updates/s.

## Precompute per-row gap coefficients into a device table for x-only topography

For topographies that depend only on x, the step kernel used to recompute the row coefficients from h and dh/dx for every row it marched through. This change builds a per-row RowCoef table once when the topography is uploaded, plus entries for the seam rows. A new TOPO mode 4 step kernel reads these through uniform scalar loads instead of recomputing them. It trades the repeated transcendental and division work per row for an extra small table that must be kept in sync with topography and seam updates, and it adds a debug API to read the table back.

```diff
diff --git a/gapflow_amd/_lib.py b/gapflow_amd/_lib.py
--- a/gapflow_amd/_lib.py
+++ b/gapflow_amd/_lib.py
@@ -108,6 +108,7 @@
     'gpf_gp_clear_model': (C.c_int, [C.c_void_p, C.c_int]),
     'gpf_gp_factorisation': (C.c_char_p, []),
     'gpf_plan_note': (C.c_char_p, [C.c_void_p]),
+    'gpf_row_coefficients': (C.c_int, [C.c_void_p, C.c_int, _DP, C.c_size_t]),
     'gpf_gp_set_scales': (C.c_int, [C.c_void_p, C.c_int, _DP, C.c_double]),
     'gpf_gp_variance': (C.c_int, [C.c_void_p, C.c_int, C.c_int, _DP]),
     'gpf_gp_pass_counts': (C.c_int, [C.c_void_p, C.POINTER(C.c_int64), C.POINTER(C.c_int64)]),
diff --git a/gapflow_amd/csrc/api.hip b/gapflow_amd/csrc/api.hip
--- a/gapflow_amd/csrc/api.hip
+++ b/gapflow_amd/csrc/api.hip
@@ -60,6 +60,8 @@
     double* q[2] = {nullptr, nullptr};
     double* topo = nullptr;
     double* topo_line = nullptr;
+    RowCoef* rowcoef = nullptr;
+    bool rowcoef_table = true;
     int topo_mode = 0;
     bool topo_hy0 = false;
     double* Ls = nullptr;
@@ -240,6 +242,7 @@
     }
     h->E.halo[0] = cfg->halo_lo; h->E.halo[1] = cfg->halo_hi;
     h->split_edges = std::getenv("GPF_STEP_UNFUSED_EDGES") != nullptr;
+    if (const char* s = std::getenv("GPF_ROWCOEF_TABLE")) h->rowcoef_table = std::atoi(s) != 0;
     h->gp_reuse_state_mean = std::getenv("GPF_GP_NO_STATE_MEAN") == nullptr;
     make_phys(*cfg, h->P);
 
@@ -283,7 +286,7 @@
     hipSetDevice(h->cfg.device);
     hipStreamSynchronize(h->stream);
     for (void* p : {(void*)h->q[0], (void*)h->q[1], (void*)h->topo, (void*)h->plan_master}) field_free(p);
-    void* ptrs[] = {h->topo_line, h->Ls, h->g1, h->seam, h->halo, h->beyond, h->st, h->partials, h->arrive, h->block_partials, h->spart,
+    void* ptrs[] = {h->topo_line, h->rowcoef, h->Ls, h->g1, h->seam, h->halo, h->beyond, h->st, h->partials, h->arrive, h->block_partials, h->spart,
                     h->log, h->stage, h->fields, h->work, h->st_trial, h->gpvar, h->gp_state_mean, h->gpscratch, h->gptile,
                     h->gp[0].Z, h->gp[0].alpha, h->gp[0].L, h->gp[1].Z, h->gp[1].alpha, h->gp[1].L,
                     h->gp[2].Z, h->gp[2].alpha, h->gp[2].L, h->gp[0].Linv, h->gp[1].Linv, h->gp[2].Linv, h->gp[0].W, h->gp[1].W, h->gp[2].W};
@@ -341,6 +344,24 @@
     if (h->fields) return GPF_OK;
     HIP_TRY(hipMalloc(&h->fields, (size_t)16 * h->L.plane * sizeof(double)));
     HIP_TRY(hipMemsetAsync(h->fields, 0, (size_t)16 * h->L.plane * sizeof(double), h->stream));
+    return GPF_OK;
+}
+
+static int build_rowcoef(gpf_handle* h, bool rows, int side) {
+    const Layout& L = h->L;
+    const int n = L.Nx + 2;
+    if (!h->rowcoef) {
+        HIP_TRY(hipMalloc(&h->rowcoef, (size_t)(n + 4) * sizeof(RowCoef)));
+        HIP_TRY(hipMemsetAsync(h->rowcoef, 0, (size_t)(n + 4) * sizeof(RowCoef), h->stream));
+    }
+    if (rows)
+        hipLaunchKernelGGL(k_row_coef_table, dim3((n + 255) / 256), dim3(256), 0, h->stream, (const double*)h->topo_line,
+                           (const double*)h->topo_line + n, 1ll, n, h->P, h->rowcoef);
+    if (side >= 0 && h->seam) {
+        const double* t = h->seam + (size_t)side * 8 * L.pitch + L.off + 1;
+        hipLaunchKernelGGL(k_row_coef_table, dim3(1), dim3(64), 0, h->stream, t, t + L.pitch, 4ll * L.pitch, 2, h->P, h->rowcoef + n + 2 * side);
+    }
+    HIP_TRY(hipGetLastError());
     return GPF_OK;
 }
 
@@ -395,6 +416,12 @@
             h->topo_hy0 = hy0;
             if (!h->topo_line) HIP_TRY(hipMalloc(&h->topo_line, (size_t)3 * (std::max(nx, ny)) * sizeof(double)));
             HIP_TRY(hipMemcpy(h->topo_line, line.data(), line.size() * sizeof(double), hipMemcpyHostToDevice));
+            if (hy0 && h->rowcoef_table) {
+                const bool fresh = h->rowcoef == nullptr;
+                GPF_TRY(build_rowcoef(h, true, -1));
+                for (int e = 0; e < 2 && fresh; ++e)
+                    if (h->has_seam[e]) GPF_TRY(build_rowcoef(h, false, e));
+            }
         }
     }
     GPF_TRY(ensure_stage(h, count));
@@ -630,8 +657,38 @@
 
 static int topo_mode_of(const gpf_handle* h) {
     if (h->Ls != nullptr || h->cfg.piezo != 0 || std::getenv("GPF_TOPO_PLANES")) return 0;
-    if (h->topo_mode == 1 && h->topo_hy0 && !std::getenv("GPF_TOPO_GENERIC")) return 3;
+    if (h->topo_mode == 1 && h->topo_hy0 && !std::getenv("GPF_TOPO_GENERIC")) return (h->rowcoef_table && h->rowcoef) ? 4 : 3;
     return h->topo_mode;
+}
+static bool topo_xonly(const gpf_handle* h) { return topo_mode_of(h) >= 3; }
+
+extern "C" int gpf_row_coefficients(gpf_handle* h, int source, double* host, size_t count) {
+    if (!h || !host || source < 0 || source > 1) return fail(GPF_ERR_INVALID, "gpf_row_coefficients: bad argument");
+    const Layout& L = h->L;
+    const int n = L.Nx + 2;
+    if (count != (size_t)8 * (n + 4)) return fail(GPF_ERR_INVALID, "gpf_row_coefficients: count must be 8*(Nx+2+4)");
+    if (topo_mode_of(h) != 4) return fail(GPF_ERR_STATE, "gpf_row_coefficients: this handle's step does not read a row-coefficient table");
+    GPF_TRY(enter(h, true));
+    const RowCoef* src = h->rowcoef;
+    RowCoef* fresh = nullptr;
+    if (source == 1) {
+        HIP_TRY(hipMalloc(&fresh, (size_t)(n + 4) * sizeof(RowCoef)));
+        HIP_TRY(hipMemsetAsync(fresh, 0, (size_t)(n + 4) * sizeof(RowCoef), h->stream));
+        const double* col = h->topo + L.off + 1;
+        hipLaunchKernelGGL(k_row_coef_table, dim3((n + 255) / 256), dim3(256), 0, h->stream, col, col + L.plane, (long long)L.pitch, n, h->P, fresh);
+        for (int e = 0; e < 2; ++e) {
+            if (!h->has_seam[e]) continue;
+            const double* t = h->seam + (size_t)e * 8 * L.pitch + L.off + 1;
+            hipLaunchKernelGGL(k_row_coef_table, dim3(1), dim3(64), 0, h->stream, t, t + L.pitch, 4ll * L.pitch, 2, h->P, fresh + n + 2 * e);
+        }
+        src = fresh;
+    }
+    hipError_t e = hipGetLastError();
+    if (e == hipSuccess) e = hipMemcpyAsync(host, src, count * sizeof(double), hipMemcpyDeviceToHost, h->stream);
+    if (e == hipSuccess) e = hipStreamSynchronize(h->stream);
+    if (fresh) hipFree(fresh);
+    if (e != hipSuccess) return fail(GPF_ERR_HIP, std::string("gpf_row_coefficients: ") + hipGetErrorString(e));
+    return GPF_OK;
 }
 
 typedef void (*step2_kernel_t)(const Step2Args, const Phys);
@@ -650,6 +707,8 @@
             k = D > 0 ? k_step2<EOS_, false, false, 1, 2> : k_step2<EOS_, false, false, -1, 2>;
         } else if (topo_mode == 3) {
             k = D > 0 ? k_step2<EOS_, false, false, 1, 3> : k_step2<EOS_, false, false, -1, 3>;
+        } else if (topo_mode == 4) {
+            k = D > 0 ? k_step2<EOS_, false, false, 1, 4> : k_step2<EOS_, false, false, -1, 4>;
         } else {
             k = D > 0 ? k_step2<EOS_, false, false, 1, 0> : k_step2<EOS_, false, false, -1, 0>;
         }
@@ -713,6 +772,7 @@
     const bool fused = step2_fused(h);
     const Strip2Geom& G2 = h->geom2[D > 0 ? 0 : 1];
     a2.qa = h->q[0]; a2.qb = h->q[1]; a2.topo = h->topo; a2.topo_line = h->topo_line; a2.Ls = h->Ls;
+    a2.rowcoef = h->rowcoef;
     a2.g1x = h->g1; a2.g1y = h->g1 + 3 * L.pitch;
     a2.st = h->st; a2.partials = h->partials; a2.block_partials = h->block_partials; a2.arrive = h->arrive;
     a2.log = h->log; a2.log_base = log_base; a2.log_cap = h->log_cap;
@@ -774,7 +834,7 @@
     }
     EOS_DISPATCH(h->cfg.eos, {
         if (!h->g1_ready) {
-            if (topo_mode_of(h) == 3) hipLaunchKernelGGL((k_ghost_stage1<EOS_, false, false, true>), ggrid, dim3(256), 0, h->stream, g, h->P);
+            if (topo_xonly(h)) hipLaunchKernelGGL((k_ghost_stage1<EOS_, false, false, true>), ggrid, dim3(256), 0, h->stream, g, h->P);
             else LS_PIEZO_DISPATCH(has_ls, h->cfg.piezo != 0, hipLaunchKernelGGL((k_ghost_stage1<EOS_, LS_, PZ_, false>), ggrid, dim3(256), 0, h->stream, g, h->P));
         }
         if (ev0) hipEventRecord(ev0, h->stream);
@@ -782,7 +842,7 @@
         if (ev1) hipEventRecord(ev1, h->stream);
         hipLaunchKernelGGL((k_ghost_fill<EOS_>), dim3(h->nghost_blocks + nsend), dim3(256), 0, h->stream, gf, f, h->nghost_blocks, h->P);
         if (p2p) {
-            if (topo_mode_of(h) == 3) hipLaunchKernelGGL((k_begin_slab<EOS_, false, false, true, true>), ggrid, dim3(256), 0, h->stream, g, w, h->P);
+            if (topo_xonly(h)) hipLaunchKernelGGL((k_begin_slab<EOS_, false, false, true, true>), ggrid, dim3(256), 0, h->stream, g, w, h->P);
             else LS_PIEZO_DISPATCH(has_ls, h->cfg.piezo != 0, hipLaunchKernelGGL((k_begin_slab<EOS_, LS_, PZ_, false, true>), ggrid, dim3(256), 0, h->stream, g, w, h->P));
         }
     });
diff --git a/gapflow_amd/csrc/api_plan.inc b/gapflow_amd/csrc/api_plan.inc
--- a/gapflow_amd/csrc/api_plan.inc
+++ b/gapflow_amd/csrc/api_plan.inc
@@ -190,6 +190,10 @@
     char buf[64];
     std::snprintf(buf, sizeof buf, ", keep %d/8 rows on-die", h->keep_rows2);
     return buf;
+}
+static const char* coef_note(const gpf_handle* h) {
+    const int topo = topo_mode_of(h);
+    return topo == 4 ? ", row coefficients from the table" : topo == 3 ? ", row coefficients evaluated in the kernel" : "";
 }
 static int plan_step2(gpf_handle* h, int D) {
     if (h->plan2_valid) return GPF_OK;
@@ -219,8 +223,8 @@
                       one_per_simd >= 1 && L.Nx / one_per_simd >= 16 && !(env_chunks && env_nt);
     if (!tune) {
         GPF_TRY(plan_apply(h, nchunks, nt, keep));
-        std::snprintf(h->plan2_note, sizeof h->plan2_note, "%d chunks per strip, %s%s (rule of thumb%s)", h->nchunks2,
-                      NT_NAME[h->nt_policy2], keep_note(h).c_str(), (env_chunks || env_nt || env_keep) ? ", pinned by the environment" : "");
+        std::snprintf(h->plan2_note, sizeof h->plan2_note, "%d chunks per strip, %s%s%s (rule of thumb%s)", h->nchunks2,
+                      NT_NAME[h->nt_policy2], coef_note(h), keep_note(h).c_str(), (env_chunks || env_nt || env_keep) ? ", pinned by the environment" : "");
         h->plan2_valid = true;
         return GPF_OK;
     }
@@ -303,8 +307,8 @@
     GPF_TRY(plan_apply(h, best_chunks, best_nt, best_keep));
     const std::string kept = keep_note(h) + (keep_seen.empty() ? (env_keep && h->nt_policy2 >= 1 ? " (pinned by the environment)" : "")
                                                                : " (timed, us: k" + keep_seen + ")");
-    std::snprintf(h->plan2_note, sizeof h->plan2_note, "%d chunks per strip, %s%s (timed, us:%s;%s%s%s)", h->nchunks2,
-                  NT_NAME[h->nt_policy2], kept.c_str(), seen.c_str(), placement_note.c_str(),
+    std::snprintf(h->plan2_note, sizeof h->plan2_note, "%d chunks per strip, %s%s%s (timed, us:%s;%s%s%s)", h->nchunks2,
+                  NT_NAME[h->nt_policy2], coef_note(h), kept.c_str(), seen.c_str(), placement_note.c_str(),
                   placement_note.empty() ? "" : "; before the placement:", placement_note.empty() ? "" : first_seen.c_str());
     DBG("plan_step2: %s", h->plan2_note);
     h->plan2_valid = true;
diff --git a/gapflow_amd/csrc/api_slab_allgather.inc b/gapflow_amd/csrc/api_slab_allgather.inc
--- a/gapflow_amd/csrc/api_slab_allgather.inc
+++ b/gapflow_amd/csrc/api_slab_allgather.inc
@@ -57,7 +57,7 @@
     const dim3 ggrid(fused ? SLAB_COMMIT_BLOCKS : std::min((L.Nx + L.Ny + 63) / 64, 512));
     EOS_DISPATCH(h->cfg.eos, {
         if (fused) hipLaunchKernelGGL((k_begin_slab<EOS_, false, false, false, false>), ggrid, dim3(256), 0, h->stream, g, w, h->P);
-        else if (topo_mode_of(h) == 3) hipLaunchKernelGGL((k_begin_slab<EOS_, false, false, true, false>), ggrid, dim3(256), 0, h->stream, g, w, h->P);
+        else if (topo_xonly(h)) hipLaunchKernelGGL((k_begin_slab<EOS_, false, false, true, false>), ggrid, dim3(256), 0, h->stream, g, w, h->P);
         else LS_PIEZO_DISPATCH(h->Ls != nullptr, h->cfg.piezo != 0, hipLaunchKernelGGL((k_begin_slab<EOS_, LS_, PZ_, false, false>), ggrid, dim3(256), 0, h->stream, g, w, h->P));
     });
     HIP_TRY(hipGetLastError());
diff --git a/gapflow_amd/csrc/api_slab_p2p.inc b/gapflow_amd/csrc/api_slab_p2p.inc
--- a/gapflow_amd/csrc/api_slab_p2p.inc
+++ b/gapflow_amd/csrc/api_slab_p2p.inc
@@ -85,5 +85,9 @@
         for (int iy = 0; iy < L.Ny + 2; ++iy) tmp[(size_t)r * L.pitch + L.off + iy] = host[(size_t)r * (L.Ny + 2) + iy];
     HIP_TRY(hipMemcpy(h->seam + (size_t)side * 8 * L.pitch, tmp.data(), tmp.size() * sizeof(double), hipMemcpyHostToDevice));
     h->has_seam[side] = true;
+    if (h->rowcoef) {
+        GPF_TRY(build_rowcoef(h, false, side));
+        HIP_TRY(hipStreamSynchronize(h->stream));
+    }
     return GPF_OK;
 }
diff --git a/gapflow_amd/csrc/aux_kernels.hip b/gapflow_amd/csrc/aux_kernels.hip
--- a/gapflow_amd/csrc/aux_kernels.hip
+++ b/gapflow_amd/csrc/aux_kernels.hip
@@ -668,6 +668,12 @@
     }
 }
 
+__global__ void k_row_coef_table(const double* __restrict__ h, const double* __restrict__ hx, long long stride, int count, Phys P,
+                                 RowCoef* __restrict__ out) {
+    const int i = blockIdx.x * blockDim.x + threadIdx.x;
+    if (i < count) out[i] = row_coefficients(h[i * stride], hx[i * stride], P);
+}
+
 __global__ void k_copy3(const double* src, double* dst, long long n) {
     for (long long i = blockIdx.x * (long long)blockDim.x + threadIdx.x; i < n; i += (long long)gridDim.x * blockDim.x)
         dst[i] = src[i];
diff --git a/gapflow_amd/csrc/step2_kernel.hip b/gapflow_amd/csrc/step2_kernel.hip
--- a/gapflow_amd/csrc/step2_kernel.hip
+++ b/gapflow_amd/csrc/step2_kernel.hip
@@ -33,6 +33,7 @@
 struct Step2Args {
     const double* qa; const double* qb;
     const double* topo; const double* topo_line; const double* Ls;
+    const RowCoef* rowcoef;
     const double* g1x; const double* g1y;
     const double* seam[2];
     double* out;
@@ -97,6 +98,15 @@
     return *(cptr)(unsigned long long)p;
 }
 
+__device__ __forceinline__ RowCoef uniform_load_coef(const RowCoef* p) {
+    typedef double d8 __attribute__((ext_vector_type(8)));
+    typedef const __attribute__((address_space(4))) d8* cptr;
+    const d8 v = *(cptr)(unsigned long long)p;
+    RowCoef r;
+    r.A = v[0]; r.B = v[1]; r.C = v[2]; r.S0 = v[3]; r.S1a = v[4]; r.S1b = v[5]; r.S2a = v[6]; r.S2b = v[7];
+    return r;
+}
+
 template <int TOPO, bool HAS_LS>
 struct RawRow {
     dpair q[3];
@@ -171,6 +181,7 @@
     double* __restrict__ qo1 = qout + L.plane;
     double* __restrict__ qo2 = qout + 2 * L.plane;
 
+    constexpr bool TABLE = TOPO == 4;
     double lh[2] = {0.0, 0.0}, lhx[2] = {0.0, 0.0}, lhy[2] = {0.0, 0.0};
     if (TOPO == 2) {
         const int c0 = min(max(iy0, 0), L.Ny + 1), c1 = min(max(iy1, 0), L.Ny + 1);
@@ -191,6 +202,8 @@
         } else if (TOPO == 1 || TOPO == 3) {
             const double th = a.topo_line[ix], thx = a.topo_line[(L.Nx + 2) + ix], thy = TOPO == 1 ? a.topo_line[2 * (L.Nx + 2) + ix] : 0.0;
             r.h[0] = r.h[1] = th; r.hx[0] = r.hx[1] = thx; r.hy[0] = r.hy[1] = thy;
+        } else if (TABLE) {
+            r.h[0] = r.h[1] = r.hx[0] = r.hx[1] = r.hy[0] = r.hy[1] = 0.0;
         } else {
             r.h[0] = lh[0]; r.h[1] = lh[1]; r.hx[0] = lhx[0]; r.hx[1] = lhx[1]; r.hy[0] = lhy[0]; r.hy[1] = lhy[1];
         }
@@ -250,7 +263,7 @@
         }
     };
     constexpr bool HEAVY = Step2Weight<EOS, HAS_LS, PIEZO>::heavy;
-    constexpr int AHEAD_ROWS = PIEZO ? 1 : (TOPO == 3 ? (HEAVY ? 2 : GPF_K2_AHEAD_LINE) : GPF_K2_AHEAD);
+    constexpr int AHEAD_ROWS = PIEZO ? 1 : ((TOPO == 3 || TABLE) ? (HEAVY ? 2 : GPF_K2_AHEAD_LINE) : GPF_K2_AHEAD);
 #ifndef GPF_K2_COUNT_STORES
 #define GPF_K2_COUNT_STORES 1
 #endif
@@ -284,6 +297,8 @@
             o.hy[0] = D > 0 ? r.t[2].x : r.t[2].y; o.hy[1] = D > 0 ? r.t[2].y : r.t[2].x;
         } else if (TOPO == 1 || TOPO == 3) {
             o.h[0] = o.h[1] = r.th; o.hx[0] = o.hx[1] = r.thx; o.hy[0] = o.hy[1] = r.thy;
+        } else if (TABLE) {
+            o.h[0] = o.h[1] = o.hx[0] = o.hx[1] = o.hy[0] = o.hy[1] = 0.0;
         } else {
             o.h[0] = lh[0]; o.h[1] = lh[1]; o.hx[0] = lhx[0]; o.hx[1] = lhx[1]; o.hy[0] = lhy[0]; o.hy[1] = lhy[1];
         }
@@ -292,7 +307,7 @@
     };
     constexpr bool LS0 = !HAS_LS && !PIEZO;
     auto closure = [&](const Row2& r, int k, const double* q, const TopoRcp& t, const GapCoef& gc, const RowCoef& rc, CellFlux& f) {
-        if (TOPO == 3) {
+        if (TOPO == 3 || TABLE) {
             cell_closure_xonly<EOS>(q ? q[0] : r.rho[k], q ? q[1] : r.jx[k], q ? q[2] : r.jy[k], rc, P, f);
         } else if (LS0) {
             cell_closure_ls0<EOS>(q ? q[0] : r.rho[k], q ? q[1] : r.jx[k], q ? q[2] : r.jy[k], gc, P, f);
@@ -319,7 +334,9 @@
             load(L.Nx, r0);
             load(L.Nx + 1, r1);
             auto seam_topo = [&](const double* __restrict__ t, Row2& r) {
-                if (TOPO == 1 || TOPO == 3) {
+                if (TABLE) {
+                    r.h[0] = r.h[1] = r.hx[0] = r.hx[1] = r.hy[0] = r.hy[1] = 0.0;
+                } else if (TOPO == 1 || TOPO == 3) {
                     r.h[0] = r.h[1] = t[L.off + 1]; r.hx[0] = r.hx[1] = t[L.pitch + L.off + 1];
                     r.hy[0] = r.hy[1] = TOPO == 1 ? t[2 * L.pitch + L.off + 1] : 0.0;
                 } else {
@@ -335,8 +352,17 @@
         }
         double fy[2][3], q1[2][3];
         CellFlux f0[2], f1[2];
-        const RowCoef rc0 = TOPO == 3 ? row_coefficients(r0.h[0], r0.hx[0], P) : RowCoef();
-        const RowCoef rc1 = TOPO == 3 ? row_coefficients(r1.h[0], r1.hx[0], P) : RowCoef();
+        RowCoef rc0 = RowCoef(), rc1 = RowCoef();
+        if (TOPO == 3) {
+            rc0 = row_coefficients(r0.h[0], r0.hx[0], P);
+            rc1 = row_coefficients(r1.h[0], r1.hx[0], P);
+        } else if (TABLE) {
+            const bool seam = a.E.halo[e_dw_x] == 2;
+            const int i0 = seam ? L.Nx + 2 + 2 * e_dw_x + 1 : (D > 0 ? 0 : L.Nx + 1);
+            const int i1 = seam ? L.Nx + 2 + 2 * e_dw_x : (D > 0 ? 1 : L.Nx);
+            rc0 = uniform_load_coef(a.rowcoef + i0);
+            rc1 = uniform_load_coef(a.rowcoef + i1);
+        }
         for (int k = 0; k < 2; ++k) {
             closure(r0, k, nullptr, topo_rcp<HAS_LS>(cell_of(r0, k)), gap_coefficients(r0.h[k], r0.hx[k], r0.hy[k]), rc0, f0[k]);
             closure(r1, k, nullptr, topo_rcp<HAS_LS>(cell_of(r1, k)), gap_coefficients(r1.h[k], r1.hx[k], r1.hy[k]), rc1, f1[k]);
@@ -374,6 +400,13 @@
     double fx1p[2][3] = {{0, 0, 0}, {0, 0, 0}};
     double part[2][3] = {{0, 0, 0}, {0, 0, 0}};
 
+    auto coef_of = [&](int n) {
+        const int m = min(n, n_last + 1);
+        return uniform_load_coef(a.rowcoef + (D > 0 ? m : L.Nx + 1 - m));
+    };
+    RowCoef rc_row = RowCoef();
+    if (TABLE) rc_row = coef_of(n_first - 1);
+
     auto march = [&](const int n, Raw& raw, Raw& spare) {
         issue(n + AHEAD, spare);
         arrive(raw, n);
@@ -388,6 +421,8 @@
         RowCoef rc = RowCoef();
         if (TOPO == 3) {
             rc = row_coefficients(cur.h[0], cur.hx[0], P);
+        } else if (TABLE) {
+            rc = rc_row;
         } else if (LS0) {
             gc[0] = gap_coefficients(cur.h[0], cur.hx[0], cur.hy[0]);
             gc[1] = gap_coefficients(cur.h[1], cur.hx[1], cur.hy[1]);
@@ -494,6 +529,7 @@
                 part[k][2] = (cur.jy[k] + q1[k][2]) - dt * (-cx * g[k].fx2 + cy * (dn[k][2] - gy[k][2]) - g[k].s2);
             }
         }
+        if (TABLE) rc_row = coef_of(n + 1);
     };
     for (int n = n_first - 1;;) {
         march(n, rowbuf[0], rowbuf[AHEAD]); if (++n > n_last + 1) break;
@@ -606,7 +642,7 @@
 }
 
 template <int EOS, bool HAS_LS, bool PIEZO, int D, int TOPO>
-__global__ __launch_bounds__(256, (Step2Weight<EOS, HAS_LS, PIEZO>::heavy ? 1 : ((TOPO == 1 || TOPO == 3) ? GPF_K2_MINWAVES_LINE : GPF_K2_MINWAVES)))
+__global__ __launch_bounds__(256, (Step2Weight<EOS, HAS_LS, PIEZO>::heavy ? 1 : ((TOPO == 1 || TOPO == 3 || TOPO == 4) ? GPF_K2_MINWAVES_LINE : GPF_K2_MINWAVES)))
 void k_step2(const Step2Args a, const Phys P) {
     __shared__ double stash[4][3][128];
     __shared__ Acc red_sm[4];
diff --git a/include/gapflow_hip.h b/include/gapflow_hip.h
--- a/include/gapflow_hip.h
+++ b/include/gapflow_hip.h
@@ -90,6 +90,7 @@
              int64_t* n_executed);
 int gpf_step_timed(gpf_handle* h, int64_t n, double* kernel_ms, double* total_ms);
 const char* gpf_plan_note(gpf_handle* h);
+int gpf_row_coefficients(gpf_handle* h, int source, double* host, size_t count);
 int gpf_step_unfused(gpf_handle* h);
 int gpf_scalars(gpf_handle* h, gpf_scalars_t* out);
 int gpf_set_ekin_old(gpf_handle* h, double value);
```

Result: faster. 123,900 Mcell-updates/s (median of 6 runs) (+3.3%).
